# daisy9542/yolo-puncture

Hardware: AMD Instinct MI355X
Metric: images/sec (higher is better)
Workload: dtype bf16

## Files before the change

### include/yolop.h

```cpp
#ifndef YOLOP_H
#define YOLOP_H

#include <stddef.h>
#include <stdint.h>

#ifdef __cplusplus
extern "C" {
#endif

#define YP_OK 0
#define YP_ERR_ARG -1
#define YP_ERR_STATE -2
#define YP_ERR_HIP -3
#define YP_ERR_WEIGHT -4

#define YP_BF16 0
#define YP_F32 1

#define YP_TASK_DETECT 0
#define YP_TASK_SEGMENT 1

#define YP_NM 32
#define YP_MAX_MASKS 480

typedef struct yp_engine yp_engine;

typedef struct yp_model_desc {
    int variant;
    int nc;
    int task;
    int dtype;
    int max_det;
    int family;
} yp_model_desc;

#define YP_FAMILY_V10 0
#define YP_FAMILY_V8 8
#define YP_FAMILY_11 11

const char* yp_last_error(void);

int yp_create(const yp_model_desc* desc, int device, yp_engine** out);
int yp_destroy(yp_engine* e);

int yp_weight_count(const yp_engine* e);
int yp_weight_info(const yp_engine* e, int i, char* name, int name_cap, int64_t shape[4], int* ndim);

int yp_set_weight(yp_engine* e, const char* name, const float* host, const int64_t* shape, int ndim);

int yp_finalize(yp_engine* e);

int yp_forward(yp_engine* e, const uint8_t* in_dev, int B, int H, int W, float* det_out, int32_t* idx_out,
               float* coeff_out, void* stream);

int yp_proto(const yp_engine* e, const void** proto_dev, int* Hp, int* Wp);

int yp_masks(yp_engine* e, int b, const float* coeff_dev, const float* boxes_dev, int n, int oh, int ow,
             int retina, uint8_t* masks_out, int64_t* id_out, int32_t* kept_out, int suppress_small,
             int min_area, void* stream);

int yp_id_mask_resized(yp_engine* e, int b, const float* coeff_dev, const float* boxes_dev, int n, int oh, int ow, int rh,
                       int rw, int64_t* id_out, int32_t* kept_out, int suppress_small, int min_area, void* stream);

int yp_masks_frames(yp_engine* e, const int32_t* frame_idx_host, int k, const float* coeff_dev, long coeff_row_stride,
                    const float* boxes_dev, int oh, int ow, uint8_t* masks_out, void* stream);
int yp_masks_frames_input(yp_engine* e, const int32_t* frame_idx_host, int k, const float* coeff_dev, long coeff_row_stride,
                          const float* boxes_dev, int oh, int ow, uint8_t* masks_out, void* stream);

#define YP_CONTOURS_LARGEST 0
#define YP_CONTOURS_ALL 1
int yp_mask_contours(const uint8_t* masks_dev, int n, int H, int W, int strategy, int max_pts, int32_t* pts_out, int32_t* count_out,
                     int32_t* parts_out, int parts_cap, double* rect_out, void* stream);
int yp_mask_contours_scaled(const uint8_t* masks_dev, int n, int H, int W, int strategy, int max_pts, int32_t* pts_out, int32_t* count_out,
                            int32_t* parts_out, int parts_cap, double* rect_out, int H0, int W0, void* stream);

#define YP_CONTOURS_ONLY_DECLINED 1
#define YP_CONTOURS_LARGE_MAX_DIM 4096
#define YP_CONTOURS_LARGE_MAX_STARTS 65536
size_t yp_mask_contours_large_workspace(int n, int H, int W);
int yp_mask_contours_large(const uint8_t* masks_dev, int n, int H, int W, int strategy, int max_pts, int32_t* pts_out, int32_t* count_out,
                           int32_t* parts_out, int parts_cap, double* rect_out, int H0, int W0, int flags, void* workspace_dev,
                           size_t workspace_bytes, void* stream);

int yp_letterbox(const uint8_t* src_dev, int h0, int w0, uint8_t* dst_dev, int out_h, int out_w, int new_h, int new_w,
                 int top, int left, int pad_value, void* stream);
int yp_letterbox_batch(const uint8_t* src_dev, int n, int h0, int w0, uint8_t* dst_dev, int out_h, int out_w, int new_h,
                       int new_w, int top, int left, int pad_value, void* stream);

typedef struct yp_u2net yp_u2net;
int yp_u2net_create(int variant, int dtype, int device, yp_u2net** out);
int yp_u2net_destroy(yp_u2net* e);
int yp_u2net_weight_count(const yp_u2net* e);
int yp_u2net_weight_info(const yp_u2net* e, int i, char* name, int name_cap, int64_t shape[4], int* ndim);
int yp_u2net_set_weight(yp_u2net* e, const char* name, const float* host, const int64_t* shape, int ndim);
int yp_u2net_finalize(yp_u2net* e);
int yp_u2net_forward(yp_u2net* e, const uint8_t* bgr_dev, int B, int H, int W, float* prob_out, float* norm_out,
                     uint8_t* mask_out, void* stream);
int yp_u2net_forward_crops(yp_u2net* e, const uint8_t* frames_dev, int N, int H, int W, const int32_t* windows, const int32_t* frame_idx,
                           int B, int ch, int cw, float* prob_out, uint8_t* crop_mask_out, uint8_t* frame_mask_out, void* stream);
int yp_u2net_set_graph(yp_u2net* e, int enable);
int yp_u2net_tensor_count(const yp_u2net* e);
int yp_u2net_tensor_info(const yp_u2net* e, int i, char* name, int name_cap, int dims[4] );
int yp_u2net_tensor_read(yp_u2net* e, int i, float* host_out);
#define YP_U2_OP_INFO 17
int yp_u2net_op_count(const yp_u2net* e);
int yp_u2net_op_info(const yp_u2net* e, int i, char* name, int name_cap, int32_t* info, int info_cap);

typedef struct yp_cls yp_cls;
int yp_cls_create(int variant, int dtype, int device, yp_cls** out);
int yp_cls_destroy(yp_cls* e);
int yp_cls_weight_count(const yp_cls* e);
int yp_cls_weight_info(const yp_cls* e, int i, char* name, int name_cap, int64_t shape[4], int* ndim);
int yp_cls_set_weight(yp_cls* e, const char* name, const float* host, const int64_t* shape, int ndim);
int yp_cls_finalize(yp_cls* e);
int yp_cls_forward(yp_cls* e, const uint8_t* frames_dev, int B, int H, int W, int bgr, const int32_t* boxes_dev, float* logits_out,
                   float* prob_out, int32_t* cls_out, void* stream);
int yp_cls_set_graph(yp_cls* e, int enable);
int yp_cls_tensor_count(const yp_cls* e);
int yp_cls_tensor_info(const yp_cls* e, int i, char* name, int name_cap, int dims[4] );
int yp_cls_tensor_read(yp_cls* e, int i, float* host_out);

typedef struct yp_comm yp_comm;
int yp_comm_unique_id(void* id128);
int yp_comm_create(const void* id128, int rank, int world, int device, yp_comm** out);
int yp_allgather(yp_comm* c, const void* send_dev, void* recv_dev, size_t bytes_per_rank, void* stream);
int yp_comm_destroy(yp_comm* c);

#define YP_MAX_ANCHORS 294912
int yp_max_batch(const yp_engine* e, int H, int W);
int yp_plan(yp_engine* e, int B, int H, int W);
int yp_op_info(const yp_engine* e, int i, char* name, int name_cap, int* kind, double* flops,
               double* bytes);
int yp_op_kernel(const yp_engine* e, int i, char* name, int name_cap);
int yp_op_output(const yp_engine* e, int i, int* tensor, int* coff, int* C);
int yp_op_input(const yp_engine* e, int i, int* tensor, int* coff, int* C, int* c_read);
int yp_op_fusion(const yp_engine* e, int i, int* pre, int* pre_stored);
int yp_debug_op_form(const yp_engine* e, int i, int* form, int* absorbed, int cap);
int yp_run_op(yp_engine* e, int i, const uint8_t* in_dev, float* det_out, int32_t* idx_out, float* coeff_out, void* stream);
int yp_tensor_write(yp_engine* e, int tensor, int coff, int C, const float* host);
int yp_tensor_count(const yp_engine* e);
int yp_tensor_info(const yp_engine* e, int i, char* name, int name_cap, int dims[4] , int* is_f32);
int yp_tensor_read(yp_engine* e, int i, float* host_out);

int yp_profile(yp_engine* e, const uint8_t* in_dev, int B, int H, int W, float* det_out, int32_t* idx_out,
               float* coeff_out, float* ms_out, int iters, void* stream);

int yp_set_nms(yp_engine* e, float conf, float iou);

int yp_set_autotune(yp_engine* e, int enable);

int yp_tuning_export(const yp_engine* e, int32_t* cfg_out, int cap);
int yp_tuning_import(yp_engine* e, int B, int H, int W, const int32_t* cfg, int n);

int yp_debug_force_conv_cfg(int cfg);
int yp_debug_op_cfg(const yp_engine* e, int i, int* cfg);
int yp_debug_last_store_form(void);
int yp_debug_conv_families(int* base, int* num_cfgs, int cap);
int yp_debug_ablation(int v);
int yp_debug_head_clocks(uint64_t* out8);
int yp_debug_topk_anchors(const uint32_t* const mk_dev[3], int B, const int hw[3][2], int k, int32_t* sel_out_dev, uint32_t* thr_out_dev, void* stream);
int yp_debug_head_branch_clocks(uint64_t* out8);
int yp_debug_head_winners(yp_engine* e, int32_t* sel_host, float* box_host, float* coeff_host);
int yp_debug_contour_clocks(uint64_t* out12);
int yp_debug_pwsp_clocks(uint64_t* out32);

int yp_tuning_source(const yp_engine* e);

int yp_debug_host_selftest(yp_engine* e);
int yp_debug_graph_info(const yp_engine* e, int64_t* out6);
int yp_debug_head_positions(yp_engine* e, int64_t* out6);
int yp_debug_marker(void* stream);

int yp_set_graph(yp_engine* e, int enable);

#ifdef __cplusplus
}
#endif
#endif
```

### yolo-puncture_amd/csrc/c2f_fused.hip

```cpp
#include "common.h"
#include <cstdio>
#include <cstdlib>
#include <vector>

namespace yp {

constexpr int CF_NW = 8;
constexpr int CF_TH = 8;
constexpr int CF_PW = 20, CF_PP = 12 * 20;
constexpr int CF_TW = 18, CF_TP = 10 * 18;
constexpr int CF_AB = CF_PP * 128;
constexpr int CF_TS = 192 * 64, CF_CS = 128 * 64;
constexpr int CF_W33 = 9 * 32 * 64, CF_W3 = 3 * 64 * 64;
constexpr int CF_LDS = 2 * CF_AB + CF_TS + CF_CS + 2 * CF_W33 + CF_W3 + 512;

__global__ __launch_bounds__(CF_NW * 64) void c2f_fused_kernel(const C2fParams p, const int tiles_h, const int tiles_w, const int G) {
    constexpr unsigned OOB = 0x80000000u;
    extern __shared__ __attribute__((aligned(1024))) unsigned char smem[];
    unsigned char* const ABs = smem;
    unsigned char* const Ts = ABs + 2 * CF_AB;
    unsigned char* const Cs = Ts + CF_TS;
    unsigned char* const W1s = Cs + CF_CS;
    unsigned char* const W2s = W1s + CF_W33;
    unsigned char* const W3s = W2s + CF_W33;
    float* const Bs = (float*)(W3s + CF_W3);

    const int tid = threadIdx.x, lane = tid & 63;
    const int wave = __builtin_amdgcn_readfirstlane(tid >> 6);
    const int fr = lane & 15, fc = lane >> 4;
    const int num_tiles = p.B * tiles_h * tiles_w;

    const int bid = xcd_remap(blockIdx.x, gridDim.x);

    const __amdgpu_buffer_rsrc_t xrs = __builtin_amdgcn_make_buffer_rsrc((void*)p.x, 0, (int)p.x_bytes, 0x00020000);
    const __amdgpu_buffer_rsrc_t w1rs = __builtin_amdgcn_make_buffer_rsrc((void*)p.w1, 0, (int)p.w1_bytes, 0x00020000);
    const __amdgpu_buffer_rsrc_t w2rs = __builtin_amdgcn_make_buffer_rsrc((void*)p.w2, 0, (int)p.w2_bytes, 0x00020000);
    const __amdgpu_buffer_rsrc_t w3rs = __builtin_amdgcn_make_buffer_rsrc((void*)p.w3, 0, (int)p.w3_bytes, 0x00020000);
    const __amdgpu_buffer_rsrc_t yrs = __builtin_amdgcn_make_buffer_rsrc((void*)p.y, 0, (int)p.y_bytes, 0x00020000);

    auto issue_ab = [&](int tile, unsigned char* dst) {
        int t = tile;
        const int tw = t % tiles_w; t /= tiles_w;
        const int th = t % tiles_h;
        const int b = t / tiles_h;
        const bool tv = tile < num_tiles;
#pragma unroll
        for (int k = 0; k < 4; ++k) {
            const int ii = wave + k * CF_NW;
            if (ii < CF_AB / 1024) {
                const int s = ii * 64 + lane;
                const int row = s >> 3, pc = s & 7;
                const int c8 = pc ^ cswz128(row);
                const int py = row / CF_PW, px = row - py * CF_PW;
                const int iy = th * CF_TH - 2 + py, ix = tw * 16 - 2 + px;
                const bool ok = tv && (unsigned)iy < (unsigned)p.H && (unsigned)ix < (unsigned)p.W;
                const unsigned voff = ok ? (unsigned)((((b * p.H + iy) * p.W + ix) * p.x_stride + p.x_coff + c8 * 8) * 2) : OOB;
                __builtin_amdgcn_raw_ptr_buffer_load_lds(xrs, (lds_void*)(dst + ii * 1024), 16, voff, 0, 0, 0);
            }
        }
    };

    for (int ii = wave; ii < CF_W33 / 1024; ii += CF_NW) {
        const int s = ii * 64 + lane;
        const int rg = s >> 2, pc = s & 3;
        const int c8 = pc ^ cswz64(rg);
        const int n = rg & 31, tap = rg >> 5;
        __builtin_amdgcn_raw_ptr_buffer_load_lds(w1rs, (lds_void*)(W1s + ii * 1024), 16, (unsigned)((n * p.Kpad1 + tap * 32 + c8 * 8) * 2), 0, 0, 0);
        __builtin_amdgcn_raw_ptr_buffer_load_lds(w2rs, (lds_void*)(W2s + ii * 1024), 16, (unsigned)((n * p.Kpad2 + tap * 32 + c8 * 8) * 2), 0, 0, 0);
    }
    for (int ii = wave; ii < CF_W3 / 1024; ii += CF_NW) {
        const int s = ii * 64 + lane;
        const int rg = s >> 2, pc = s & 3;
        const int c8 = pc ^ cswz64(rg);
        const int n = rg & 63, ch = rg >> 6;
        __builtin_amdgcn_raw_ptr_buffer_load_lds(w3rs, (lds_void*)(W3s + ii * 1024), 16, (unsigned)((n * p.Kpad3 + ch * 32 + c8 * 8) * 2), 0, 0, 0);
    }

    const int cf = wave & 1, wq = wave >> 1;
    if (tid < 128) Bs[tid] = tid < 32 ? p.bias1[tid] : tid < 64 ? p.bias2[tid - 32] : p.bias3[tid - 64];
    const float* const bias1 = Bs + cf * 16 + fc * 4;
    const float* const bias2 = Bs + 32 + cf * 16 + fc * 4;
    const float* const bias3 = Bs + 64 + cf * 32 + fc * 4;

    int tile = bid;
    issue_ab(tile, ABs);
    __builtin_amdgcn_s_waitcnt(0 | (7 << 4) | (0xF << 8));

    asm volatile("s_waitcnt lgkmcnt(0)" ::: "memory");
    __builtin_amdgcn_s_barrier();
    bf16x8 wf1[9], wf2[9];
#pragma unroll
    for (int tap = 0; tap < 9; ++tap) {
        const int rw = tap * 32 + cf * 16 + fr;
        wf1[tap] = *(const bf16x8*)(W1s + swz64((unsigned)(rw * 64 + fc * 16)));
        wf2[tap] = *(const bf16x8*)(W2s + swz64((unsigned)(rw * 64 + fc * 16)));
    }

    unsigned long long clk[7] = {0, 0, 0, 0, 0, 0, 0};
#define CF_STAMP(i) if (p.clk) { const unsigned long long now = __builtin_amdgcn_s_memtime(); clk[i] += now - last; last = now; }
    unsigned long long last = p.clk ? __builtin_amdgcn_s_memtime() : 0ull;
    for (int it = 0; tile < num_tiles; tile += G, ++it) {
        int t = tile;
        const int tw = t % tiles_w; t /= tiles_w;
        const int th = t % tiles_h;
        const int b = t / tiles_h;
        unsigned char* const AB = ABs + (it & 1) * CF_AB;
        if (it) asm volatile("s_waitcnt vmcnt(4)" ::: "memory");
        CF_STAMP(0)
        __builtin_amdgcn_s_barrier();
        CF_STAMP(1)
        issue_ab(tile + G, ABs + ((it & 1) ^ 1) * CF_AB);

        {
            constexpr int D = 3;
            bf16x8 xf[D + 1][3];
            int ty[3], tx[3];
#pragma unroll
            for (int j = 0; j < 3; ++j) {
                const int q = (wq + 4 * j) * 16 + fr;
                const int qc = q < CF_TP ? q : CF_TP - 1;
                ty[j] = qc / CF_TW; tx[j] = qc - ty[j] * CF_TW;
            }
            auto rd = [&](int tap) {
#pragma unroll
                for (int j = 0; j < 3; ++j) {
                    const int pp = (ty[j] + tap / 3) * CF_PW + tx[j] + tap % 3;
                    xf[tap % (D + 1)][j] = *(const bf16x8*)(AB + pp * 128 + (((4 + fc) ^ cswz128(pp)) * 16));
                }
            };
            f32x4 acc[3];
#pragma unroll
            for (int j = 0; j < 3; ++j) acc[j] = *(const f32x4*)bias1;
#pragma unroll
            for (int tap = 0; tap < D; ++tap) rd(tap);
            __builtin_amdgcn_sched_barrier(0);
#pragma unroll
            for (int tap = 0; tap < 9; ++tap) {
                if (tap + D < 9) rd(tap + D);
#pragma unroll
                for (int j = 0; j < 3; ++j) acc[j] = __builtin_amdgcn_mfma_f32_16x16x32_bf16(wf1[tap], xf[tap % (D + 1)][j], acc[j], 0, 0, 0);
                __builtin_amdgcn_sched_barrier(0);
            }
#pragma unroll
            for (int j = 0; j < 3; ++j) {
                const int q = (wq + 4 * j) * 16 + fr;
                const int iy = th * CF_TH - 1 + ty[j], ix = tw * 16 - 1 + tx[j];
                const bool in = (unsigned)iy < (unsigned)p.H && (unsigned)ix < (unsigned)p.W;
                float v[4] = {acc[j][0], acc[j][1], acc[j][2], acc[j][3]};
                if (p.act1 == ACT_SILU) silu4_packed(v);
                __attribute__((aligned(8))) __bf16 o[4];
#pragma unroll
                for (int i = 0; i < 4; ++i) o[i] = (__bf16)(in ? v[i] : 0.f);
                if (q < CF_TP) lds_write8(Ts + q * 64 + (((cf * 2 + (fc >> 1)) ^ cswz64(q)) * 16) + (fc & 1) * 8, *(const unsigned long long*)o);
            }
        }
        asm volatile("s_waitcnt lgkmcnt(0)" ::: "memory");
        CF_STAMP(2)
        __builtin_amdgcn_s_barrier();
        CF_STAMP(3)
        {
            constexpr int D = 4;
            bf16x8 xf[D + 1][2];
            unsigned long long rr[2] = {0ull, 0ull};
            auto rd = [&](int tap) {
#pragma unroll
                for (int j = 0; j < 2; ++j) {
                    const int tp = (wq + 4 * j + tap / 3) * CF_TW + fr + tap % 3;
                    xf[tap % (D + 1)][j] = *(const bf16x8*)(Ts + swz64((unsigned)(tp * 64 + fc * 16)));
                }
            };
            f32x4 acc[2];
#pragma unroll
            for (int j = 0; j < 2; ++j) acc[j] = *(const f32x4*)bias2;
#pragma unroll
            for (int tap = 0; tap < D; ++tap) rd(tap);
#pragma unroll
            for (int j = 0; j < 2; ++j) {
                const int pp = (wq + 4 * j + 2) * CF_PW + fr + 2;
                if (p.shortcut) rr[j] = lds_read8_async(AB + pp * 128 + (((4 + cf * 2 + (fc >> 1)) ^ cswz128(pp)) * 16) + (fc & 1) * 8);
            }
            __builtin_amdgcn_sched_barrier(0);
#pragma unroll
            for (int tap = 0; tap < 9; ++tap) {
                if (tap + D < 9) rd(tap + D);
#pragma unroll
                for (int j = 0; j < 2; ++j) acc[j] = __builtin_amdgcn_mfma_f32_16x16x32_bf16(wf2[tap], xf[tap % (D + 1)][j], acc[j], 0, 0, 0);
                __builtin_amdgcn_sched_barrier(0);
            }
            asm volatile("s_waitcnt lgkmcnt(0)" : "+v"(rr[0]), "+v"(rr[1])::"memory");
#pragma unroll
            for (int j = 0; j < 2; ++j) {
                float v[4] = {acc[j][0], acc[j][1], acc[j][2], acc[j][3]};
                if (p.act2 == ACT_SILU) silu4_packed(v);
                if (p.shortcut) {
                    const unsigned lo = (unsigned)rr[j], hi = (unsigned)(rr[j] >> 32);
                    v[0] += __uint_as_float(lo << 16); v[1] += __uint_as_float(lo & 0xffff0000u);
                    v[2] += __uint_as_float(hi << 16); v[3] += __uint_as_float(hi & 0xffff0000u);
                }
                const int q = (wq + 4 * j) * 16 + fr;
                __attribute__((aligned(8))) __bf16 o[4] = {(__bf16)v[0], (__bf16)v[1], (__bf16)v[2], (__bf16)v[3]};
                lds_write8(Cs + q * 64 + (((cf * 2 + (fc >> 1)) ^ cswz64(q)) * 16) + (fc & 1) * 8, *(const unsigned long long*)o);
            }
        }
        asm volatile("s_waitcnt lgkmcnt(0)" ::: "memory");
        CF_STAMP(4)
        __builtin_amdgcn_s_barrier();
        CF_STAMP(5)
        {
            bf16x8 xf[2][3], wf3[3][2];
#pragma unroll
            for (int ch = 0; ch < 3; ++ch)
#pragma unroll
                for (int a = 0; a < 2; ++a) { const int rw = ch * 64 + (cf * 2 + a) * 16 + fr; wf3[ch][a] = *(const bf16x8*)(W3s + swz64((unsigned)(rw * 64 + fc * 16))); }
#pragma unroll
            for (int j = 0; j < 2; ++j) {
                const int r = wq + 4 * j;
                const int pp = (r + 2) * CF_PW + fr + 2, q = r * 16 + fr;
                xf[j][0] = *(const bf16x8*)(AB + pp * 128 + ((fc ^ cswz128(pp)) * 16));
                xf[j][1] = *(const bf16x8*)(AB + pp * 128 + (((4 + fc) ^ cswz128(pp)) * 16));
                xf[j][2] = *(const bf16x8*)(Cs + swz64((unsigned)(q * 64 + fc * 16)));
            }
            f32x4 acc[2][2];
#pragma unroll
            for (int j = 0; j < 2; ++j)
#pragma unroll
                for (int a = 0; a < 2; ++a) acc[j][a] = *(const f32x4*)(bias3 + a * 16);
#pragma unroll
            for (int ch = 0; ch < 3; ++ch)
#pragma unroll
                for (int j = 0; j < 2; ++j)
#pragma unroll
                    for (int a = 0; a < 2; ++a) acc[j][a] = __builtin_amdgcn_mfma_f32_16x16x32_bf16(wf3[ch][a], xf[j][ch], acc[j][a], 0, 0, 0);
            const int wo = tw * 16 + fr;
#pragma unroll
            for (int j = 0; j < 2; ++j) {
                const int ho = th * CF_TH + wq + 4 * j;
                const bool pix_ok = (ho < p.H) && (wo < p.W);
                const unsigned m = (unsigned)((b * p.H + ho) * p.W + wo);
#pragma unroll
                for (int a = 0; a < 2; ++a) {
                    float v[4] = {acc[j][a][0], acc[j][a][1], acc[j][a][2], acc[j][a][3]};
                    if (p.act3 == ACT_SILU) silu4_packed(v);
                    const int co = (cf * 2 + a) * 16 + fc * 4;
                    const unsigned off = pix_ok ? (m * (unsigned)p.y_stride + (unsigned)(p.y_coff + co)) * 2u : OOB;
                    __attribute__((aligned(8))) __bf16 o[4] = {(__bf16)v[0], (__bf16)v[1], (__bf16)v[2], (__bf16)v[3]};
                    __builtin_amdgcn_raw_buffer_store_b64(*(const __attribute__((ext_vector_type(2))) unsigned*)o, yrs, off, 0, 0);
                }
            }
        }
        CF_STAMP(6)
    }
    __builtin_amdgcn_s_waitcnt(0 | (7 << 4) | (0xF << 8));
    if (p.clk && lane == 0)
        for (int i = 0; i < 7; ++i) p.clk[((size_t)blockIdx.x * CF_NW + wave) * 7 + i] = clk[i];
}

bool c2f_fused_valid(const C2fParams& p) {
    if (p.C != 32 || p.Cout != 64 || p.Kpad1 != 9 * 32 || p.Kpad2 != 9 * 32 || p.Kpad3 != 96) return false;
    if ((p.x_stride & 7) || (p.x_coff & 7) || (p.y_stride & 3) || (p.y_coff & 3)) return false;
    if (p.x_bytes >= (1ull << 31) || p.y_bytes >= (1ull << 31)) return false;
    if (p.w1_bytes < (size_t)32 * p.Kpad1 * 2 || p.w2_bytes < (size_t)32 * p.Kpad2 * 2 || p.w3_bytes < (size_t)64 * p.Kpad3 * 2) return false;
    const long covered = (long)((p.H + CF_TH - 1) / CF_TH * CF_TH) * ((p.W + 15) / 16 * 16);
    if (covered * 2 > (long)p.H * p.W * 3) return false;
    return true;
}

hipError_t launch_c2f_fused(const C2fParams& p, hipStream_t st) {
    const int tiles_h = (p.H + CF_TH - 1) / CF_TH, tiles_w = (p.W + 15) / 16;
    const int num_tiles = p.B * tiles_h * tiles_w;
    int G = 256;
    if (G > num_tiles) G = num_tiles;
    static size_t granted = 0;
    if (hipError_t e = allow_dynamic_lds((const void*)c2f_fused_kernel, (size_t)CF_LDS, granted)) return e;
    static const bool clocks = env_on("YOLOP_C2F_CLOCKS");
    if (clocks) {
        C2fParams q = p;
        const size_t n = (size_t)G * CF_NW * 7;
        if (hipMalloc((void**)&q.clk, n * 8) != hipSuccess) return hipErrorOutOfMemory;
        hipLaunchKernelGGL(c2f_fused_kernel, dim3(G), dim3(CF_NW * 64), (size_t)CF_LDS, st, q, tiles_h, tiles_w, G);
        (void)hipStreamSynchronize(st);
        std::vector<unsigned long long> h(n);
        (void)hipMemcpy(h.data(), q.clk, n * 8, hipMemcpyDeviceToHost);
        (void)hipFree(q.clk);
        static const char* nm[7] = {"wait-dma", "barrier1", "S2", "barrier2", "S3", "barrier3", "S4"};
        const double tiles_per = (double)num_tiles / G;
        for (int w = 0; w < CF_NW; w += 7) {
            fprintf(stderr, "[c2f clocks] wave %d, s_memtime ticks per tile:", w);
            for (int i = 0; i < 7; ++i) {
                double s = 0;
                for (int g = 0; g < G; ++g) s += (double)h[((size_t)g * CF_NW + w) * 7 + i];
                fprintf(stderr, " %s %.0f", nm[i], s / G / tiles_per);
            }
            fprintf(stderr, "\n");
        }
        return hipGetLastError();
    }
    hipLaunchKernelGGL(c2f_fused_kernel, dim3(G), dim3(CF_NW * 64), (size_t)CF_LDS, st, p, tiles_h, tiles_w, G);
    return hipGetLastError();
}

}
```

### yolo-puncture_amd/csrc/common.h

```cpp
#pragma once
#include <hip/hip_runtime.h>
#include <stdint.h>
#include <atomic>
#include <cstdlib>
#include <string>
#include <vector>

namespace yp {

enum DType { DT_BF16 = 0, DT_F32 = 1 };
enum Act { ACT_NONE = 0, ACT_SILU = 1, ACT_RELU = 2 };

enum OpKind {
    OP_STEM = 0,
    OP_CONV = 1,
    OP_DWCONV = 2,
    OP_POOL5 = 3,
    OP_UPSAMPLE = 4,
    OP_ATTN = 5,
    OP_HEAD = 6,
    OP_CONVT = 7,
    OP_AMAX = 9,
    OP_POOL3 = 8,
};

struct View {
    int t = -1;
    int coff = 0;
    int C = 0;
};

struct TensorDesc {
    std::string name;
    int C = 0;
    int sdiv = 1;
    bool f32 = false;
    int H = 0, W = 0;
    size_t bytes = 0;
    void* ptr = nullptr;
};

struct WeightDesc {
    std::string name;
    int cout = 0, cin_g = 0, k = 1, groups = 1;
    int cin_pad = 0;
    bool transposed = false;
    bool is_stem = false;
    bool have_w = false, have_b = false;
    std::vector<float> w, b;
    void* d_w = nullptr;
    void* d_w2 = nullptr;
    float* d_b = nullptr;
    int Kpad = 0;
    size_t mat_bytes = 0;
};

enum Form {
    FORM_PLAIN = 0,
    FORM_DWPW,
    FORM_DWPW_TAIL,
    FORM_S2PW,
    FORM_FRONTEND,
    FORM_C2F,
    FORM_SCDOWN,
    FORM_PWSP,
    FORM_CLS_OUT,
};

struct Op {
    int kind = OP_CONV;
    std::string name;
    View in, out, res;
    int widx = -1;
    int k = 1, s = 1, act = ACT_NONE;
    int gs = 0, gstride = 0;
    int nh = 0, kd = 0, hd = 0;
    View box[3], cls[3], cf[3];
    View amax[3];
    int nlev = 0;
    double flops = 0, bytes = 0;
    std::string kernel;
    int cfg = -1;
    int fuse_dw = -1;
    Form form = FORM_PLAIN;
    bool skip = false;
    int fuse_pre = -1;
    int stem_op = -1;
    int fold_up = -1;
    bool folded = false;
    int c2f_m1 = -1, c2f_m2 = -1;
    int scd_pre = -1;
    int fuse_tail = -1, tail_amax = -1;
    int amax_post = -1;
    int pw_pre = -1;
    bool pw_store = false;
    int lane = 0;
    bool nms = false;
    int hb_box[3][3] = {{-1, -1, -1}, {-1, -1, -1}, {-1, -1, -1}}, hb_cf[3][3] = {{-1, -1, -1}, {-1, -1, -1}, {-1, -1, -1}};
    bool sparse_box = false, sparse_cf = false;
};

struct ConvParams {
    const void* x; int x_stride, x_coff;
    int H, W, Cin;
    const void* w; int Kpad;
    const float* bias;
    void* y; int y_stride, y_coff; int Ho, Wo, Cout;
    const void* res; int res_stride, res_coff;
    int M;
    int ks, stride, pad;
    int act, out_f32;
    int up, oy, ox;
    size_t x_bytes, w_bytes, y_bytes;
    int cfg;
    int dbg;
    const void* x2; size_t x2_bytes; int x2_stride, x2_coff, x2_C, x2_H, x2_W;
    const void* w2; const float* bias2; int C2, act2, Kpad2; size_t w2_bytes;
    unsigned long long* clk;
    int dil;
    int pool_in, src_H, src_W;
    int up_bilinear;
    int wide;
};

struct DwParams {
    const void* x; int x_stride, x_coff; int H, W, C;
    const void* w;
    const float* bias;
    void* y; int y_stride, y_coff; int Ho, Wo;
    const void* res; int res_stride, res_coff;
    int B, ks, stride, pad, act;
    int gs, gstride;
    size_t x_bytes;
};

struct StemParams {
    const uint8_t* x; int H, W;
    const float* w;
    const void* wpk;
    const float* bias;
    void* y; int y_stride, y_coff; int Ho, Wo, C0; int B;
    int act;
};

struct FrontParams {
    const uint8_t* img; int imgH, imgW, B;
    const void* w0; const float* bias0; int act0, C0; int H1, W1;
    const void* w1; const float* bias1; int act1, C1, Kpad1; size_t w1_bytes;
    const void* w2; const float* bias2; int act2, C2, Kpad2; size_t w2_bytes;
    void* y; int y_stride, y_coff; size_t y_bytes; int Ho, Wo;
    unsigned long long* clk;
};
bool frontend_valid(const FrontParams& p);
hipError_t launch_frontend(const FrontParams& p, hipStream_t st);

struct C2fParams {
    const void* x; int x_stride, x_coff; size_t x_bytes;
    int B, H, W, C;
    const void* w1; const float* bias1; int act1, Kpad1; size_t w1_bytes;
    const void* w2; const float* bias2; int act2, Kpad2; size_t w2_bytes;
    int shortcut;
    const void* w3; const float* bias3; int act3, Kpad3, Cout; size_t w3_bytes;
    void* y; int y_stride, y_coff; size_t y_bytes;
    unsigned long long* clk;
};
bool c2f_fused_valid(const C2fParams& p);

struct ScdParams {
    const void* x; int x_stride, x_coff; size_t x_bytes; int B, H, W, K;
    const void* w1; const float* bias1; int act1, Kpad1, C; size_t w1_bytes;
    const void* wd; const float* biasd; int actd;
    void* y; int y_stride, y_coff; size_t y_bytes; int Ho, Wo;
    unsigned long long* clk;
};
bool scdown_fused_valid(const ScdParams& p);
const char* scdown_fused_kernel_name(const ScdParams& p);
bool scdown_stream_valid(const ScdParams& p);
const char* scdown_stream_kernel_name(const ScdParams& p);
hipError_t launch_scdown_stream(const ScdParams& p, hipStream_t st);
hipError_t launch_scdown_fused(const ScdParams& p, hipStream_t st);
hipError_t launch_c2f_fused(const C2fParams& p, hipStream_t st);

struct PoolParams {
    const void* x; int x_stride, x_coff;
    void* y; int y_stride, y_coff;
    int B, H, W, C;
};

struct UpParams {
    const void* x; int x_stride, x_coff;
    void* y; int y_stride, y_coff;
    int B, H, W, C;
};

struct AttnParams {
    const void* qkv; int q_stride, q_coff;
    void* o; int o_stride, o_coff;
    int B, N, nh, kd, hd;
    float scale;
};

struct HeadParams {
    const float* box[3]; const float* cls[3]; const float* cf[3];
    int hw[3][2]; int nlev;
    int B, nc, max_det, A;
    float* det; int32_t* idx; float* coeff;
    void* scratch;
    const unsigned* mk[3];
    const float* nms_params;
    float* nms_ws;
    int* sp_sel; int* sp_wlist; int* sp_wcount; unsigned* sp_thr; float* sp_box; float* sp_cf;
    int* sp_plist; int* sp_pcount; int sp_plist_off[3], sp_plist_cap[3];
};
hipError_t launch_head_stage1(const HeadParams& p, hipStream_t st);
hipError_t launch_head_stage2(const HeadParams& p, hipStream_t st);
constexpr int HEAD_MAXK = 512;
struct HeadBranchParams {
    const void* x[3]; int x_stride[3], x_coff[3], H[3], W[3], Cin[3]; size_t x_bytes[3];
    const void* w0[3]; int Kpad0[3]; const float* b0[3];
    const void* w1[3]; int Kpad1[3]; const float* b1[3];
    const void* w2[3]; int Kpad2[3]; const float* b2[3];
    int act0, act1;
    int B, max_det, maxk, cmid, cout;
    int A0, A1;
    const int* sel;
    const int* wlist;
    const int* wcount;
    float* out;
    const int* plist; const int* pcount;
    int plist_off[3], plist_cap[3];
    void* t0; size_t t0_off[3], t0_bytes;
    int pos_grid;
};
bool head_branch_valid(const HeadBranchParams& p);
hipError_t launch_head_branch(const HeadBranchParams& p, hipStream_t st);
hipError_t launch_head_nms(const HeadParams& p, hipStream_t st);
size_t head_nms_scratch_bytes(int B, int A);
hipError_t launch_head_nms_large(const HeadParams& p, hipStream_t st);

inline bool env_on(const char* name) { const char* v = std::getenv(name); return v && *v == '1'; }
inline int env_int(const char* name, int dflt) { const char* v = std::getenv(name); return v ? atoi(v) : dflt; }

inline hipError_t allow_dynamic_lds(const void* kern, size_t bytes, size_t& granted) {
    if (bytes <= 64 * 1024 || bytes <= granted) return hipSuccess;
    hipFuncAttributes fa;
    if (hipError_t e = hipFuncGetAttributes(&fa, kern)) return e;
    const size_t most = 160 * 1024 - fa.sharedSizeBytes;
    if (hipError_t e = hipFuncSetAttribute(kern, hipFuncAttributeMaxDynamicSharedMemorySize, (int)most)) return e;
    granted = most;
    return hipSuccess;
}

inline std::atomic<bool>& store_form_watched() { static std::atomic<bool> v{false}; return v; }
inline std::atomic<int>& last_store_form() { static std::atomic<int> v{-1}; return v; }
inline bool wide_store_ok(int want, int frags, int Cout, int y_stride, int y_coff, bool out_f32, const void* res = nullptr, int res_stride = 0, int res_coff = 0) {
    const bool ok = want && !out_f32 && frags > 0 && (frags & 1) == 0 && (Cout % 32) == 0 && (y_stride & 7) == 0 && (y_coff & 7) == 0 &&
                    (!res || ((res_stride & 7) == 0 && (res_coff & 7) == 0));
    if (store_form_watched().load(std::memory_order_relaxed)) last_store_form().store(ok ? 1 : 0, std::memory_order_relaxed);
    return ok;
}
inline ConvParams with_store_form(const ConvParams& p, int frags) {
    ConvParams q = p;
    q.wide = wide_store_ok(p.wide, frags, p.Cout, p.y_stride, p.y_coff, p.out_f32 != 0, p.res, p.res_stride, p.res_coff) ? 1 : 0;
    return q;
}

hipError_t launch_conv(const ConvParams& p, int dtype, hipStream_t st);
hipError_t launch_conv_igemm(const ConvParams& p, int dtype, hipStream_t st);
std::string conv_kernel_name(const ConvParams& p, int dtype);
bool conv_cfg_usable(const ConvParams& p, int dtype, int cfg);
bool conv_dma_supported(const ConvParams& p);
int conv_dma_requested_cfg(const ConvParams& p);
int conv_launch_cfg(const ConvParams& p, int dtype);
void conv_dma_force_cfg(int cfg);
int conv_dma_forced_cfg();
void conv_set_debug_ablation(int v);
int conv_debug_ablation();
bool tile_balance_enabled(int family);

struct ConvFamily {
    int base, num_cfgs;
    bool (*valid)(const ConvParams& p, int c);
    std::string (*symbol)(const ConvParams& p, int c);
    hipError_t (*launch)(const ConvParams& p, int c, hipStream_t st);
    bool two_source;
    const char* tune_env;
    bool opt_in;
};
inline const char* res_f32_args(const ConvParams& p) { return p.out_f32 ? ",false,true" : p.res ? ",true,false" : ",false,false"; }
extern const ConvFamily conv_dma_family, conv_halo_family, conv_halo_p_family, conv_dma_p_family, conv_dma_lc_family, conv_halo_s2_family,
    conv_tile1_family, conv_wreg_family, conv_pxd_family, conv_ks_family, conv_wres_family, conv_wrs_family;
constexpr int kNumConvFamilies = 12;
extern const ConvFamily* const kConvFamilies[kNumConvFamilies];
int conv_halo_s2_pw_cfg(const ConvParams& p);
hipError_t launch_dwconv(const DwParams& p, int dtype, hipStream_t st);
std::string dwconv_kernel_name(const DwParams& p, int dtype);
hipError_t launch_stem(const StemParams& p, int dtype, hipStream_t st);
std::string stem_kernel_name(const StemParams& p, int dtype);
hipError_t launch_pool5(const PoolParams& p, int dtype, hipStream_t st);
hipError_t launch_sppf_pool3(const PoolParams& p, int dtype, hipStream_t st);
bool sppf_pool3_fits(const PoolParams& p, int dtype);
bool dwconv_mfma_valid(const DwParams& p, int dtype);
hipError_t launch_dwconv_mfma(const DwParams& p, hipStream_t st);
const char* dwconv_mfma_kernel_name(const DwParams& p);
hipError_t launch_upsample(const UpParams& p, int dtype, hipStream_t st);
hipError_t launch_attention(const AttnParams& p, int dtype, hipStream_t st);
bool attention_fits(const AttnParams& p, int dtype, int* max_tokens);
bool conv_small_valid(const ConvParams& p, int dtype);
hipError_t launch_conv_small(const ConvParams& p, int dtype, hipStream_t st);
bool conv_halo_f32_valid(const ConvParams& p, int dtype);
hipError_t launch_conv_halo_f32(const ConvParams& p, int dtype, hipStream_t st);
hipError_t launch_head(const HeadParams& p, hipStream_t st);
hipError_t launch_letterbox(const uint8_t* src, int h0, int w0, uint8_t* dst, int out_h, int out_w, int new_h, int new_w, int top,
                            int left, int pad, hipStream_t st);
hipError_t launch_letterbox_batch(const uint8_t* src, int n, int h0, int w0, uint8_t* dst, int out_h, int out_w, int new_h, int new_w,
                                  int top, int left, int pad, hipStream_t st);
size_t head_scratch_bytes(int B, int A);
constexpr int HEAD_LDS_ANCHORS = 12288;
constexpr int HEAD_MAX_ANCHORS = HEAD_LDS_ANCHORS * (HEAD_LDS_ANCHORS / HEAD_MAXK);
inline int head_large_chunks(int A) { return (A + HEAD_LDS_ANCHORS - 1) / HEAD_LDS_ANCHORS; }
inline size_t head_large_ckeys_offset(int B, int A) { return ((size_t)B * A * sizeof(unsigned) + 255) & ~(size_t)255; }
hipError_t launch_head_large(const HeadParams& p, int mode, hipStream_t st);
const char* head_large_kernel_name(int mode);
hipError_t head_read_clocks(unsigned long long* out8);
hipError_t head_branch_read_clocks(unsigned long long* out8);
hipError_t launch_copy_out(const float* det, float* det_out, const int32_t* idx, int32_t* idx_out, const float* coeff, float* coeff_out,
                           size_t rows, hipStream_t st);
hipError_t launch_anchor_max_level(const float* cls, int B, int HW, int nc, unsigned* out, hipStream_t st);

struct DwPwParams {
    const void* x; int x_stride, x_coff; int B, H, W, C; size_t x_bytes;
    const void* w_dw; const float* b_dw; int act_dw;
    const void* w_pw; int Kpad; size_t wpw_bytes; const float* b_pw; int act_pw;
    void* y; int y_stride, y_coff; size_t y_bytes; int Cout; int out_f32;
    unsigned long long* clk;
    const void* w3; int Kpad3; size_t w3_bytes; const float* b3; int C3;
    float* y3; int y3_stride, y3_coff; size_t y3_bytes;
    unsigned* keys;
};
bool dwpw_stream_valid(const DwPwParams& p);
hipError_t launch_dwpw_stream(const DwPwParams& p, hipStream_t st);
struct PwSpParams {
    const void* x; int x_stride, x_coff; size_t x_bytes; int B, H, W, K;
    const void* w1; const float* bias1; int act1, Kpad1, C1; size_t w1_bytes;
    void* y1; int y1_stride, y1_coff;
    const void* res1; int res1_stride, res1_coff;
    int sp;
    int sp_c0, Csp;
    const void* wd; const float* biasd; int actd;
    const void* res; int res_stride, res_coff;
    void* y2; int y2_stride, y2_coff;
    int dbg;
};
bool pwsp_valid(const PwSpParams& p);
const char* pwsp_kernel_name(const PwSpParams& p);
constexpr int PWSP_CFG = 1000;
hipError_t launch_pwsp(const PwSpParams& p, hipStream_t st);
hipError_t pwsp_read_clocks(unsigned long long* out32);

struct ClsOutParams {
    const void* x; int x_stride, x_coff; size_t x_bytes;
    int M, K, nc;
    const void* w; int Kpad; size_t w_bytes; const float* bias;
    float* y; int y_stride, y_coff;
    unsigned* keys;
};
bool cls_out_valid(const ClsOutParams& p);
const char* cls_out_kernel_name(const ClsOutParams& p);
hipError_t launch_cls_out(const ClsOutParams& p, hipStream_t st);

bool conv_dwpw_valid(const DwPwParams& p);
const char* conv_dwpw_kernel_name(const DwPwParams& p);
hipError_t launch_conv_dwpw(const DwPwParams& p, hipStream_t st);

struct MaskParams {
    const void* proto; int Hp, Wp;
    const float* coeff; const float* boxes; int n;
    int oh, ow;
    int t, l, ch, cw;
    float bsx, bsy;
    int crop_before;
    uint8_t* masks; int64_t* ids; int32_t* kept; int32_t* area;
    int suppress_small, min_area;
    int rh, rw;
};
hipError_t launch_masks(const MaskParams& p, int dtype, hipStream_t st);
size_t masks_workspace_bytes(const MaskParams& p);
struct MaskFramesParams {
    MaskParams p;
    const int32_t* fidx; int k;
    size_t proto_stride; long coeff_stride;
};
hipError_t launch_masks_frames(const MaskFramesParams& f, float* M, int dtype, hipStream_t st);
hipError_t contour_read_clocks(unsigned long long* out12);
hipError_t launch_contours(const uint8_t* masks, int n, int H, int W, int strategy, int max_pts, int32_t* pts, int32_t* count, int32_t* parts, int parts_cap,
                           double* rect, hipStream_t st);
hipError_t launch_contours_scaled(const uint8_t* masks, int n, int H, int W, int H0, int W0, int strategy, int max_pts, int32_t* pts, int32_t* count,
                                  int32_t* parts, int parts_cap, double* rect, hipStream_t st);

constexpr int CL_MAXDIM = 4096;
constexpr int CL_MAXCAND = 65536;
size_t contours_large_workspace_bytes(int n, int H, int W);
hipError_t launch_contours_large(const uint8_t* masks, int n, int H, int W, int strategy, int max_pts, int32_t* pts, int32_t* count, int32_t* parts,
                                 int parts_cap, double* rect, int H0, int W0, int flags, void* workspace, hipStream_t st);

static inline uint16_t f2bf(float f) {
    uint32_t u;
    __builtin_memcpy(&u, &f, 4);
    if ((u & 0x7fffffffu) > 0x7f800000u) return (uint16_t)((u >> 16) | 0x40);
    u += 0x7fffu + ((u >> 16) & 1u);
    return (uint16_t)(u >> 16);
}
static inline float bf2f(uint16_t h) {
    uint32_t u = ((uint32_t)h) << 16;
    float f;
    __builtin_memcpy(&f, &u, 4);
    return f;
}

}

#include "kernel_util.h"
```

### yolo-puncture_amd/csrc/conv_dwpw_stream.hip

```cpp
#include "common.h"
#include <cstdlib>

namespace yp {

constexpr int DS_TH = 8, DS_TW = 16;
constexpr int DS_C = 128;
constexpr int DS_HP = (DS_TH + 2) * (DS_TW + 2);
constexpr int DS_PIECES = 48;
constexpr int DS_HB = DS_PIECES * 1024;
constexpr int DS_AB = DS_TH * DS_TW * 256;

template <int NW>
__global__ __launch_bounds__(NW * 64, 2) void conv_dwpw_stream_kernel(const DwPwParams p, const int tiles_h, const int tiles_w, const int num_tiles, const int G) {
    constexpr int RPW = DS_TH / NW;
    constexpr int NFW = 8 / NW;
    constexpr int NSLOT = NW == 8 ? 2 : 1;
    constexpr int NST = DS_TH * NFW;
    constexpr unsigned OOB = 0x80000000u;
    extern __shared__ __attribute__((aligned(1024))) unsigned char smem[];
    unsigned char* const Hs = smem;
    unsigned char* const As = smem + NSLOT * DS_HB;
    const int tid = threadIdx.x, lane = tid & 63;
    const int wave = __builtin_amdgcn_readfirstlane(tid >> 6);
    const int fr = lane & 15, fc = lane >> 4;

    const __amdgpu_buffer_rsrc_t xrs = __builtin_amdgcn_make_buffer_rsrc((void*)p.x, 0, (int)p.x_bytes, 0x00020000);
    const __amdgpu_buffer_rsrc_t wrs = __builtin_amdgcn_make_buffer_rsrc((void*)p.w_pw, 0, (int)p.wpw_bytes, 0x00020000);
    const __amdgpu_buffer_rsrc_t yrs = __builtin_amdgcn_make_buffer_rsrc((void*)p.y, 0, (int)p.y_bytes, 0x00020000);

    auto issue_tile = [&](int tile, int slot) {
        int t = tile;
        const int tw = t % tiles_w; t /= tiles_w;
        const int th = t % tiles_h;
        const int b = t / tiles_h;
        const int h0 = th * DS_TH - 1, w0 = tw * DS_TW - 1;
        unsigned char* const dst = Hs + slot * DS_HB;
#pragma unroll
        for (int j = 0; j < DS_PIECES / NW; ++j) {
            const int ii = wave + j * NW;
            const int s = ii * 64 + lane;
            const int hp = s >> 4, c = s & 15;
            const int hy = hp / (DS_TW + 2), hx = hp - hy * (DS_TW + 2);
            const int hi = h0 + hy, wi = w0 + hx;
            const bool ok = tile < num_tiles && hp < DS_HP && (unsigned)hi < (unsigned)p.H && (unsigned)wi < (unsigned)p.W;
            const unsigned voff = ok ? (unsigned)((((b * p.H + hi) * p.W + wi) * p.x_stride + p.x_coff + c * 8) * 2) : OOB;
            __builtin_amdgcn_raw_ptr_buffer_load_lds(xrs, (lds_void*)(dst + ii * 1024), 16, voff, 0, 0, 0);
        }
    };
    int tile = blockIdx.x;
    issue_tile(tile, 0);

    f32x2 wd[9], bd;
    {
        const unsigned* w32 = (const unsigned*)p.w_dw;
#pragma unroll
        for (int t = 0; t < 9; ++t) {
            const unsigned u = w32[t * (DS_C / 2) + lane];
            wd[t] = f32x2{__uint_as_float(u << 16), __uint_as_float(u & 0xffff0000u)};
        }
        bd = f32x2{p.b_dw[2 * lane], p.b_dw[2 * lane + 1]};
    }
    bf16x8 wreg[4][NFW];
    float bpw[NFW][4];
#pragma unroll
    for (int i = 0; i < NFW; ++i) {
#pragma unroll
        for (int ks = 0; ks < 4; ++ks) {
            const unsigned voff = (unsigned)((((wave * NFW + i) * 16 + fr) * p.Kpad + (ks >> 1) * 64 + fc * 16 + (ks & 1) * 8) * 2);
            const __attribute__((ext_vector_type(4))) unsigned v = __builtin_amdgcn_raw_buffer_load_b128(wrs, voff, 0, 0);
            wreg[ks][i] = __builtin_bit_cast(bf16x8, v);
        }
#pragma unroll
        for (int r = 0; r < 4; ++r) { const int co = (wave * NFW + i) * 16 + fc * 4 + r; bpw[i][r] = (co < p.Cout) ? p.b_pw[co] : 0.f; }
    }
    wait_vmcnt<0>();
#pragma unroll
    for (int t = 0; t < 9; ++t) asm volatile("" : "+v"(wd[t]));
    asm volatile("" : "+v"(bd));
#pragma unroll
    for (int i = 0; i < NFW; ++i) {
#pragma unroll
        for (int ks = 0; ks < 4; ++ks) asm volatile("" : "+v"(wreg[ks][i]));
#pragma unroll
        for (int r = 0; r < 4; ++r) asm volatile("" : "+v"(bpw[i][r]));
    }

    const unsigned as_l = lds_addr(As);
    for (int it = 0; tile < num_tiles; tile += G, ++it) {
        if (it == 0) wait_vmcnt<0>();
        else wait_vmcnt<NST>();
        __builtin_amdgcn_s_barrier();
        const int slot = NSLOT == 2 ? (it & 1) : 0;
        if (NSLOT == 2) issue_tile(tile + G, slot ^ 1);
        int t = tile;
        const int tw = t % tiles_w; t /= tiles_w;
        const int th = t % tiles_h;
        const int b = t / tiles_h;
#pragma unroll
        for (int rr = 0; rr < RPW; ++rr) {
            const int row = wave * RPW + rr;
            f32x2 win[3][3];
            auto rd = [&](int ky, int col) -> f32x2 {
                const unsigned u = *(const unsigned*)(Hs + slot * DS_HB + ((row + ky) * (DS_TW + 2) + col) * 256 + lane * 4);
                return f32x2{__uint_as_float(u << 16), __uint_as_float(u & 0xffff0000u)};
            };
#pragma unroll
            for (int ky = 0; ky < 3; ++ky) { win[ky][0] = rd(ky, 0); win[ky][1] = rd(ky, 1); }
#pragma unroll
            for (int x = 0; x < DS_TW; ++x) {
#pragma unroll
                for (int ky = 0; ky < 3; ++ky) win[ky][2] = rd(ky, x + 2);
                f32x2 a = bd;
#pragma unroll
                for (int ky = 0; ky < 3; ++ky)
#pragma unroll
                    for (int kx = 0; kx < 3; ++kx) a = __builtin_elementwise_fma(win[ky][kx], wd[ky * 3 + kx], a);
                if (p.act_dw == ACT_SILU) {
                    f32x2 e = a * -1.4426950408889634f;
                    e[0] = __builtin_amdgcn_exp2f(e[0]); e[1] = __builtin_amdgcn_exp2f(e[1]);
                    e = e + 1.0f;
                    e[0] = __builtin_amdgcn_rcpf(e[0]); e[1] = __builtin_amdgcn_rcpf(e[1]);
                    a = a * e;
                }
                __attribute__((aligned(4))) __bf16 o[2] = {(__bf16)a[0], (__bf16)a[1]};
                const int px = row * DS_TW + x;
                const unsigned dst = as_l + (unsigned)(px * 256 + (((lane >> 2) ^ (px & 15)) << 4) + (lane & 3) * 4);
                asm volatile("ds_write_b32 %0, %1" : : "v"(dst), "v"(*(const unsigned*)o) : "memory");
#pragma unroll
                for (int ky = 0; ky < 3; ++ky) { win[ky][0] = win[ky][1]; win[ky][1] = win[ky][2]; }
            }
        }
        asm volatile("s_waitcnt lgkmcnt(0)" ::: "memory");
        __builtin_amdgcn_s_barrier();
        if (NSLOT == 1) issue_tile(tile + G, 0);
        f32x4 acc[NFW][DS_TH];
#pragma unroll
        for (int i = 0; i < NFW; ++i)
#pragma unroll
            for (int f = 0; f < DS_TH; ++f) acc[i][f] = f32x4{bpw[i][0], bpw[i][1], bpw[i][2], bpw[i][3]};
#pragma unroll
        for (int ks = 0; ks < 4; ++ks) {
            const int ch = (ks >> 1) * 8 + fc * 2 + (ks & 1);
            bf16x8 xf[DS_TH];
#pragma unroll
            for (int f = 0; f < DS_TH; ++f) xf[f] = *(const bf16x8*)(As + (f * 16 + fr) * 256 + ((ch ^ fr) << 4));
#pragma unroll
            for (int i = 0; i < NFW; ++i)
#pragma unroll
                for (int f = 0; f < DS_TH; ++f) acc[i][f] = __builtin_amdgcn_mfma_f32_16x16x32_bf16(wreg[ks][i], xf[f], acc[i][f], 0, 0, 0);
        }
        const int wo = tw * DS_TW + fr;
#pragma unroll
        for (int i = 0; i < NFW; ++i) {
            const int co = (wave * NFW + i) * 16 + fc * 4;
#pragma unroll
            for (int f = 0; f < DS_TH; ++f) {
                const int ho = th * DS_TH + f;
                const bool ok = ho < p.H && wo < p.W && co < p.Cout;
                float v[4] = {acc[i][f][0], acc[i][f][1], acc[i][f][2], acc[i][f][3]};
                if (p.act_pw == ACT_SILU) silu4_packed(v);
                __attribute__((aligned(8))) __bf16 o[4] = {(__bf16)v[0], (__bf16)v[1], (__bf16)v[2], (__bf16)v[3]};
                const unsigned off = ok ? (unsigned)((((b * p.H + ho) * p.W + wo) * p.y_stride + p.y_coff + co) * 2) : OOB;
                __builtin_amdgcn_raw_buffer_store_b64(*(const __attribute__((ext_vector_type(2))) unsigned*)o, yrs, off, 0, 0);
            }
        }
    }
    wait_vmcnt<0>();
}

bool dwpw_stream_valid(const DwPwParams& p) {
    static const bool off = env_on("YOLOP_NO_DWPW_STREAM");
    if (off || p.w3 || p.out_f32 || p.clk) return false;
    if (p.C != DS_C || p.Kpad != DS_C || p.Cout != 128) return false;
    if ((p.x_stride & 7) || (p.x_coff & 7) || (p.y_stride & 3) || (p.y_coff & 3)) return false;
    if (p.x_bytes >= (1ull << 31) || p.y_bytes >= (1ull << 31) || p.wpw_bytes >= (1ull << 31)) return false;
    if (p.act_dw != ACT_SILU && p.act_dw != ACT_NONE) return false;
    if (p.act_pw != ACT_SILU && p.act_pw != ACT_NONE) return false;
    return (long)((p.H + DS_TH - 1) / DS_TH * DS_TH) * ((p.W + DS_TW - 1) / DS_TW * DS_TW) * 2 <= (long)p.H * p.W * 3;
}

template <int NW>
static hipError_t launch_dwpw_stream_t(const DwPwParams& p, hipStream_t st) {
    const size_t sh = (size_t)(NW == 8 ? 2 : 1) * DS_HB + DS_AB;
    auto kern = conv_dwpw_stream_kernel<NW>;
    static size_t granted = 0;
    if (hipError_t e = allow_dynamic_lds((const void*)kern, sh, granted)) return e;
    const int tiles_h = (p.H + DS_TH - 1) / DS_TH, tiles_w = (p.W + DS_TW - 1) / DS_TW;
    const int num_tiles = p.B * tiles_h * tiles_w;
    const int gmax = NW == 8 ? 256 : 512;
    const int G = num_tiles < gmax ? num_tiles : gmax;
    hipLaunchKernelGGL(kern, dim3((unsigned)G), dim3(NW * 64), sh, st, p, tiles_h, tiles_w, num_tiles, G);
    return hipGetLastError();
}

hipError_t launch_dwpw_stream(const DwPwParams& p, hipStream_t st) {
    if (!dwpw_stream_valid(p)) return hipErrorInvalidValue;
    static const bool one = env_on("YOLOP_DWPW_STREAM_ONE");
    return one ? launch_dwpw_stream_t<8>(p, st) : launch_dwpw_stream_t<4>(p, st);
}

}
```

### yolo-puncture_amd/csrc/conv_wres.hip

```cpp
#include "common.h"

namespace yp {

constexpr int WR_NW = 8;
constexpr int WR_MAXNF = 8;

template <int N, int FM, int NFW> __device__ __forceinline__ void wr_wait_lgkm(bf16x8 (&xs)[FM], bf16x8 (&ws)[NFW]) {
    static_assert(N >= 0 && N < 16, "lgkmcnt range");
    asm volatile("s_waitcnt lgkmcnt(%0)" : : "n"(N) : "memory");
#pragma unroll
    for (int f = 0; f < FM; ++f) asm volatile("" : "+v"(xs[f]));
#pragma unroll
    for (int i = 0; i < NFW; ++i) asm volatile("" : "+v"(ws[i]));
}

template <int TP, int WGN, bool HAS_RES>
__global__ __launch_bounds__(WR_NW * 64) void conv_wres_kernel(const ConvParams p, const int NB, const int nblk, const int G, const int TPe) {
    constexpr int WGM = WR_NW / WGN;
    constexpr int FM = TP / (16 * WGM);
    constexpr int NFW = WR_MAXNF / WGN;
    static_assert(FM >= 1 && FM * 16 * WGM == TP, "pixel tile");
    constexpr unsigned OOB = 0x80000000u;
    extern __shared__ __attribute__((aligned(1024))) unsigned char smem[];
    const int K = p.Cin, KA = p.x2_C, KB = K - KA;
    const int RBW = K * 2, RBA = KA * 2, RBB = KB * 2;
    const int mA = (KA % 128) == 0 ? 15 : 7, mB = (KB % 128) == 0 ? 15 : 7, mW = ((K % 128) == 0 && (KA % 128) == 0) ? 15 : 7;
    const int nfb = (NB + 15) >> 4;
    const int nfw = nfb / WGN;
    unsigned char* const Ws = smem;
    const size_t xtile = (size_t)TP * RBW;
    unsigned char* const Xs = smem + (size_t)nfb * 16 * RBW;
    const int tid = threadIdx.x, lane = tid & 63;
    const int wave = __builtin_amdgcn_readfirstlane(tid >> 6);
    const int wm = wave % WGM, wn = wave / WGM;
    const int fr = lane & 15, fc = lane >> 4;
    const int ntiles = (p.M + TPe - 1) / TPe;
    const int HoWo = p.Ho * p.Wo;

    const int xcd = blockIdx.x & 7, slot = blockIdx.x >> 3;
    const int nb = slot % nblk, g = (slot / nblk) * 8 + xcd;
    const int Gt = G / nblk;
    const int n0 = nb * NB;

    const __amdgpu_buffer_rsrc_t xrs = __builtin_amdgcn_make_buffer_rsrc((void*)p.x, 0, (int)p.x_bytes, 0x00020000);
    const __amdgpu_buffer_rsrc_t x2rs = __builtin_amdgcn_make_buffer_rsrc((void*)(KA > 0 ? p.x2 : p.x), 0, (int)(KA > 0 ? p.x2_bytes : p.x_bytes), 0x00020000);
    const __amdgpu_buffer_rsrc_t wrs = __builtin_amdgcn_make_buffer_rsrc((void*)p.w, 0, (int)p.w_bytes, 0x00020000);
    const __amdgpu_buffer_rsrc_t yrs = __builtin_amdgcn_make_buffer_rsrc((void*)p.y, 0, (int)p.y_bytes, 0x00020000);

    auto issue_tile = [&](int tile, unsigned char* dst) {
        const long row0 = (long)tile * TPe;
        if (KA > 0) {
            const int cpr = RBA >> 4, pieces = (TP * cpr) >> 6;
            for (int ii = wave; ii < pieces; ii += WR_NW) {
                const int s = ii * 64 + lane;
                const int r = s / cpr, pc = s - r * cpr;
                const int c = pc ^ (r & mA);
                const long m = row0 + r;
                unsigned voff = OOB;
                if (m < p.M && r < TPe) {
                    const int mi = (int)m;
                    const int b = mi / HoWo, q = mi - b * HoWo;
                    const int ho = q / p.Wo, wo = q - ho * p.Wo;
                    voff = (unsigned)((((b * p.x2_H + (ho >> 1)) * p.x2_W + (wo >> 1)) * p.x2_stride + p.x2_coff + c * 8) * 2);
                }
                __builtin_amdgcn_raw_ptr_buffer_load_lds(x2rs, (lds_void*)(dst + ii * 1024), 16, voff, 0, 0, 0);
            }
        }
        {
            unsigned char* const d2 = dst + (size_t)TP * RBA;
            const int cpr = RBB >> 4, pieces = (TP * cpr) >> 6;
            for (int ii = wave; ii < pieces; ii += WR_NW) {
                const int s = ii * 64 + lane;
                const int r = s / cpr, pc = s - r * cpr;
                const int c = pc ^ (r & mB);
                const long m = row0 + r;
                const unsigned voff = (m < p.M && r < TPe) ? (unsigned)((m * p.x_stride + p.x_coff + KA + c * 8) * 2) : OOB;
                __builtin_amdgcn_raw_ptr_buffer_load_lds(xrs, (lds_void*)(d2 + ii * 1024), 16, voff, 0, 0, 0);
            }
        }
    };
    {
        const int cpr = RBW >> 4, pieces = (nfb * 16 * cpr) >> 6;
        for (int ii = wave; ii < pieces; ii += WR_NW) {
            const int s = ii * 64 + lane;
            const int r = s / cpr, pc = s - r * cpr;
            const int c = pc ^ (r & mW);
            const unsigned voff = (unsigned)(((n0 + r) * p.Kpad + c * 8) * 2);
            __builtin_amdgcn_raw_ptr_buffer_load_lds(wrs, (lds_void*)(Ws + ii * 1024), 16, voff, 0, 0, 0);
        }
    }
    int tile = g;
    if (tile < ntiles) issue_tile(tile, Xs);

    float bias[NFW][4];
#pragma unroll
    for (int i = 0; i < NFW; ++i)
#pragma unroll
        for (int r = 0; r < 4; ++r) {
            const int co = n0 + (wn * nfw + i) * 16 + fc * 4 + r;
            bias[i][r] = (i < nfw && co < p.Cout) ? p.bias[co] : 0.f;
        }
    wait_vmcnt<0>();
#pragma unroll
    for (int i = 0; i < NFW; ++i)
#pragma unroll
        for (int r = 0; r < 4; ++r) asm volatile("" : "+v"(bias[i][r]));

    for (int it = 0; tile < ntiles; tile += Gt, ++it) {
        if (it == 0) wait_vmcnt<0>();
        else wait_vmcnt<FM * NFW>();
        __builtin_amdgcn_s_barrier();
        if (tile + Gt < ntiles) issue_tile(tile + Gt, Xs + ((it & 1) ^ 1) * xtile);
        const unsigned char* const XA = Xs + (it & 1) * xtile;
        const unsigned char* const XB = XA + (size_t)TP * RBA;
        f32x4 acc[NFW][FM];
#pragma unroll
        for (int i = 0; i < NFW; ++i)
#pragma unroll
            for (int f = 0; f < FM; ++f) acc[i][f] = f32x4{bias[i][0], bias[i][1], bias[i][2], bias[i][3]};
        auto run_segment = [&](const unsigned char* X, int rb, int kchunk0, int nks, int mX) {
            unsigned xrow[FM], wrow[NFW];
            const unsigned xl = (unsigned)(size_t)(const __attribute__((address_space(3))) unsigned char*)X;
            const unsigned wl = (unsigned)(size_t)(const __attribute__((address_space(3))) unsigned char*)Ws;
#pragma unroll
            for (int f = 0; f < FM; ++f) xrow[f] = xl + (unsigned)(((wm * FM + f) * 16 + fr) * rb);
#pragma unroll
            for (int i = 0; i < NFW; ++i) wrow[i] = wl + (unsigned)(((wn * nfw + min(i, nfw - 1)) * 16 + fr) * RBW + kchunk0 * 16);
            const unsigned swx = (unsigned)(fr & mX), sww = (unsigned)(fr & mW);
            auto rd = [&](bf16x8 (&xd)[FM], bf16x8 (&wd)[NFW], int ks) {
                const unsigned ch = (unsigned)(ks * 4 + fc);
                const unsigned offx = (ch ^ swx) << 4, offw = (ch ^ sww) << 4;
#pragma unroll
                for (int f = 0; f < FM; ++f) asm volatile("ds_read_b128 %0, %1" : "=v"(xd[f]) : "v"(xrow[f] + offx));
#pragma unroll
                for (int i = 0; i < NFW; ++i) asm volatile("ds_read_b128 %0, %1" : "=v"(wd[i]) : "v"(wrow[i] + offw));
            };
            auto mma = [&](bf16x8 (&xd)[FM], bf16x8 (&wd)[NFW]) {
#pragma unroll
                for (int i = 0; i < NFW; ++i)
#pragma unroll
                    for (int f = 0; f < FM; ++f) acc[i][f] = __builtin_amdgcn_mfma_f32_16x16x32_bf16(wd[i], xd[f], acc[i][f], 0, 0, 0);
            };
            bf16x8 xa[FM], wa[NFW], xb[FM], wb[NFW];
            rd(xa, wa, 0);
            for (int ks = 0; ks < nks; ks += 2) {
                rd(xb, wb, ks + 1);
                wr_wait_lgkm<FM + NFW>(xa, wa);
                mma(xa, wa);
                if (ks + 2 < nks) {
                    rd(xa, wa, ks + 2);
                    wr_wait_lgkm<FM + NFW>(xb, wb);
                } else {
                    wr_wait_lgkm<0>(xb, wb);
                }
                mma(xb, wb);
            }
        };
        if (KA > 0) run_segment(XA, RBA, 0, KA >> 5, mA);
        run_segment(XB, RBB, KA >> 3, KB >> 5, mB);
#pragma unroll
        for (int f = 0; f < FM; ++f) {
            const int ri = (wm * FM + f) * 16 + fr;
            const long m = (long)tile * TPe + ri;
#pragma unroll
            for (int i = 0; i < NFW; ++i) {
                const int co = n0 + (wn * nfw + i) * 16 + fc * 4;
                const bool ok = i < nfw && ri < TPe && m < p.M && co < p.Cout;
                float v[4] = {acc[i][f][0], acc[i][f][1], acc[i][f][2], acc[i][f][3]};
                if (p.act == ACT_SILU && i < nfw) silu4_packed(v);
                if (HAS_RES && ok) {
                    const uint2 rr = *(const uint2*)((const __bf16*)p.res + m * p.res_stride + p.res_coff + co);
                    v[0] += __uint_as_float(rr.x << 16); v[1] += __uint_as_float(rr.x & 0xffff0000u);
                    v[2] += __uint_as_float(rr.y << 16); v[3] += __uint_as_float(rr.y & 0xffff0000u);
                }
                __attribute__((aligned(8))) __bf16 o[4] = {(__bf16)v[0], (__bf16)v[1], (__bf16)v[2], (__bf16)v[3]};
                const unsigned off = ok ? (unsigned)((m * p.y_stride + p.y_coff + co) * 2) : OOB;
                __builtin_amdgcn_raw_buffer_store_b64(*(const __attribute__((ext_vector_type(2))) unsigned*)o, yrs, off, 0, 0);
            }
        }
    }
    wait_vmcnt<0>();
}

struct WresCfg { int TP, WGN; const char* name; };
static const WresCfg kWres[] = {
    {64, 2, "conv_wres_kernel<64,2"},
    {128, 2, "conv_wres_kernel<128,2"},
    {32, 4, "conv_wres_kernel<32,4"},
};
constexpr int kNumWres = (int)(sizeof(kWres) / sizeof(kWres[0]));

static std::string conv_wres_symbol(const ConvParams& p, int c) { return std::string(kWres[c].name) + (p.res ? ",true>" : ",false>"); }

static void wres_blocks(const ConvParams& p, const WresCfg& k, int& NB, int& nblk) {
    nblk = (p.Cout + 127) / 128;
    const int q = 16 * k.WGN;
    NB = ((p.Cout + nblk - 1) / nblk + q - 1) / q * q;
}
static size_t wres_lds(const ConvParams& p, const WresCfg& k) {
    int NB, nblk;
    wres_blocks(p, k, NB, nblk);
    return (size_t)NB * p.Cin * 2 + (size_t)2 * k.TP * p.Cin * 2;
}

static bool conv_wres_cfg_valid(const ConvParams& p, int c) {
    if (c < 0 || c >= kNumWres) return false;
    const WresCfg& k = kWres[c];
    if (p.ks != 1 || p.stride != 1 || p.up != 1 || p.w2 || p.out_f32 || p.pool_in || p.up_bilinear) return false;
    if (p.act != ACT_SILU && p.act != ACT_NONE) return false;
    if (p.Cin < 64 || (p.Cin % 64) != 0 || p.Kpad != p.Cin || p.Cin > 1024) return false;
    if (p.x2_C > 0 && ((p.x2_C % 64) != 0 || p.x2_C >= p.Cin || (p.x2_stride & 7) || (p.x2_coff & 7) || p.x2_bytes >= (1ull << 31))) return false;
    if ((p.x_stride & 7) || (p.x_coff & 7)) return false;
    if ((p.Cout & 3) || (p.y_stride & 3) || (p.y_coff & 3) || (p.res && ((p.res_stride & 3) || (p.res_coff & 3)))) return false;
    if (p.x_bytes >= (1ull << 31) || p.w_bytes >= (1ull << 31) || p.y_bytes >= (1ull << 31) || p.M <= 0 || p.Ho <= 0 || p.Wo <= 0) return false;
    if ((((size_t)k.TP * (p.Cin - p.x2_C) * 2) & 1023) || (((size_t)k.TP * p.x2_C * 2) & 1023)) return false;
    return wres_lds(p, k) <= 156 * 1024;
}

template <int TP, int WGN, bool HAS_RES>
static hipError_t launch_wres_t(const ConvParams& p, const WresCfg& k, hipStream_t st) {
    int NB, nblk;
    wres_blocks(p, k, NB, nblk);
    const size_t sh = wres_lds(p, k);
    auto kern = conv_wres_kernel<TP, WGN, HAS_RES>;
    static size_t granted = 0;
    if (hipError_t e = allow_dynamic_lds((const void*)kern, sh, granted)) return e;
    const int ntiles = (p.M + TP - 1) / TP;
    const int gmax = sh <= 78 * 1024 ? 512 : 256;
    int lanes8 = gmax / (8 * nblk);
    if (lanes8 < 1) lanes8 = 1;
    while (lanes8 > 1 && (lanes8 - 1) * 8 >= ntiles) --lanes8;
    const int G = lanes8 * 8 * nblk;
    const long lanes = (long)lanes8 * 8;
    const int rounds = (int)((p.M + lanes * TP - 1) / (lanes * TP));
    const int TPe = tile_balance_enabled(2) ? (int)((p.M + lanes * rounds - 1) / (lanes * rounds)) : TP;
    hipLaunchKernelGGL(kern, dim3((unsigned)G), dim3(WR_NW * 64), sh, st, p, NB, nblk, G, TPe);
    return hipGetLastError();
}

static hipError_t launch_conv_wres(const ConvParams& p, int c, hipStream_t st) {
    if (!conv_wres_cfg_valid(p, c)) return hipErrorInvalidValue;
    const WresCfg& k = kWres[c];
    const bool r = p.res != nullptr;
    switch (c) {
        case 0: return r ? launch_wres_t<64, 2, true>(p, k, st) : launch_wres_t<64, 2, false>(p, k, st);
        case 1: return r ? launch_wres_t<128, 2, true>(p, k, st) : launch_wres_t<128, 2, false>(p, k, st);
        default: return r ? launch_wres_t<32, 4, true>(p, k, st) : launch_wres_t<32, 4, false>(p, k, st);
    }
}

#if !defined(__HIP_DEVICE_COMPILE__)
const ConvFamily conv_wres_family = {1100, kNumWres, conv_wres_cfg_valid, conv_wres_symbol, launch_conv_wres, true, "YOLOP_NO_WRES", false};
#endif

}
```

### yolo-puncture_amd/csrc/engine.hip

```cpp
#include "../../include/yolop.h"
#include "common.h"
#include <algorithm>
#include <array>
#include <chrono>

#include <cmath>
#include <cstdarg>
#include <cstdio>
#include <cstring>
#include <cstdlib>
#include <dlfcn.h>
#include <fcntl.h>
#include <fstream>
#include <map>
#include <sstream>
#include <memory>

using namespace yp;

static thread_local char g_err[512] = "";
static int fail(int code, const char* fmt, ...) {
    va_list ap;
    va_start(ap, fmt);
    vsnprintf(g_err, sizeof(g_err), fmt, ap);
// ... 524 lines not shown
    }
    B.lane = 0;
    head.lane = 0;
    e.ops.push_back(head);
    return finish_graph_passes(e);
}

static bool views_overlap(const View& a, const View& b) {
    return a.t >= 0 && a.t == b.t && a.coff < b.coff + b.C && b.coff < a.coff + a.C;
}
static std::vector<int> readers_of(const yp_engine& e, const View& v, int except = -1) {
    std::vector<int> r;
    for (size_t j = 0; j < e.ops.size(); ++j)
        if ((int)j != except && (views_overlap(e.ops[j].in, v) || views_overlap(e.ops[j].res, v))) r.push_back((int)j);
    return r;
}

static int finish_graph_passes(yp_engine& e) {
    for (size_t i = 0; i + 1 < e.ops.size(); ++i) {
        const Op& d = e.ops[i];
        Op& c = e.ops[i + 1];
        if (d.kind != OP_DWCONV || d.k != 3 || d.s != 1 || d.res.t >= 0 || d.gs != 0) continue;
        if (c.kind != OP_CONV || c.k != 1 || c.s != 1 || c.res.t >= 0) continue;
        if (c.in.t != d.out.t || c.in.coff != d.out.coff || c.in.C != d.out.C) continue;
        if (readers_of(e, d.out, (int)i + 1).empty()) c.fuse_dw = (int)i;
    }
    for (size_t i = 0; i < e.ops.size(); ++i) {
        const Op& u = e.ops[i];
        if (u.kind != OP_UPSAMPLE || (u.out.C % 64) != 0) continue;
        const std::vector<int> readers = readers_of(e, u.out);
        if (readers.size() != 1) continue;
        Op& c = e.ops[readers[0]];
        if (c.kind != OP_CONV || c.k != 1 || c.s != 1 || views_overlap(c.res, u.out) || c.in.t != u.out.t || c.in.coff != u.out.coff || c.in.C <= u.out.C) continue;
        c.fold_up = (int)i;
    }
    for (size_t i = 0; i + 1 < e.ops.size(); ++i) {
        const Op& a = e.ops[i];
        Op& c = e.ops[i + 1];
        if (a.kind != OP_CONV || a.k != 3 || a.s != 2 || a.res.t >= 0) continue;
        if (c.kind != OP_CONV || c.k != 1 || c.s != 1 || c.res.t >= 0 || c.fold_up >= 0 || c.fuse_dw >= 0) continue;
        if (c.in.t != a.out.t || c.in.coff != a.out.coff || c.in.C != a.out.C) continue;
        if (!readers_of(e, a.out, (int)i + 1).empty()) continue;
        c.fuse_pre = (int)i;
        for (size_t j = 0; j < e.ops.size(); ++j)
            if (e.ops[j].kind == OP_STEM && e.ops[j].out.t == a.in.t && readers_of(e, View{a.in.t, 0, e.tensors[a.in.t].C}, (int)i).empty()) c.stem_op = (int)j;
    }
    for (size_t i = 1; i < e.ops.size(); ++i) {
        Op& c2 = e.ops[i];
        const Op& c1 = e.ops[i - 1];
        if (c2.kind != OP_CONV || c2.k != 1 || c2.s != 1 || c2.res.t >= 0 || c2.act != ACT_NONE || c2.fold_up >= 0 || c2.fuse_dw >= 0 || c2.fuse_pre >= 0) continue;
        if (!e.tensors[c2.out.t].f32 || c2.out.coff != 0 || c2.out.C != e.tensors[c2.out.t].C) continue;
        if (c1.kind != OP_CONV || c1.fuse_dw < 0 || c1.res.t >= 0) continue;
        if (c2.in.t != c1.out.t || c2.in.coff != c1.out.coff || c2.in.C != c1.out.C) continue;
        if (!readers_of(e, c1.out, (int)i).empty()) continue;
        c2.fuse_tail = (int)i - 1;
        if (i + 1 < e.ops.size() && e.ops[i + 1].kind == OP_AMAX && e.ops[i + 1].in.t == c2.out.t) c2.tail_amax = (int)i + 1;
    }
    for (size_t i = 0; i < e.ops.size(); ++i) {
        const Op& m = e.ops[i];
        if (m.kind != OP_AMAX) continue;
        for (size_t j = 0; j < i; ++j) {
            Op& c = e.ops[j];
            if (c.kind == OP_CONV && c.k == 1 && c.s == 1 && c.act == ACT_NONE && c.res.t < 0 && c.fold_up < 0 && c.out.t == m.in.t && c.out.coff == 0 &&
                c.out.C == e.tensors[c.out.t].C && e.tensors[c.out.t].f32 && m.in.coff == 0 && m.in.C == c.out.C)
                c.amax_post = (int)i;
        }
    }
    for (size_t i = 0; i < e.ops.size(); ++i) {
        Op& d = e.ops[i];
        const bool dw = d.kind == OP_DWCONV && (d.k == 3 || d.k == 7) && d.s == 1 && d.gs == 0;
        if (!dw && d.kind != OP_POOL3) continue;
        int c = -1;
        for (size_t j = i; j-- > 0;) {
            if (views_overlap(e.ops[j].out, d.in)) { c = (int)j; break; }
        }
        if (c < 0) continue;
        const Op& pw = e.ops[c];
        if (pw.kind != OP_CONV || pw.k != 1 || pw.s != 1 || pw.res.t >= 0 || pw.fold_up >= 0) continue;
        if (d.in.coff < pw.out.coff || d.in.coff + d.in.C > pw.out.coff + pw.out.C) continue;
        if (e.tensors[pw.out.t].f32 || e.tensors[d.out.t].f32) continue;
        d.pw_pre = c;
    }
    return YP_OK;
}

static bool plain_conv(const Op& o) { return (o.kind == OP_CONV || o.kind == OP_CONVT) && !o.skip && o.form == FORM_PLAIN; }
static size_t tensor_elem_bytes(const yp_engine& e, const TensorDesc& t) { return (t.f32 || e.dtype == DT_F32) ? 4 : 2; }
static double view_bytes(const yp_engine& e, const View& v) {
    if (v.t < 0) return 0.0;
    const TensorDesc& t = e.tensors[v.t];
    return (double)e.pB * t.H * t.W * v.C * (double)tensor_elem_bytes(e, t);
}

struct RunArgs { const uint8_t* in; float* det; int32_t* idx; float* coeff; };

static ConvParams conv_params(const yp_engine& e, const Op& o) {
    if (o.form == FORM_S2PW || o.form == FORM_FRONTEND) {
        const Op& a = e.ops[o.fuse_pre];
        Op a1 = a;
        a1.cfg = o.cfg;
        ConvParams p = conv_params(e, a1);
        const WeightDesc& w2 = e.weights[o.widx];
        const TensorDesc& to = e.tensors[o.out.t];
        p.y = to.ptr; p.y_stride = to.C; p.y_coff = o.out.coff; p.y_bytes = to.bytes;
        p.w2 = w2.d_w; p.bias2 = w2.d_b; p.C2 = o.out.C; p.act2 = o.act; p.Kpad2 = w2.Kpad; p.w2_bytes = w2.mat_bytes;
        return p;
    }
    const WeightDesc& w = e.weights[o.widx];
    const TensorDesc &ti = e.tensors[o.in.t], &to = e.tensors[o.out.t];
    ConvParams p{};
    p.x = ti.ptr; p.x_stride = ti.C; p.x_coff = o.in.coff; p.H = ti.H; p.W = ti.W; p.Cin = o.in.C;
    if (w.cin_pad > o.in.C) p.Cin = w.cin_pad;
    p.w = w.d_w; p.Kpad = w.Kpad; p.bias = w.d_b;
    p.y = to.ptr; p.y_stride = to.C; p.y_coff = o.out.coff; p.Ho = to.H; p.Wo = to.W; p.Cout = o.out.C;
    if (o.res.t >= 0) { const TensorDesc& tr = e.tensors[o.res.t]; p.res = tr.ptr ? tr.ptr : (const void*)1; p.res_stride = tr.C; p.res_coff = o.res.coff; }
    p.M = e.pB * to.H * to.W; p.ks = o.k; p.stride = o.s; p.pad = o.k / 2; p.act = o.act;
    p.out_f32 = (to.f32 && e.dtype == DT_BF16) ? 1 : 0;
    p.wide = (e.dtype == DT_BF16 && !p.out_f32 && !e.narrow_store) ? 1 : 0;
    p.up = 1; p.oy = 0; p.ox = 0;
    p.x_bytes = ti.bytes; p.w_bytes = w.mat_bytes; p.y_bytes = to.bytes; p.cfg = o.cfg; p.dbg = conv_debug_ablation();
    if (o.folded) {
        const Op& u = e.ops[o.fold_up];
        const TensorDesc& t2 = e.tensors[u.in.t];
        p.x2 = t2.ptr; p.x2_bytes = t2.bytes; p.x2_stride = t2.C; p.x2_coff = u.in.coff; p.x2_C = u.out.C; p.x2_H = t2.H; p.x2_W = t2.W;
    }
    return p;
}

static FrontParams front_params(const yp_engine& e, const Op& o, const uint8_t* img) {
    const Op& c1 = e.ops[o.fuse_pre];
    const Op& st = e.ops[o.stem_op];
    const WeightDesc &w0 = e.weights[st.widx], &w1 = e.weights[c1.widx], &w2 = e.weights[o.widx];
    const TensorDesc &t0 = e.tensors[st.out.t], &to = e.tensors[o.out.t];
    FrontParams p{};
    p.img = img; p.imgH = e.pH; p.imgW = e.pW; p.B = e.pB;
    p.w0 = w0.d_w2; p.bias0 = w0.d_b; p.act0 = st.act; p.C0 = st.out.C; p.H1 = t0.H; p.W1 = t0.W;
    p.w1 = w1.d_w; p.bias1 = w1.d_b; p.act1 = c1.act; p.C1 = c1.out.C; p.Kpad1 = w1.Kpad; p.w1_bytes = w1.mat_bytes;
    p.w2 = w2.d_w; p.bias2 = w2.d_b; p.act2 = o.act; p.C2 = o.out.C; p.Kpad2 = w2.Kpad; p.w2_bytes = w2.mat_bytes;
    p.y = to.ptr; p.y_stride = to.C; p.y_coff = o.out.coff; p.y_bytes = to.bytes; p.Ho = to.H; p.Wo = to.W;
    return p;
}

static C2fParams c2f_params(const yp_engine& e, const Op& o) {
    const Op &m1 = e.ops[o.c2f_m1], &m2 = e.ops[o.c2f_m2];
    const WeightDesc &w1 = e.weights[m1.widx], &w2 = e.weights[m2.widx], &w3 = e.weights[o.widx];
    const TensorDesc &ti = e.tensors[o.in.t], &to = e.tensors[o.out.t];
    C2fParams p{};
    p.x = ti.ptr; p.x_stride = ti.C; p.x_coff = o.in.coff; p.x_bytes = ti.bytes; p.B = e.pB; p.H = ti.H; p.W = ti.W; p.C = m1.in.C;
    p.w1 = w1.d_w; p.bias1 = w1.d_b; p.act1 = m1.act; p.Kpad1 = w1.Kpad; p.w1_bytes = w1.mat_bytes;
    p.w2 = w2.d_w; p.bias2 = w2.d_b; p.act2 = m2.act; p.Kpad2 = w2.Kpad; p.w2_bytes = w2.mat_bytes;
    p.shortcut = m2.res.t >= 0 ? 1 : 0;
    p.w3 = w3.d_w; p.bias3 = w3.d_b; p.act3 = o.act; p.Kpad3 = w3.Kpad; p.Cout = o.out.C; p.w3_bytes = w3.mat_bytes;
    p.y = to.ptr; p.y_stride = to.C; p.y_coff = o.out.coff; p.y_bytes = to.bytes;
    if (m1.in.t != o.in.t || m1.in.coff != o.in.coff + p.C || m2.out.t != o.in.t || m2.out.coff != o.in.coff + 2 * p.C || o.in.C != 3 * p.C ||
        m1.k != 3 || m2.k != 3 || m1.s != 1 || m2.s != 1 || m1.out.C != p.C || m2.out.C != p.C || m1.res.t >= 0 ||
        (m2.res.t >= 0 && (m2.res.t != m1.in.t || m2.res.coff != m1.in.coff)) || (to.f32 && e.dtype == DT_BF16)) p.C = 0;
    return p;
}

static ScdParams scd_params(const yp_engine& e, const Op& o) {
    const Op& c1 = e.ops[o.scd_pre];
    const WeightDesc &w1 = e.weights[c1.widx], &wd = e.weights[o.widx];
    const TensorDesc &ti = e.tensors[c1.in.t], &to = e.tensors[o.out.t];
    ScdParams p{};
    p.x = ti.ptr; p.x_stride = ti.C; p.x_coff = c1.in.coff; p.x_bytes = ti.bytes; p.B = e.pB; p.H = ti.H; p.W = ti.W; p.K = c1.in.C;
    p.w1 = w1.d_w; p.bias1 = w1.d_b; p.act1 = c1.act; p.Kpad1 = w1.Kpad; p.C = c1.out.C; p.w1_bytes = w1.mat_bytes;
    p.wd = wd.d_w; p.biasd = wd.d_b; p.actd = o.act;
    p.y = to.ptr; p.y_stride = to.C; p.y_coff = o.out.coff; p.y_bytes = to.bytes; p.Ho = to.H; p.Wo = to.W;
    if (c1.k != 1 || c1.s != 1 || c1.res.t >= 0 || o.k != 3 || o.s != 2 || o.res.t >= 0 || o.gs != 0 || o.in.t != c1.out.t ||
        o.in.coff != c1.out.coff || o.in.C != c1.out.C || o.out.C != c1.out.C || c1.fold_up >= 0 || to.f32) p.K = 0;
    return p;
}

static ClsOutParams cls_out_params(const yp_engine& e, const Op& o) {
    ClsOutParams p{};
    const WeightDesc& w = e.weights[o.widx];
    const TensorDesc &ti = e.tensors[o.in.t], &to = e.tensors[o.out.t], &tk = e.tensors[e.ops[o.amax_post].out.t];
    p.x = ti.ptr; p.x_stride = ti.C; p.x_coff = o.in.coff; p.x_bytes = ti.bytes;
    p.M = e.pB * to.H * to.W; p.K = o.in.C; p.nc = o.out.C;
    p.w = w.d_w; p.Kpad = w.Kpad; p.w_bytes = w.mat_bytes; p.bias = w.d_b;
    p.y = (float*)to.ptr; p.y_stride = to.C; p.y_coff = o.out.coff;
    p.keys = (unsigned*)tk.ptr;
    if (w.cin_pad != o.in.C) p.K = 0;
    return p;
}

static PwSpParams pwsp_params(const yp_engine& e, const Op& o) {
    PwSpParams p{};
    const bool pair = o.kind != OP_CONV;
    const Op& c1 = pair ? e.ops[o.pw_pre] : o;
    const WeightDesc& w1 = e.weights[c1.widx];
    const TensorDesc &ti = e.tensors[c1.in.t], &t1 = e.tensors[c1.out.t];
    p.x = ti.ptr; p.x_stride = ti.C; p.x_coff = c1.in.coff; p.x_bytes = ti.bytes; p.B = e.pB; p.H = ti.H; p.W = ti.W; p.K = c1.in.C;
    p.w1 = w1.d_w; p.bias1 = w1.d_b; p.act1 = c1.act; p.Kpad1 = w1.Kpad; p.C1 = c1.out.C; p.w1_bytes = w1.mat_bytes;
    p.dbg = conv_debug_ablation();
    if (!pair || o.pw_store) { p.y1 = t1.ptr ? t1.ptr : (void*)1; p.y1_stride = t1.C; p.y1_coff = c1.out.coff; }
    if (!pair) {
        if (c1.res.t >= 0) { const TensorDesc& tr = e.tensors[c1.res.t]; p.res1 = tr.ptr ? tr.ptr : (const void*)1; p.res1_stride = tr.C; p.res1_coff = c1.res.coff; }
        if (w1.cin_pad != c1.in.C || t1.f32 || c1.k != 1 || c1.s != 1 || c1.fold_up >= 0) p.sp = -1;
        return p;
    }
    const TensorDesc& t2 = e.tensors[o.out.t];
    p.sp = o.kind == OP_POOL3 ? 3 : (o.k == 3 ? 1 : 2);
    p.sp_c0 = o.in.coff - c1.out.coff; p.Csp = o.in.C;
    if (o.kind == OP_DWCONV) {
        const WeightDesc& wd = e.weights[o.widx];
        p.wd = wd.d_w; p.biasd = wd.d_b; p.actd = o.act;
        if (o.res.t >= 0) { const TensorDesc& tr = e.tensors[o.res.t]; p.res = tr.ptr ? tr.ptr : (const void*)1; p.res_stride = tr.C; p.res_coff = o.res.coff; }
        if (o.out.C != o.in.C) p.sp = -1;
    } else if (o.out.C != 3 * o.in.C) p.sp = -1;
    p.y2 = t2.ptr ? t2.ptr : (void*)1; p.y2_stride = t2.C; p.y2_coff = o.out.coff;
    if (w1.cin_pad != c1.in.C || c1.in.t < 0) p.sp = -1;
    return p;
}

static ConvParams convt_params(const yp_engine& e, const Op& o, int dy, int dx) {
    const WeightDesc& w = e.weights[o.widx];
    const TensorDesc &ti = e.tensors[o.in.t], &to = e.tensors[o.out.t];
    ConvParams p{};
    p.x = ti.ptr; p.x_stride = ti.C; p.x_coff = o.in.coff; p.H = ti.H; p.W = ti.W; p.Cin = o.in.C;
    const size_t sub = (size_t)((w.cout + 127) / 128 * 128) * w.Kpad * e.es();
    p.w = (const char*)w.d_w + sub * (dy * 2 + dx); p.Kpad = w.Kpad; p.bias = w.d_b;
    p.y = to.ptr; p.y_stride = to.C; p.y_coff = o.out.coff; p.Ho = ti.H; p.Wo = ti.W; p.Cout = o.out.C;
    p.M = e.pB * ti.H * ti.W; p.ks = 1; p.stride = 1; p.pad = 0; p.act = o.act; p.out_f32 = 0;
    p.up = 2; p.oy = dy; p.ox = dx;
    p.x_bytes = ti.bytes; p.w_bytes = w.mat_bytes; p.y_bytes = to.bytes; p.cfg = o.cfg;
    return p;
}

static DwPwParams dwpw_params(const yp_engine& e, const Op& c) {
    if (c.form == FORM_DWPW_TAIL) {
        DwPwParams p = dwpw_params(e, e.ops[c.fuse_tail]);
        const WeightDesc& w3 = e.weights[c.widx];
        const TensorDesc& to = e.tensors[c.out.t];
        p.w3 = w3.d_w ? w3.d_w : (const void*)1; p.Kpad3 = w3.Kpad; p.w3_bytes = w3.mat_bytes; p.b3 = w3.d_b ? w3.d_b : (const float*)1; p.C3 = c.out.C;
        p.y3 = to.ptr ? (float*)to.ptr : (float*)1; p.y3_stride = to.C; p.y3_coff = c.out.coff; p.y3_bytes = to.bytes;
        p.keys = c.tail_amax >= 0 ? (unsigned*)e.tensors[e.ops[c.tail_amax].out.t].ptr : nullptr;
        p.out_f32 = 0;
        return p;
    }
    const Op& d = e.ops[c.fuse_dw];
    const WeightDesc &wd = e.weights[d.widx], &wp = e.weights[c.widx];
    const TensorDesc &ti = e.tensors[d.in.t], &to = e.tensors[c.out.t];
    DwPwParams p{};
    p.x = ti.ptr; p.x_stride = ti.C; p.x_coff = d.in.coff; p.B = e.pB; p.H = ti.H; p.W = ti.W; p.C = d.in.C; p.x_bytes = ti.bytes;
    p.w_dw = wd.d_w; p.b_dw = wd.d_b; p.act_dw = d.act;
    p.w_pw = wp.d_w; p.Kpad = wp.Kpad; p.wpw_bytes = wp.mat_bytes; p.b_pw = wp.d_b; p.act_pw = c.act;
    p.y = to.ptr; p.y_stride = to.C; p.y_coff = c.out.coff; p.y_bytes = to.bytes; p.Cout = c.out.C;
    p.out_f32 = (to.f32 && e.dtype == DT_BF16) ? 1 : 0;
    return p;
}

static DwParams dw_params(const yp_engine& e, const Op& o) {
    const WeightDesc& w = e.weights[o.widx];
    const TensorDesc &ti = e.tensors[o.in.t], &to = e.tensors[o.out.t];
    DwParams p{};
    p.x = ti.ptr; p.x_stride = ti.C; p.x_coff = o.in.coff; p.H = ti.H; p.W = ti.W; p.C = o.out.C;
    p.w = w.d_w; p.bias = w.d_b;
    p.y = to.ptr; p.y_stride = to.C; p.y_coff = o.out.coff; p.Ho = to.H; p.Wo = to.W;
    if (o.res.t >= 0) { const TensorDesc& tr = e.tensors[o.res.t]; p.res = tr.ptr ? tr.ptr : (const void*)1; p.res_stride = tr.C; p.res_coff = o.res.coff; }
    p.B = e.pB; p.ks = o.k; p.stride = o.s; p.pad = o.k / 2; p.act = o.act; p.gs = o.gs; p.gstride = o.gstride;
    p.x_bytes = ti.bytes;
    return p;
}

static StemParams stem_params(const yp_engine& e, const Op& o, const uint8_t* img) {
    const WeightDesc& w = e.weights[o.widx];
    const TensorDesc& to = e.tensors[o.out.t];
    StemParams p{};
    p.x = img; p.H = e.pH; p.W = e.pW; p.w = (const float*)w.d_w; p.wpk = w.d_w2; p.bias = w.d_b;
    p.y = to.ptr; p.y_stride = to.C; p.y_coff = o.out.coff; p.Ho = to.H; p.Wo = to.W; p.C0 = o.out.C; p.B = e.pB; p.act = o.act;
    return p;
}

struct FormRec {
    const char* off_env;
    bool own_cfg;
    bool reads_frames;
    int (*absorbed)(const yp_engine& e, const Op& o, int m[3]);
    std::string (*admit)(const yp_engine& e, const Op& o, int& cfg);
    void (*views)(const yp_engine& e, const Op& o, View& in, View& extra);
    hipError_t (*launch)(const yp_engine& e, const Op& o, const RunArgs& a, hipStream_t st);
};
static int link1(int i, int m[3]) { m[0] = i; return i >= 0 ? 1 : 0; }

static int dwpw_absorbed(const yp_engine&, const Op& o, int m[3]) { return link1(o.fuse_dw, m); }
static std::string dwpw_admit(const yp_engine& e, const Op& o, int&) {
    const DwPwParams q = dwpw_params(e, o);
    return conv_dwpw_valid(q) ? conv_dwpw_kernel_name(q) : "";
}
static void dwpw_views(const yp_engine& e, const Op& o, View& in, View&) { in = e.ops[o.fuse_dw].in; }
static hipError_t dwpw_launch(const yp_engine& e, const Op& o, const RunArgs&, hipStream_t st) { return launch_conv_dwpw(dwpw_params(e, o), st); }

static int tail_absorbed(const yp_engine& e, const Op& o, int m[3]) {
    if (o.fuse_tail < 0) return 0;
    m[0] = e.ops[o.fuse_tail].fuse_dw; m[1] = o.fuse_tail; m[2] = o.tail_amax;
    return o.tail_amax >= 0 ? 3 : 2;
}
static std::string tail_admit(const yp_engine& e, const Op& o, int& cfg) {
    return e.tail && e.ops[o.fuse_tail].form == FORM_DWPW ? dwpw_admit(e, o, cfg) : "";
}
static void tail_views(const yp_engine& e, const Op& o, View& in, View& extra) {
    in = e.ops[e.ops[o.fuse_tail].fuse_dw].in;
    if (o.tail_amax >= 0) extra = e.ops[o.tail_amax].out;
}

static int s2pw_absorbed(const yp_engine&, const Op& o, int m[3]) { return link1(o.fuse_pre, m); }
static std::string s2pw_admit(const yp_engine& e, const Op& o, int& cfg) {
    const ConvParams q = conv_params(e, o);
    const int c = conv_halo_s2_pw_cfg(q);
    if (c < 0) return "";
    cfg = conv_halo_s2_family.base + c;
    return conv_halo_s2_family.symbol(q, c);
}
static void s2pw_views(const yp_engine& e, const Op& o, View& in, View&) { in = e.ops[o.fuse_pre].in; }
static hipError_t s2pw_launch(const yp_engine& e, const Op& o, const RunArgs&, hipStream_t st) {
    return conv_halo_s2_family.launch(conv_params(e, o), o.cfg - conv_halo_s2_family.base, st);
}

static int front_absorbed(const yp_engine&, const Op& o, int m[3]) {
    m[0] = o.stem_op; m[1] = o.fuse_pre;
    return o.stem_op >= 0 && o.fuse_pre >= 0 ? 2 : 0;
}
static std::string front_admit(const yp_engine& e, const Op& o, int&) {
    return e.weights[e.ops[o.stem_op].widx].d_w2 && frontend_valid(front_params(e, o, nullptr)) ? "frontend_kernel" : "";
}
static void front_views(const yp_engine&, const Op&, View& in, View&) { in = View{}; }
static hipError_t front_launch(const yp_engine& e, const Op& o, const RunArgs& a, hipStream_t st) { return launch_frontend(front_params(e, o, a.in), st); }

static int c2f_absorbed(const yp_engine&, const Op& o, int m[3]) {
    m[0] = o.c2f_m1; m[1] = o.c2f_m2;
    return o.c2f_m1 >= 0 ? 2 : 0;
}
static std::string c2f_admit(const yp_engine& e, const Op& o, int&) { return c2f_fused_valid(c2f_params(e, o)) ? "c2f_fused_kernel" : ""; }
static void c2f_views(const yp_engine& e, const Op& o, View& in, View&) { in = View{o.in.t, o.in.coff, 2 * e.ops[o.c2f_m1].in.C}; }
static hipError_t c2f_launch(const yp_engine& e, const Op& o, const RunArgs&, hipStream_t st) { return launch_c2f_fused(c2f_params(e, o), st); }

static int scd_absorbed(const yp_engine&, const Op& o, int m[3]) { return link1(o.scd_pre, m); }
static std::string scd_admit(const yp_engine& e, const Op& o, int&) {
    const ScdParams q = scd_params(e, o);
    return scdown_fused_valid(q) ? scdown_fused_kernel_name(q) : "";
}
static void scd_views(const yp_engine& e, const Op& o, View& in, View&) { in = e.ops[o.scd_pre].in; }
static hipError_t scd_launch(const yp_engine& e, const Op& o, const RunArgs&, hipStream_t st) { return launch_scdown_fused(scd_params(e, o), st); }

static int pwsp_absorbed(const yp_engine&, const Op& o, int m[3]) { return link1(o.pw_pre, m); }
static std::string pwsp_admit(const yp_engine& e, const Op& o, int&) {
    const PwSpParams q = pwsp_params(e, o);
    return pwsp_valid(q) ? pwsp_kernel_name(q) : "";
}
static void pwsp_views(const yp_engine& e, const Op& o, View& in, View& extra) {
    in = e.ops[o.pw_pre].in;
    if (o.pw_store) extra = e.ops[o.pw_pre].out;
}
static hipError_t pwsp_launch(const yp_engine& e, const Op& o, const RunArgs&, hipStream_t st) { return launch_pwsp(pwsp_params(e, o), st); }

static int clsout_absorbed(const yp_engine&, const Op& o, int m[3]) { return link1(o.amax_post, m); }
static std::string clsout_admit(const yp_engine& e, const Op& o, int&) {
    const ClsOutParams q = cls_out_params(e, o);
    return cls_out_valid(q) ? cls_out_kernel_name(q) : "";
}
static void clsout_views(const yp_engine& e, const Op& o, View&, View& extra) { extra = e.ops[o.amax_post].out; }
static hipError_t clsout_launch(const yp_engine& e, const Op& o, const RunArgs&, hipStream_t st) { return launch_cls_out(cls_out_params(e, o), st); }

static const FormRec kForms[] = {
         {nullptr, false, false, nullptr, nullptr, nullptr, nullptr},
          {nullptr, false, false, dwpw_absorbed, dwpw_admit, dwpw_views, dwpw_launch},
     {nullptr, false, false, tail_absorbed, tail_admit, tail_views, dwpw_launch},
          {nullptr, true, false, s2pw_absorbed, s2pw_admit, s2pw_views, s2pw_launch},
      {"YOLOP_NO_FRONT", false, true, front_absorbed, front_admit, front_views, front_launch},
           {"YOLOP_NO_C2F", false, false, c2f_absorbed, c2f_admit, c2f_views, c2f_launch},
        {"YOLOP_NO_SCD", false, false, scd_absorbed, scd_admit, scd_views, scd_launch},
          {"YOLOP_NO_PWSP", false, false, pwsp_absorbed, pwsp_admit, pwsp_views, pwsp_launch},
       {"YOLOP_NO_CLSOUT", false, false, clsout_absorbed, clsout_admit, clsout_views, clsout_launch},
};
constexpr int kNumForms = (int)(sizeof(kForms) / sizeof(kForms[0]));
static_assert(kNumForms == FORM_CLS_OUT + 1, "one record per Form, in the enum's order");
static const FormRec* fused(const Op& o) { return (o.skip || o.form == FORM_PLAIN) ? nullptr : &kForms[o.form]; }
static void build_form_params(const yp_engine& e, const Op& o) { int cfg; (void)kForms[o.form].admit(e, o, cfg); }

static void op_views(const yp_engine& e, const Op& o, std::vector<View>& rd, std::vector<View>& wr) {
    rd.clear(); wr.clear();
    if (o.skip) return;
    View in = o.in, extra;
    if (const FormRec* r = fused(o)) r->views(e, o, in, extra);
    if (in.t >= 0) rd.push_back(in);
    if (o.folded) rd.push_back(e.ops[o.fold_up].in);
    if (o.res.t >= 0) rd.push_back(o.res);
    if (o.out.t >= 0) wr.push_back(o.out);
    if (extra.t >= 0) wr.push_back(extra);
    if (o.kind == OP_HEAD)
        for (int l = 0; l < 3; ++l) {
            if (o.sparse_box) rd.push_back(e.ops[o.hb_box[l][0]].in);
            else if (o.box[l].t >= 0) rd.push_back(o.box[l]);
            if (o.cls[l].t >= 0) rd.push_back(o.cls[l]);
            if (o.sparse_cf) rd.push_back(e.ops[o.hb_cf[l][0]].in);
            else if (o.cf[l].t >= 0) rd.push_back(o.cf[l]);
            if (o.amax[l].t >= 0) rd.push_back(o.amax[l]);
        }
}

static void drop_graph(yp_engine& e) {
// ... 1294 lines not shown

int yp_letterbox(const uint8_t* src_dev, int h0, int w0, uint8_t* dst_dev, int out_h, int out_w, int new_h, int new_w, int top, int left,
                 int pad_value, void* stream) {
    if (!src_dev || !dst_dev) return fail(YP_ERR_ARG, "yp_letterbox: null buffer");
    if (h0 <= 0 || w0 <= 0 || new_h <= 0 || new_w <= 0 || out_h <= 0 || out_w <= 0 || top < 0 || left < 0 || top + new_h > out_h ||
        left + new_w > out_w || pad_value < 0 || pad_value > 255)
        return fail(YP_ERR_ARG, "yp_letterbox: bad geometry %dx%d -> %dx%d at (%d,%d) in %dx%d", h0, w0, new_h, new_w, top, left, out_h, out_w);
    if ((long)h0 * w0 * 3 >= (1l << 31) || (long)out_h * out_w * 3 >= (1l << 31)) return fail(YP_ERR_ARG, "yp_letterbox: image too large");
    HIPCHK(launch_letterbox(src_dev, h0, w0, dst_dev, out_h, out_w, new_h, new_w, top, left, pad_value, (hipStream_t)stream));
    return YP_OK;
}

int yp_letterbox_batch(const uint8_t* src_dev, int n, int h0, int w0, uint8_t* dst_dev, int out_h, int out_w, int new_h, int new_w, int top,
                       int left, int pad_value, void* stream) {
    if (n < 0 || n > 65535) return fail(YP_ERR_ARG, "yp_letterbox_batch: n = %d outside [0,65535]", n);
    if (n > 0 && (!src_dev || !dst_dev)) return fail(YP_ERR_ARG, "yp_letterbox_batch: null buffer");
    if (h0 <= 0 || w0 <= 0 || new_h <= 0 || new_w <= 0 || out_h <= 0 || out_w <= 0 || top < 0 || left < 0 || top + new_h > out_h ||
        left + new_w > out_w || pad_value < 0 || pad_value > 255)
        return fail(YP_ERR_ARG, "yp_letterbox_batch: bad geometry %dx%d -> %dx%d at (%d,%d) in %dx%d", h0, w0, new_h, new_w, top, left, out_h, out_w);
    if ((long long)n * h0 * w0 * 3 >= (1ll << 31) || (long long)n * out_h * out_w * 3 >= (1ll << 31))
        return fail(YP_ERR_ARG, "yp_letterbox_batch: batch too large");
    if (n == 0) return YP_OK;
    HIPCHK(launch_letterbox_batch(src_dev, n, h0, w0, dst_dev, out_h, out_w, new_h, new_w, top, left, pad_value, (hipStream_t)stream));
    return YP_OK;
}

int yp_debug_head_clocks(uint64_t* out8) {
    if (!out8) return fail(YP_ERR_ARG, "yp_debug_head_clocks: null output");
    HIPCHK(hipDeviceSynchronize());
    HIPCHK(head_read_clocks((unsigned long long*)out8));
    return YP_OK;
}

int yp_debug_head_branch_clocks(uint64_t* out8) {
    if (!out8) return fail(YP_ERR_ARG, "yp_debug_head_branch_clocks: null output");
    HIPCHK(hipDeviceSynchronize());
    HIPCHK(head_branch_read_clocks((unsigned long long*)out8));
    return YP_OK;
}

int yp_debug_head_winners(yp_engine* e, int32_t* sel_host, float* box_host, float* coeff_host) {
    if (!e) return fail(YP_ERR_ARG, "null engine");
    if (!e->allocated) return fail(YP_ERR_STATE, "no forward has run yet");
    const Op* h = nullptr;
    for (const Op& o : e->ops) if (o.kind == OP_HEAD) h = &o;
    if (!h || !(h->sparse_box || h->sparse_cf) || !e->sp_ws) return 0;
    HIPCHK(hipSetDevice(e->device));
    HIPCHK(hipDeviceSynchronize());
    const SparseWs ws = sparse_ws_layout(*e);
    const char* base = (const char*)e->sp_ws;
    if (sel_host) HIPCHK(hipMemcpy(sel_host, base + ws.sel, (size_t)e->pB * HEAD_MAXK * 4, hipMemcpyDeviceToHost));
    if (box_host && h->sparse_box) HIPCHK(hipMemcpy(box_host, base + ws.box, (size_t)e->pB * e->desc.max_det * 64 * 4, hipMemcpyDeviceToHost));
    if (coeff_host && h->sparse_cf) HIPCHK(hipMemcpy(coeff_host, base + ws.cf, (size_t)e->pB * e->desc.max_det * 32 * 4, hipMemcpyDeviceToHost));
    return (h->sparse_box ? 1 : 0) | (h->sparse_cf ? 2 : 0);
}

int yp_debug_topk_anchors(const uint32_t* const mk_dev[3], int B, const int hw[3][2], int k, int32_t* sel_out_dev, uint32_t* thr_out_dev, void* stream) {
    if (!mk_dev || !hw || !sel_out_dev || !thr_out_dev) return fail(YP_ERR_ARG, "yp_debug_topk_anchors: null argument");
    if (B < 1 || B > 4096) return fail(YP_ERR_ARG, "yp_debug_topk_anchors: B = %d (1 .. 4096)", B);
    if (k < 1 || k > HEAD_MAXK) return fail(YP_ERR_ARG, "yp_debug_topk_anchors: k = %d (1 .. %d)", k, HEAD_MAXK);
    HeadParams p{};
    size_t A = 0;
    for (int l = 0; l < 3; ++l) {
        if (!mk_dev[l]) return fail(YP_ERR_ARG, "yp_debug_topk_anchors: level %d has no keys", l);
        if (hw[l][0] < 1 || hw[l][1] < 1 || hw[l][0] > 65536 || hw[l][1] > 65536) return fail(YP_ERR_ARG, "yp_debug_topk_anchors: level %d is %dx%d", l, hw[l][0], hw[l][1]);
        p.mk[l] = mk_dev[l]; p.hw[l][0] = hw[l][0]; p.hw[l][1] = hw[l][1];
        A += (size_t)hw[l][0] * hw[l][1];
    }
    if (A > (size_t)YP_MAX_ANCHORS) return fail(YP_ERR_ARG, "yp_debug_topk_anchors: %zu anchors; at most %d (YP_MAX_ANCHORS)", A, YP_MAX_ANCHORS);
    p.nlev = 3; p.A = (int)A; p.B = B; p.nc = 1; p.max_det = k;
    const size_t sel_b = (size_t)B * HEAD_MAXK * 4, wl_b = 3 * sel_b, wc_b = ((size_t)B * 3 * 4 + 255) & ~(size_t)255;
    char* ws = nullptr;
    HIPCHK(hipMalloc((void**)&ws, sel_b + wl_b + wc_b + head_scratch_bytes(B, (int)A)));
    p.sp_sel = (int*)ws; p.sp_wlist = (int*)(ws + sel_b); p.sp_wcount = (int*)(ws + sel_b + wl_b); p.sp_thr = thr_out_dev;
    p.scratch = ws + sel_b + wl_b + wc_b;
    hipStream_t st = (hipStream_t)stream;
    hipError_t err = launch_head_stage1(p, st);
    if (err == hipSuccess) err = hipMemcpyAsync(sel_out_dev, p.sp_sel, sel_b, hipMemcpyDeviceToDevice, st);
    if (err == hipSuccess) err = hipStreamSynchronize(st);
    (void)hipFree(ws);
    if (err != hipSuccess) return fail(YP_ERR_HIP, "yp_debug_topk_anchors: %s", hipGetErrorString(err));
    return YP_OK;
}

int yp_tuning_source(const yp_engine* e) {
    if (!e) return YP_ERR_ARG;
    return e->tune_source;
}

int yp_debug_graph_info(const yp_engine* e, int64_t* out6) {
    if (!e || !out6) return fail(YP_ERR_ARG, "yp_debug_graph_info: null argument");
    out6[0] = e->n_captures; out6[1] = e->g_nodes; out6[2] = e->g_edges; out6[3] = e->g_edges_expected;
    out6[4] = (int64_t)e->lanes_used.size() + 1; out6[5] = e->gexec ? 1 : 0;
    return YP_OK;
}

int yp_debug_head_positions(yp_engine* e, int64_t* out6) {
    if (!e || !out6) return fail(YP_ERR_ARG, "yp_debug_head_positions: null argument");
    for (int i = 0; i < 6; ++i) out6[i] = 0;
    if (!e->allocated) return fail(YP_ERR_STATE, "no forward has run yet");
    const Op* h = nullptr;
    for (const Op& o : e->ops) if (o.kind == OP_HEAD) h = &o;
    if (!h || !(h->sparse_box || h->sparse_cf) || !e->sp_ws) return 0;
    HIPCHK(hipSetDevice(e->device));
    HIPCHK(hipDeviceSynchronize());
    const SparseWs ws = sparse_ws_layout(*e);
    const char* base = (const char*)e->sp_ws;
    int pc[8];
    HIPCHK(hipMemcpy(pc, base + ws.pcount, sizeof(pc), hipMemcpyDeviceToHost));
    std::vector<int> wc((size_t)e->pB * 3);
    HIPCHK(hipMemcpy(wc.data(), base + ws.wcount, wc.size() * 4, hipMemcpyDeviceToHost));
    for (int l = 0; l < 3; ++l) {
        out6[l] = std::min(pc[4 + l], ws.plist_cap[l]);
        for (int b = 0; b < e->pB; ++b) out6[3 + l] += wc[(size_t)b * 3 + l];
    }
    return 1;
}

__global__ void op_marker_kernel(int* sink) { if (sink) *sink = 0; }
int yp_debug_marker(void* stream) {
    hipLaunchKernelGGL(op_marker_kernel, dim3(1), dim3(1), 0, (hipStream_t)stream, (int*)nullptr);
    HIPCHK(hipGetLastError());
    return YP_OK;
}

int yp_debug_pwsp_clocks(uint64_t* out32) {
    if (!out32) return fail(YP_ERR_ARG, "yp_debug_pwsp_clocks: null output");
    HIPCHK(hipDeviceSynchronize());
    HIPCHK(pwsp_read_clocks((unsigned long long*)out32));
    return YP_OK;
}

int yp_debug_contour_clocks(uint64_t* out12) {
    if (!out12) return fail(YP_ERR_ARG, "yp_debug_contour_clocks: null output");
    HIPCHK(hipDeviceSynchronize());
    HIPCHK(contour_read_clocks((unsigned long long*)out12));
    return YP_OK;
}

int yp_debug_ablation(int v) {
    conv_set_debug_ablation(v);
    return 0;
}

int yp_debug_force_conv_cfg(int cfg) {
    conv_dma_force_cfg(cfg);
    return conv_dma_family.num_cfgs;
}

int yp_debug_last_store_form(void) {
    store_form_watched().store(true);
    return last_store_form().exchange(-1);
}

int yp_debug_op_cfg(const yp_engine* e, int i, int* cfg) {
    if (!e || i < 0 || i >= (int)e->ops.size() || !cfg) return fail(YP_ERR_ARG, "bad argument");
    *cfg = op_launch_cfg(*e, e->ops[i]);
    return YP_OK;
}

int yp_debug_conv_families(int* base, int* num_cfgs, int cap) {
    for (int f = 0; f < kNumConvFamilies && f < cap; ++f) {
        if (base) base[f] = kConvFamilies[f]->base;
        if (num_cfgs) num_cfgs[f] = kConvFamilies[f]->num_cfgs;
    }
    return kNumConvFamilies;
}

int yp_debug_host_selftest(yp_engine* e) {
    if (!e) return fail(YP_ERR_ARG, "null engine");
    if (!e->planned) return fail(YP_ERR_STATE, "yp_plan has not been called");
    size_t acc = 0;
    if (!e->finalized)
        for (WeightDesc& w : e->weights) {
            if (!w.have_w || !w.have_b || w.w.empty()) continue;
            std::vector<unsigned char> main, aux;
            pack_weight(*e, w, main, aux);
            acc += main.size() + aux.size();
        }
    for (const Op& o : e->ops) {
        if (o.skip) continue;
        if (fused(o)) build_form_params(*e, o);
        else if (o.kind == OP_CONV) acc += (size_t)conv_params(*e, o).Cout;
    }
    save_tune_cache(*e);
    (void)load_tune_cache(*e);
    {
        const std::string tp = tune_cache_path(*e, true);
        if (!tp.empty() && std::ifstream(tp).good()) {
            std::vector<std::pair<int, std::string>> keep;
            for (const Op& o : e->ops) keep.emplace_back(o.cfg, o.kernel);
            const bool ok = load_tune_cache(*e, true);
            for (size_t i = 0; i < e->ops.size(); ++i) { e->ops[i].cfg = keep[i].first; e->ops[i].kernel = keep[i].second; }
            if (!ok) return fail(YP_ERR_STATE, "packaged tune table %s does not apply to this build's plan", tp.c_str());
        }
    }
    remember_tuning(*e);
    if (!recall_tuning(*e)) return fail(YP_ERR_STATE, "internal: tuning memo lost");
    int rc = build_lane_schedule(*e);
    if (rc != YP_OK) return rc;
    std::vector<char> rec(e->ops.size(), 0);
    std::vector<char> seen(e->n_lanes, 0);
    seen[0] = 1;
    for (const auto& stp : e->lane_steps) {
        const Op& o = e->ops[stp.op];
        for (int j : stp.waits)
            if (!rec[j]) return fail(YP_ERR_STATE, "internal: %s waits on %s, which never records", o.name.c_str(), e->ops[j].name.c_str());
        if (!seen[o.lane]) {
            bool via = stp.fork;
            for (int j : stp.waits) via |= seen[e->ops[j].lane] != 0;
            if (!via) return fail(YP_ERR_STATE, "internal: lane %d would start outside the capture at %s", o.lane, o.name.c_str());
            seen[o.lane] = 1;
        }
        if (stp.record) rec[stp.op] = 1;
    }
    int used = 0;
    for (int l = 1; l < e->n_lanes; ++l) used += seen[l];
    if (used != (int)e->lanes_used.size()) return fail(YP_ERR_STATE, "internal: %d side lanes launch but %zu are joined", used, e->lanes_used.size());
    {
        int next_id = 0, lane0_nodes = 0, bad = 0, nsteps = 0;
        auto launch = [&](const yp_engine::LaneStep& stp, std::vector<int>& deps, std::vector<int>& tail) -> int {
            for (int d : deps) if (d < 0 || d >= next_id) ++bad;
            if (deps.empty() && lane0_nodes > 0) ++bad;
            if (e->ops[stp.op].lane == 0) ++lane0_nodes;
            tail.assign(1, next_id++);
            ++nsteps;
            return YP_OK;
        };
        size_t joined = 0;
        auto finish = [&](std::vector<int>& all) -> int { joined = all.size(); return YP_OK; };
        int edges = 0;
        rc = walk_lane_dag<int>(*e, launch, finish, &edges);
        if (rc != YP_OK) return rc;
        if (bad) return fail(YP_ERR_STATE, "internal: the capture DAG has %d dangling or forward dependencies", bad);
        if (joined != e->lanes_used.size() + 1 || nsteps != (int)e->lane_steps.size()) return fail(YP_ERR_STATE, "internal: the capture ends behind %zu lane tails, %zu lanes launched", joined, e->lanes_used.size() + 1);
    }
    return (int)e->lane_steps.size() + (acc == 0 ? 0 : 0);
}

int yp_set_nms(yp_engine* e, float conf, float iou) {
    if (!e) return fail(YP_ERR_ARG, "null engine");
    if (!(conf >= 0.f && conf < 1.f) || !(iou > 0.f && iou <= 1.f)) return fail(YP_ERR_ARG, "yp_set_nms: conf in [0,1), iou in (0,1]");
    if (conf == e->nms_conf && iou == e->nms_iou) return YP_OK;
    e->nms_conf = conf; e->nms_iou = iou;
    e->nms_dirty = true;
    return YP_OK;
}

int yp_set_autotune(yp_engine* e, int enable) {
    if (!e) return fail(YP_ERR_ARG, "null engine");
    e->tune = enable != 0;
    e->tuned.clear();
    return YP_OK;
}

int yp_tuning_export(const yp_engine* e, int32_t* cfg_out, int cap) {
    if (!e) return fail(YP_ERR_ARG, "null engine");
    if (!e->allocated) return fail(YP_ERR_STATE, "yp_tuning_export: no forward has run on the current plan");
    const int n = (int)e->ops.size();
    if (cfg_out) {
        if (cap < n) return fail(YP_ERR_ARG, "yp_tuning_export: %d ops, buffer holds %d", n, cap);
        for (int i = 0; i < n; ++i) cfg_out[i] = e->ops[i].cfg;
    }
    return n;
}

int yp_tuning_import(yp_engine* e, int B, int H, int W, const int32_t* cfg, int n) {
    if (!e || !cfg) return fail(YP_ERR_ARG, "null argument");
    if (!e->finalized) return fail(YP_ERR_STATE, "yp_finalize has not been called");
    HIPCHK(hipSetDevice(e->device));
    HIPCHK(hipDeviceSynchronize());
    e->planned = false;
    int rc = make_plan(*e, B, H, W);
    if (rc != YP_OK) return rc;
    if (n != (int)e->ops.size()) return fail(YP_ERR_ARG, "yp_tuning_import: %d ids for a plan of %zu ops", n, e->ops.size());
    std::vector<int> v(cfg, cfg + n);
    if (!apply_tuning(*e, v.data(), n)) return fail(YP_ERR_ARG, "yp_tuning_import: a configuration id is not launchable for its layer in this build");
    remember_tuning(*e);
    return YP_OK;
}

int yp_set_graph(yp_engine* e, int enable) {
    if (!e) return fail(YP_ERR_ARG, "null engine");
    if (enable < 0 || enable > 3) return fail(YP_ERR_ARG, "yp_set_graph: 0 eager, 1 replay with lanes, 2 replay without lanes, 3 auto");
    const bool lanes = enable != 2;
    if (enable != 0 && e->use_lanes != lanes && e->gexec) {
        HIPCHK(hipSetDevice(e->device));
        if (e->have_last) HIPCHK(hipEventSynchronize(e->ev_done));
        drop_graph(*e);
        e->auto_replay.clear();
    }
    e->use_graph = enable != 0;
    e->graph_auto = enable == 3;
    if (enable != 0) e->use_lanes = lanes;
    return YP_OK;
}

int yp_profile(yp_engine* e, const uint8_t* in_dev, int B, int H, int W, float* det_out, int32_t* idx_out,
               float* coeff_out, float* ms_out, int iters, void* stream) {
    int rc = prepare(e, B, H, W, in_dev, det_out);
    if (rc != YP_OK) return rc;
    if (!ms_out || iters <= 0) return fail(YP_ERR_ARG, "bad profile arguments");
    HIPCHK(hipSetDevice(e->device));
    hipStream_t st = (hipStream_t)stream;
    RunArgs a{in_dev, det_out, idx_out, coeff_out};
    const size_t n = e->ops.size();
// ... 151 lines not shown
```

### yolo-puncture_amd/csrc/pwsp.hip

```cpp
#include "common.h"
#include <cstdlib>
#include <algorithm>

namespace yp {

typedef __attribute__((ext_vector_type(4))) unsigned u32x4;

__device__ unsigned long long g_ps_clk[32];
#define PS_STAMP(i) do { if (blockIdx.x == 0 && tid == 0) g_ps_clk[i] = __builtin_readcyclecounter(); } while (0)
hipError_t pwsp_read_clocks(unsigned long long* out32) { return hipMemcpyFromSymbol(out32, HIP_SYMBOL(g_ps_clk), 32 * sizeof(unsigned long long)); }

constexpr int PS_MF = 2;
constexpr int PS_NW = 16;
constexpr int PS_NT = PS_NW * 64;

template <int NS, int SP>
__global__ __launch_bounds__(PS_NT) void pwsp_kernel(const PwSpParams p) {
    constexpr int FN = NS / 16;
    constexpr int BK = 64, NSLOT = 3;
    constexpr int W_INSTR = NS / 8;
    constexpr int SLOT = W_INSTR * 1024;
    constexpr unsigned OOB = 0x80000000u;
    constexpr int KS = SP == 1 ? 3 : SP == 2 ? 7 : 1, PAD = KS / 2;
    constexpr int PIX = SP == 3 ? NS * 2 : NS * 2 + 8;
    constexpr int DW_NP = NS / 2, DW_G = PS_NT / DW_NP;
    constexpr int DW_PH = NS == 64 ? 5 : 3, DW_PW = 3;
    static_assert(SP != 3 || NS == 32, "the pool form keeps 64-byte pixel rows");

    extern __shared__ __attribute__((aligned(1024))) unsigned char smem[];
    unsigned char* const dump = smem + NSLOT * SLOT;
    unsigned char* const img = smem + NSLOT * SLOT + 1024;

    const int tid = threadIdx.x, lane = tid & 63;
    const int wave = __builtin_amdgcn_readfirstlane(tid >> 6);
    const int fr = lane & 15, fc = lane >> 4;
    const int HW = p.H * p.W;
    const int nsl = p.C1 / NS;

    int b, sl;
    {
        const int bid = blockIdx.x, nwg = gridDim.x;
        if ((p.B & 7) == 0) { const int xcd = bid & 7, j = bid >> 3; b = (j / nsl) * 8 + xcd; sl = j % nsl; }
        else { b = bid / nsl; sl = bid % nsl; }
        (void)nwg;
    }
    PS_STAMP(0);
    const int n0 = sl * NS;
    const bool spatial = SP != 0 && n0 >= p.sp_c0 && n0 + NS <= p.sp_c0 + p.Csp;
    const int nk = (p.Kpad1 + BK - 1) / BK;
    const __amdgpu_buffer_rsrc_t wrs = __builtin_amdgcn_make_buffer_rsrc((void*)p.w1, 0, (int)p.w1_bytes, 0x00020000);

    const int dgx = (p.W + DW_PW - 1) / DW_PW, dgy = (p.H + DW_PH - 1) / DW_PH;
    const int IW = (SP == 1 || SP == 2) ? dgx * DW_PW + 2 * PAD : p.W, IH = (SP == 1 || SP == 2) ? dgy * DW_PH + 2 * PAD : p.H;
    constexpr int PXS = 256 * 128;
    unsigned char* const wring = smem;
    unsigned char* const pxa = img;
    unsigned char* const pxb = img + 2 * PXS;
    const int nmf = (HW + 15) >> 4;
    const __amdgpu_buffer_rsrc_t xrs = __builtin_amdgcn_make_buffer_rsrc((void*)p.x, 0, (int)p.x_bytes, 0x00020000);
    unsigned pa_off[2], pb_off[2];
    int p_kc[2], w_kc;
#pragma unroll
    for (int j = 0; j < 2; ++j) {
        const int row = (wave * 2 + j) * 8 + (lane >> 3);
        const int c = (lane & 7) ^ ((row >> 1) & 7);
        p_kc[j] = c * 8;
        pa_off[j] = (row < HW && row < 256) ? (unsigned)((b * HW + row) * p.x_stride + p.x_coff + c * 8) * 2u : OOB;
        pb_off[j] = (row + 256 < HW) ? (unsigned)((b * HW + row + 256) * p.x_stride + p.x_coff + c * 8) * 2u : OOB;
    }
    unsigned wconst;
    {
        const int s_ = wave * 64 + lane;
        const int row = s_ >> 3, pc = s_ & 7;
        const int c = pc ^ ((row >> 1) & 7);
        w_kc = c * 8;
        wconst = (wave < W_INSTR) ? (unsigned)(((n0 + row) * p.Kpad1 + c * 8) * 2) : OOB;
    }
    auto kbyte = [&](int kt) { return (unsigned)(kt * BK) * 2u; };
    auto issue_A = [&](int kt) {
        const bool live = kt < nk;
        const unsigned kb = kbyte(kt);
        __builtin_amdgcn_raw_ptr_buffer_load_lds(wrs, (lds_void*)((wave < W_INSTR) ? wring + (kt % NSLOT) * SLOT + wave * 1024 : dump), 16,
                                                 (live && wconst != OOB && kt * BK + w_kc < p.K) ? wconst + kb : OOB, 0, 0, 0);
#pragma unroll
        for (int j = 0; j < 2; ++j)
            __builtin_amdgcn_raw_ptr_buffer_load_lds(xrs, (lds_void*)(pxa + (kt & 1) * PXS + (wave * 2 + j) * 1024), 16,
                                                     (live && pa_off[j] != OOB && kt * BK + p_kc[j] < p.K && !(p.dbg & 2)) ? pa_off[j] + kb : OOB, 0, 0, 0);
    };
    auto issue_B = [&](int kt) {
        const bool live = kt < nk;
        const unsigned kb = kbyte(kt);
#pragma unroll
        for (int j = 0; j < 2; ++j)
            __builtin_amdgcn_raw_ptr_buffer_load_lds(xrs, (lds_void*)(pxb + (kt & 1) * PXS + (wave * 2 + j) * 1024), 16,
                                                     (live && pb_off[j] != OOB && kt * BK + p_kc[j] < p.K && !(p.dbg & 2)) ? pb_off[j] + kb : OOB, 0, 0, 0);
    };

    f32x4 acc[FN][PS_MF];
#pragma unroll
    for (int a = 0; a < FN; ++a) {
        const float4 b4 = *(const float4*)(p.bias1 + n0 + a * 16 + fc * 4);
#pragma unroll
        for (int f = 0; f < PS_MF; ++f) acc[a][f] = f32x4{b4.x, b4.y, b4.z, b4.w};
    }
    const bool hasA = wave < nmf, hasB = wave + 16 < nmf;
    issue_A(0); issue_B(0); issue_A(1);
    PS_STAMP(1);
    const unsigned fro = (unsigned)(fr * 128), frs = (unsigned)((fr >> 1) & 7);
    for (int g = 0; g < nk; ++g) {
        if (g < 16) PS_STAMP(8 + g);
        __builtin_amdgcn_s_waitcnt(5 | (7 << 4) | (0xF << 8));
        __builtin_amdgcn_s_barrier();
        issue_B(g + 1);
        const unsigned char* ws = wring + (g % NSLOT) * SLOT;
        bf16x8 wf[2][FN];
#pragma unroll
        for (int s_ = 0; s_ < 2; ++s_)
#pragma unroll
            for (int a = 0; a < FN; ++a) wf[s_][a] = *(const bf16x8*)(ws + a * 2048 + fro + (((unsigned)(s_ * 4 + fc) ^ frs) << 4));
        if (hasA && !(p.dbg & 1)) {
            const unsigned char* ps = pxa + (g & 1) * PXS + wave * 2048;
#pragma unroll
            for (int s_ = 0; s_ < 2; ++s_) {
                const bf16x8 xf = *(const bf16x8*)(ps + fro + (((unsigned)(s_ * 4 + fc) ^ frs) << 4));
#pragma unroll
                for (int a = 0; a < FN; ++a) acc[a][0] = __builtin_amdgcn_mfma_f32_16x16x32_bf16(wf[s_][a], xf, acc[a][0], 0, 0, 0);
            }
        }
        __builtin_amdgcn_s_waitcnt(5 | (7 << 4) | (0xF << 8));
        __builtin_amdgcn_s_barrier();
        issue_A(g + 2);
        if (hasB && !(p.dbg & 1)) {
            const unsigned char* ps = pxb + (g & 1) * PXS + wave * 2048;
#pragma unroll
            for (int s_ = 0; s_ < 2; ++s_) {
                const bf16x8 xf = *(const bf16x8*)(ps + fro + (((unsigned)(s_ * 4 + fc) ^ frs) << 4));
#pragma unroll
                for (int a = 0; a < FN; ++a) acc[a][1] = __builtin_amdgcn_mfma_f32_16x16x32_bf16(wf[s_][a], xf, acc[a][1], 0, 0, 0);
            }
        }
    }
    __builtin_amdgcn_s_waitcnt(0 | (7 << 4) | (0xF << 8));
    __syncthreads();
    if (SP == 1 || SP == 2) {
        if (spatial) {
            const int n16 = (IH * IW * PIX + 15) >> 4;
            for (int i = tid; i < n16; i += PS_NT) *(uint4*)(img + (size_t)i * 16) = make_uint4(0, 0, 0, 0);
            __syncthreads();
        }
    }

    PS_STAMP(2);
#pragma unroll
    for (int f = 0; f < PS_MF; ++f) {
        const int m = (wave + PS_NW * f) * 16 + fr;
        const bool ok = m < HW;
        const int py = ok ? m / p.W : 0, px = ok ? m - py * p.W : 0;
#pragma unroll
        for (int a = 0; a < FN; ++a) {
            float v[4] = {acc[a][f][0], acc[a][f][1], acc[a][f][2], acc[a][f][3]};
            if (p.act1 == ACT_SILU) silu4_packed(v);
            const int co = a * 16 + fc * 4;
            if (SP == 0 && p.res1 && ok) {
                const uint2 rr = *(const uint2*)((const __bf16*)p.res1 + (size_t)(b * HW + m) * p.res1_stride + p.res1_coff + n0 + co);
                v[0] += __uint_as_float(rr.x << 16); v[1] += __uint_as_float(rr.x & 0xffff0000u);
                v[2] += __uint_as_float(rr.y << 16); v[3] += __uint_as_float(rr.y & 0xffff0000u);
            }
            __attribute__((aligned(8))) __bf16 o[4] = {(__bf16)v[0], (__bf16)v[1], (__bf16)v[2], (__bf16)v[3]};
            if (ok && p.y1) *(uint2*)((__bf16*)p.y1 + (size_t)(b * HW + m) * p.y1_stride + p.y1_coff + n0 + co) = *(const uint2*)o;
            if (SP != 0 && ok && spatial) *(uint2*)(img + (size_t)((py + PAD) * IW + px + PAD) * PIX + co * 2) = *(const uint2*)o;
        }
    }
    PS_STAMP(3);
    if (SP == 0) return;
    if (!spatial || (p.dbg & 4)) return;
    __syncthreads();
    PS_STAMP(4);

    const int cs0 = n0 - p.sp_c0;
    if constexpr (SP == 1 || SP == 2) {
        typedef __attribute__((address_space(3))) const unsigned* lds_u32p;
        typedef __attribute__((address_space(3))) const f32x2* lds_f2p;
        typedef __attribute__((address_space(3))) f32x2* lds_f2w;
        const int cp = tid % DW_NP, grp = tid / DW_NP;
        const int c = cs0 + cp * 2;
        const unsigned img_l = (unsigned)(size_t)(__attribute__((address_space(3))) unsigned char*)img;
        const unsigned wl_l = img_l + (unsigned)(((IH * IW * PIX) + 15) & ~15);
        f32x2 wk[KS == 3 ? 9 : 1];
        if constexpr (KS == 3) {
#pragma unroll
            for (int t = 0; t < 9; ++t) {
                const unsigned d = *(const unsigned*)((const __bf16*)p.wd + (size_t)t * p.Csp + c);
                wk[t] = f32x2{__uint_as_float(d << 16), __uint_as_float(d & 0xffff0000u)};
            }
        } else {
            for (int t = tid; t < KS * KS * DW_NP; t += PS_NT) {
                const unsigned d = *(const unsigned*)((const __bf16*)p.wd + (size_t)(t / DW_NP) * p.Csp + cs0 + (t % DW_NP) * 2);
                *(lds_f2w)(size_t)(wl_l + (unsigned)t * 8u) = f32x2{__uint_as_float(d << 16), __uint_as_float(d & 0xffff0000u)};
            }
            __syncthreads();
        }
        const f32x2 bias = f32x2{p.biasd[c], p.biasd[c + 1]};
        const int npatch = dgx * dgy;
        for (int q = grp; q < npatch; q += DW_G) {
            const int qy = q / dgx, qx = q - qy * dgx;
            const int oy0 = qy * DW_PH, ox0 = qx * DW_PW;
            f32x2 o[DW_PH][DW_PW];
#pragma unroll
            for (int i = 0; i < DW_PH; ++i)
#pragma unroll
                for (int j = 0; j < DW_PW; ++j) o[i][j] = bias;
            unsigned rowa = img_l + (unsigned)((oy0 * IW + ox0) * PIX + cp * 4);
#pragma unroll
            for (int r = 0; r < DW_PH + KS - 1; ++r) {
                unsigned wa = wl_l + (unsigned)cp * 8u;
                asm volatile("" : "+v"(wa));
                f32x2 xin[DW_PW + KS - 1];
#pragma unroll
                for (int cc = 0; cc < DW_PW + KS - 1; ++cc) {
                    const unsigned d = *(lds_u32p)(size_t)(rowa + (unsigned)(cc * PIX));
                    xin[cc] = f32x2{__uint_as_float(d << 16), __uint_as_float(d & 0xffff0000u)};
                }
#pragma unroll
                for (int i = 0; i < DW_PH; ++i) {
                    const int ky = r - i;
                    if (ky < 0 || ky >= KS) continue;
#pragma unroll
                    for (int kx = 0; kx < KS; ++kx) {
                        f32x2 w;
                        if constexpr (KS == 3) w = wk[ky * 3 + kx];
                        else w = *(lds_f2p)(size_t)(wa + (unsigned)((ky * KS + kx) * DW_NP * 8));
#pragma unroll
                        for (int j = 0; j < DW_PW; ++j) o[i][j] = __builtin_elementwise_fma(xin[j + kx], w, o[i][j]);
                    }
                }
                rowa += (unsigned)(IW * PIX);
#pragma unroll
                for (int i = 0; i < DW_PH; ++i) {
                    asm volatile("" : "+v"(o[i][0]), "+v"(o[i][1]), "+v"(o[i][2]));
                }
            }
            const unsigned pix0 = (unsigned)(b * HW + oy0 * p.W + ox0);
#pragma unroll
            for (int i = 0; i < DW_PH; ++i)
#pragma unroll
                for (int j = 0; j < DW_PW; ++j) {
                    if (oy0 + i >= p.H || ox0 + j >= p.W) continue;
                    float v0 = o[i][j][0], v1 = o[i][j][1];
                    if (p.actd == ACT_SILU) { v0 = silu_rcp(v0); v1 = silu_rcp(v1); }
                    const unsigned pix = pix0 + (unsigned)(i * p.W + j);
                    if (p.res) {
                        const unsigned rr = *(const unsigned*)((const __bf16*)p.res + (size_t)(pix * (unsigned)p.res_stride + (unsigned)(p.res_coff + c)));
                        v0 += __uint_as_float(rr << 16); v1 += __uint_as_float(rr & 0xffff0000u);
                    }
                    __attribute__((aligned(4))) __bf16 ob[2] = {(__bf16)v0, (__bf16)v1};
                    *(unsigned*)((__bf16*)p.y2 + (size_t)(pix * (unsigned)p.y2_stride + (unsigned)(p.y2_coff + c))) = *(const unsigned*)ob;
                }
        }
    } else if constexpr (SP == 3) {
        unsigned char* const bufA = img;
        unsigned char* const bufB = img + (size_t)HW * 64;
        unsigned char* const tmp = img + (size_t)HW * 128;
        const int items = HW * 4, W = p.W, H = p.H;
        for (int i = tid; i < items; i += PS_NT) *(uint4*)(bufA + i * 16) = bf16x8_key(*(const uint4*)(bufA + i * 16));
        __syncthreads();
        for (int stage = 0; stage < 3; ++stage) {
            const unsigned char* src = (stage & 1) ? bufB : bufA;
            unsigned char* dst = (stage & 1) ? bufA : bufB;
            for (int i = tid; i < items; i += PS_NT) {
                const int pxl = i >> 2, y = pxl / W, x = pxl - y * W;
                const int x0 = max(x - 2, 0), x1 = max(x - 1, 0), x3 = min(x + 1, W - 1), x4 = min(x + 2, W - 1);
                const unsigned char* row = src + (size_t)(y * W) * 64 + (i & 3) * 16;
                uint4 m = *(const uint4*)(row + x * 64);
                m = pkmax4(m, *(const uint4*)(row + x0 * 64));
                m = pkmax4(m, *(const uint4*)(row + x1 * 64));
                m = pkmax4(m, *(const uint4*)(row + x3 * 64));
                m = pkmax4(m, *(const uint4*)(row + x4 * 64));
                *(uint4*)(tmp + i * 16) = m;
            }
            __syncthreads();
            __bf16* yb = (__bf16*)p.y2 + (size_t)b * HW * p.y2_stride + p.y2_coff + stage * p.Csp + cs0;
            for (int i = tid; i < items; i += PS_NT) {
                const int pxl = i >> 2, y = pxl / W, x = pxl - y * W;
                const int y0 = max(y - 2, 0), y1 = max(y - 1, 0), y3 = min(y + 1, H - 1), y4 = min(y + 2, H - 1);
                const unsigned char* col = tmp + (size_t)x * 64 + (i & 3) * 16;
                uint4 m = *(const uint4*)(col + (size_t)(y * W) * 64);
                m = pkmax4(m, *(const uint4*)(col + (size_t)(y0 * W) * 64));
                m = pkmax4(m, *(const uint4*)(col + (size_t)(y1 * W) * 64));
                m = pkmax4(m, *(const uint4*)(col + (size_t)(y3 * W) * 64));
                m = pkmax4(m, *(const uint4*)(col + (size_t)(y4 * W) * 64));
                *(uint4*)(dst + i * 16) = m;
                *(uint4*)(yb + (size_t)pxl * p.y2_stride + (i & 3) * 8) = bf16x8_key(m);
            }
            __syncthreads();
        }
    }
    PS_STAMP(5);
}

static size_t pwsp_lds_bytes(const PwSpParams& p, int NS) {
    const size_t ring = (size_t)3 * (NS / 8) * 1024 + 1024;
    const size_t px = (size_t)4 * 256 * 128;
    size_t sp = 0;
    if (p.sp == 3) sp = (size_t)p.H * p.W * 64 * 3;
    else if (p.sp != 0) {
        const int pad = p.sp == 1 ? 1 : 3, PH = NS == 64 ? 5 : 3, PW = 3;
        const int IH = (p.H + PH - 1) / PH * PH + 2 * pad, IW = (p.W + PW - 1) / PW * PW + 2 * pad;
        sp = (((size_t)IH * IW * (NS * 2 + 8) + 15) & ~(size_t)15) + (p.sp == 2 ? (size_t)49 * (NS / 2) * 8 : 0);
    }
    return ring + std::max(px, sp);
}

int pwsp_slice(const PwSpParams& p) {
    if (p.sp == 3) return 32;
    static const int force = env_int("YOLOP_PWSP_NS", 0);
    if (force == 32) return 32;
    if (force == 64 && (p.C1 % 64) == 0 && (p.sp == 0 || ((p.sp_c0 % 64) == 0 && (p.Csp % 64) == 0))) return 64;
    if ((p.C1 % 64) == 0 && (p.sp == 0 || ((p.sp_c0 % 64) == 0 && (p.Csp % 64) == 0)) && (long)p.B * (p.C1 / 64) >= 96) return 64;
    return 32;
}

bool pwsp_valid(const PwSpParams& p) {
    if (p.sp < 0 || p.sp > 3) return false;
    const int NS = pwsp_slice(p);
    if ((p.C1 % NS) != 0 || (p.K % 32) != 0 || p.Kpad1 != p.K || p.K < 64) return false;
    if (p.H * p.W > 16 * PS_MF * PS_NW || p.H < 1 || p.W < 1) return false;
    if ((p.x_stride & 7) || (p.x_coff & 7) || p.x_bytes >= (1ull << 31) || p.w1_bytes >= (1ull << 31)) return false;
    if (p.y1 && ((p.y1_stride & 3) || (p.y1_coff & 3))) return false;
    if (p.res1 && (p.sp != 0 || (p.res1_stride & 3) || (p.res1_coff & 3))) return false;
    if ((p.C1 + 127) / 128 * 128 < p.C1) return false;
    if (p.sp != 0) {
        if (!p.y2 || (p.sp_c0 % NS) != 0 || (p.Csp % NS) != 0 || p.sp_c0 < 0 || p.sp_c0 + p.Csp > p.C1) return false;
        if ((p.y2_stride & 7) || (p.y2_coff & 7)) return false;
        if (p.res && ((p.res_stride & 1) || (p.res_coff & 1))) return false;
        if (p.sp == 3 && p.res) return false;
    } else if (!p.y1) return false;
    return pwsp_lds_bytes(p, NS) <= 160 * 1024;
}

const char* pwsp_kernel_name(const PwSpParams& p) {
    const int NS = pwsp_slice(p);
    static const char* n[2][4] = {{"pwsp_kernel<32,0>", "pwsp_kernel<32,1>", "pwsp_kernel<32,2>", "pwsp_kernel<32,3>"},
                                  {"pwsp_kernel<64,0>", "pwsp_kernel<64,1>", "pwsp_kernel<64,2>", "pwsp_kernel<64,3>"}};
    return n[NS == 64][p.sp];
}

template <int NS, int SP>
static hipError_t launch_pwsp_t(const PwSpParams& p, hipStream_t st) {
    const size_t sh = pwsp_lds_bytes(p, NS);
    auto kern = pwsp_kernel<NS, SP>;
    static size_t granted = 0;
    if (hipError_t e = allow_dynamic_lds((const void*)kern, sh, granted)) return e;
    hipLaunchKernelGGL(kern, dim3((unsigned)(p.B * (p.C1 / NS))), dim3(PS_NT), sh, st, p);
    return hipGetLastError();
}

hipError_t launch_pwsp(const PwSpParams& p, hipStream_t st) {
    if (!pwsp_valid(p)) return hipErrorInvalidValue;
    const int NS = pwsp_slice(p);
    if (NS == 64) {
        switch (p.sp) {
            case 0: return launch_pwsp_t<64, 0>(p, st);
            case 1: return launch_pwsp_t<64, 1>(p, st);
            case 2: return launch_pwsp_t<64, 2>(p, st);
            default: return hipErrorInvalidValue;
        }
    }
    switch (p.sp) {
        case 0: return launch_pwsp_t<32, 0>(p, st);
        case 1: return launch_pwsp_t<32, 1>(p, st);
        case 2: return launch_pwsp_t<32, 2>(p, st);
        default: return launch_pwsp_t<32, 3>(p, st);
    }
}

}
```

### yolo-puncture_amd/engine.py

```python
from __future__ import annotations

import ctypes as C
import os
from typing import Dict, List, Optional, Tuple

import numpy as np
import torch

from .weights import fold_state

_LIB: Optional[C.CDLL] = None
_HERE = os.path.dirname(os.path.abspath(__file__))
LIB_PATH = os.environ.get("YOLOP_LIB") or os.path.join(_HERE, "libyolop.so")

YP_BF16, YP_F32 = 0, 1
TASK_DETECT, TASK_SEGMENT = 0, 1
OP_KINDS = {0: "stem", 1: "conv", 2: "dwconv", 3: "pool5", 4: "upsample", 5: "attn", 6: "head", 7: "convT", 8: "pool3", 9: "amax"}
FORMS = ("plain", "dwpw", "dwpw_tail", "s2pw", "frontend", "c2f", "scdown", "pwsp", "cls_out")


class ModelDesc(C.Structure):
    _fields_ = [("variant", C.c_int), ("nc", C.c_int), ("task", C.c_int), ("dtype", C.c_int), ("max_det", C.c_int), ("family", C.c_int)]


class YolopError(RuntimeError):
    pass


def load_library(path: Optional[str] = None) -> C.CDLL:
    global _LIB
    if _LIB is not None and path is None:
        return _LIB
    p = path or LIB_PATH
    if not os.path.isfile(p):
        raise YolopError(f"{p} not found: build it with `python -c 'import __graft_entry__ as g; g.build()'` "
                         f"(hipcc --offload-arch=gfx950). There is no CPU fallback for the hot path.")
    lib = C.CDLL(p)
    vp, ip, fp = C.c_void_p, C.POINTER(C.c_int), C.POINTER(C.c_float)
    lib.yp_last_error.restype = C.c_char_p
    lib.yp_create.argtypes = [C.POINTER(ModelDesc), C.c_int, C.POINTER(vp)]
    lib.yp_destroy.argtypes = [vp]
    lib.yp_weight_count.argtypes = [vp]
    lib.yp_weight_info.argtypes = [vp, C.c_int, C.c_char_p, C.c_int, C.POINTER(C.c_int64), ip]
    lib.yp_set_weight.argtypes = [vp, C.c_char_p, vp, C.POINTER(C.c_int64), C.c_int]
    lib.yp_finalize.argtypes = [vp]
    lib.yp_forward.argtypes = [vp, vp, C.c_int, C.c_int, C.c_int, vp, vp, vp, vp]
    lib.yp_proto.argtypes = [vp, C.POINTER(vp), ip, ip]
    lib.yp_masks.argtypes = [vp, C.c_int, vp, vp, C.c_int, C.c_int, C.c_int, C.c_int, vp, vp, vp, C.c_int, C.c_int, vp]
    lib.yp_id_mask_resized.argtypes = [vp, C.c_int, vp, vp] + [C.c_int] * 5 + [vp, vp, C.c_int, C.c_int, vp]
    lib.yp_id_mask_resized.restype = C.c_int
    lib.yp_mask_contours.argtypes = [vp, C.c_int, C.c_int, C.c_int, C.c_int, vp, vp, vp, vp]
    lib.yp_mask_contours.restype = C.c_int
    lib.yp_mask_contours_scaled.argtypes = [vp, C.c_int, C.c_int, C.c_int, C.c_int, C.c_int, vp, vp, vp, C.c_int, vp, C.c_int, C.c_int, vp]
    lib.yp_mask_contours_scaled.restype = C.c_int
    lib.yp_mask_contours_large_workspace.argtypes = [C.c_int, C.c_int, C.c_int]
    lib.yp_mask_contours_large_workspace.restype = C.c_size_t
    lib.yp_mask_contours_large.argtypes = [vp, C.c_int, C.c_int, C.c_int, C.c_int, C.c_int, vp, vp, vp, C.c_int, vp, C.c_int, C.c_int, C.c_int, vp,
                                           C.c_size_t, vp]
    lib.yp_mask_contours_large.restype = C.c_int
    lib.yp_plan.argtypes = [vp, C.c_int, C.c_int, C.c_int]
    lib.yp_max_batch.argtypes = [vp, C.c_int, C.c_int]
    lib.yp_max_batch.restype = C.c_int
    lib.yp_debug_topk_anchors.argtypes = [C.POINTER(vp), C.c_int, C.POINTER(C.c_int), C.c_int, vp, vp, vp]
    lib.yp_debug_topk_anchors.restype = C.c_int
    lib.yp_op_info.argtypes = [vp, C.c_int, C.c_char_p, C.c_int, ip, C.POINTER(C.c_double), C.POINTER(C.c_double)]
    lib.yp_op_output.argtypes = [vp, C.c_int, ip, ip, ip]
    lib.yp_op_kernel.argtypes = [vp, C.c_int, C.c_char_p, C.c_int]
    lib.yp_op_fusion.argtypes = [vp, C.c_int, ip, ip]
    lib.yp_op_fusion.restype = C.c_int
    lib.yp_debug_op_form.argtypes = [vp, C.c_int, ip, ip, C.c_int]
    lib.yp_debug_op_form.restype = C.c_int
    lib.yp_run_op.argtypes = [vp, C.c_int, vp, vp, vp, vp, vp]
    lib.yp_tensor_write.argtypes = [vp, C.c_int, C.c_int, C.c_int, vp]
    lib.yp_tensor_count.argtypes = [vp]
    lib.yp_tensor_info.argtypes = [vp, C.c_int, C.c_char_p, C.c_int, ip, ip]
    lib.yp_tensor_read.argtypes = [vp, C.c_int, vp]
    lib.yp_profile.argtypes = [vp, vp, C.c_int, C.c_int, C.c_int, vp, vp, vp, vp, C.c_int, vp]
    lib.yp_set_graph.argtypes = [vp, C.c_int]
    lib.yp_set_autotune.argtypes = [vp, C.c_int]
    lib.yp_set_nms.argtypes = [vp, C.c_float, C.c_float]
    lib.yp_set_nms.restype = C.c_int
    lib.yp_debug_host_selftest.argtypes = [vp]
    lib.yp_debug_host_selftest.restype = C.c_int
    lib.yp_tuning_source.argtypes = [vp]
    lib.yp_tuning_source.restype = C.c_int
    lib.yp_debug_graph_info.argtypes = [vp, C.POINTER(C.c_int64)]
    lib.yp_debug_graph_info.restype = C.c_int
    lib.yp_debug_head_positions.argtypes = [vp, C.POINTER(C.c_int64)]
    lib.yp_debug_head_positions.restype = C.c_int
    lib.yp_debug_marker.argtypes = [vp]
    lib.yp_debug_marker.restype = C.c_int
    lib.yp_debug_force_conv_cfg.argtypes = [C.c_int]
    lib.yp_debug_op_cfg.argtypes = [vp, C.c_int, ip]
    lib.yp_debug_op_cfg.restype = C.c_int
    lib.yp_debug_last_store_form.argtypes = []
    lib.yp_debug_last_store_form.restype = C.c_int
    lib.yp_debug_conv_families.argtypes = [ip, ip, C.c_int]
    lib.yp_debug_conv_families.restype = C.c_int
    lib.yp_debug_ablation.argtypes = [C.c_int]
    lib.yp_debug_head_clocks.argtypes = [C.POINTER(C.c_uint64)]
    lib.yp_debug_head_branch_clocks.argtypes = [C.POINTER(C.c_uint64)]
    lib.yp_debug_contour_clocks.argtypes = [C.POINTER(C.c_uint64)]
    lib.yp_debug_pwsp_clocks.argtypes = [C.POINTER(C.c_uint64)]
    lib.yp_letterbox.argtypes = [vp, C.c_int, C.c_int, vp] + [C.c_int] * 7 + [vp]
    lib.yp_letterbox.restype = C.c_int
    lib.yp_letterbox_batch.argtypes = [vp, C.c_int, C.c_int, C.c_int, vp] + [C.c_int] * 7 + [vp]
    lib.yp_letterbox_batch.restype = C.c_int
    lib.yp_masks_frames.argtypes = [vp, vp, C.c_int, vp, C.c_long, vp, C.c_int, C.c_int, vp, vp]
    lib.yp_masks_frames.restype = C.c_int
    lib.yp_masks_frames_input.argtypes = [vp, vp, C.c_int, vp, C.c_long, vp, C.c_int, C.c_int, vp, vp]
    lib.yp_masks_frames_input.restype = C.c_int
    lib.yp_comm_unique_id.argtypes = [vp]
    lib.yp_comm_create.argtypes = [vp, C.c_int, C.c_int, C.c_int, C.POINTER(vp)]
    lib.yp_allgather.argtypes = [vp, vp, vp, C.c_size_t, vp]
    lib.yp_comm_destroy.argtypes = [vp]
    for fn in ("yp_comm_unique_id", "yp_comm_create", "yp_allgather", "yp_comm_destroy"):
        getattr(lib, fn).restype = C.c_int
    for fn in ("yp_create", "yp_destroy", "yp_weight_count", "yp_weight_info", "yp_set_weight", "yp_finalize",
               "yp_forward", "yp_proto", "yp_masks", "yp_plan", "yp_op_info", "yp_op_output", "yp_op_input", "yp_tensor_count",
               "yp_tensor_info", "yp_tensor_read", "yp_profile", "yp_set_graph", "yp_run_op", "yp_tensor_write",
               "yp_op_kernel", "yp_set_autotune", "yp_debug_force_conv_cfg", "yp_debug_ablation"):
        getattr(lib, fn).restype = C.c_int
    if path is None:
        _LIB = lib
    return lib


EXPORTS = ["yp_last_error", "yp_create", "yp_destroy", "yp_weight_count", "yp_weight_info", "yp_set_weight",
           "yp_finalize", "yp_forward", "yp_proto", "yp_masks", "yp_id_mask_resized", "yp_plan", "yp_op_info", "yp_op_output", "yp_op_input", "yp_op_fusion",
           "yp_tensor_count", "yp_tensor_info", "yp_tensor_read", "yp_profile", "yp_set_graph", "yp_run_op",
           "yp_tensor_write", "yp_op_kernel", "yp_set_autotune", "yp_tuning_export", "yp_tuning_import", "yp_set_nms", "yp_debug_force_conv_cfg", "yp_debug_op_cfg", "yp_debug_op_form", "yp_debug_last_store_form", "yp_debug_conv_families", "yp_debug_ablation", "yp_debug_head_clocks", "yp_debug_head_branch_clocks", "yp_debug_head_winners", "yp_debug_contour_clocks", "yp_debug_pwsp_clocks", "yp_debug_host_selftest", "yp_debug_graph_info", "yp_tuning_source", "yp_debug_head_positions", "yp_debug_marker", "yp_max_batch", "yp_debug_topk_anchors", "yp_letterbox", "yp_letterbox_batch", "yp_masks_frames", "yp_masks_frames_input", "yp_mask_contours",
           "yp_mask_contours_scaled", "yp_mask_contours_large_workspace", "yp_mask_contours_large", "yp_comm_unique_id", "yp_comm_create", "yp_allgather", "yp_comm_destroy",
           "yp_u2net_create", "yp_u2net_destroy", "yp_u2net_weight_count", "yp_u2net_weight_info", "yp_u2net_set_weight", "yp_u2net_finalize",
           "yp_u2net_forward", "yp_u2net_forward_crops", "yp_u2net_set_graph", "yp_u2net_tensor_count", "yp_u2net_tensor_info", "yp_u2net_tensor_read",
           "yp_u2net_op_count", "yp_u2net_op_info",
           "yp_cls_create", "yp_cls_destroy", "yp_cls_weight_count", "yp_cls_weight_info", "yp_cls_set_weight", "yp_cls_finalize",
           "yp_cls_forward", "yp_cls_set_graph", "yp_cls_tensor_count", "yp_cls_tensor_info", "yp_cls_tensor_read"]


MAX_ANCHORS = 294912


def topk_anchors(mk: List[torch.Tensor], hw, k: int) -> Tuple[torch.Tensor, torch.Tensor]:
    lib = load_library()
    if len(mk) != 3 or len(hw) != 3:
        raise ValueError("three levels")
    B = int(mk[0].shape[0])
    dev = mk[0].device
    for t, (h, w) in zip(mk, hw):
        if t.dtype != torch.int32 or not t.is_contiguous() or t.device != dev or tuple(t.shape) != (B, int(h) * int(w)):
            raise ValueError("mk[l] must be contiguous int32 [B, H_l * W_l] on one device")
    sel = torch.full((B, 512), -1, dtype=torch.int32, device=dev)
    thr = torch.zeros((B,), dtype=torch.int32, device=dev)
    ptrs = (C.c_void_p * 3)(*[t.data_ptr() for t in mk])
    hwa = (C.c_int * 6)(*[int(v) for pair in hw for v in pair])
    rc = lib.yp_debug_topk_anchors(ptrs, B, hwa, int(k), C.c_void_p(sel.data_ptr()), C.c_void_p(thr.data_ptr()), C.c_void_p(_stream_ptr(dev)))
    if rc < 0:
        raise YolopError(lib.yp_last_error().decode())
    return sel, thr


def conv_families() -> List[Tuple[int, int]]:
    lib = load_library()
    n = lib.yp_debug_conv_families(None, None, 0)
    base, num = (C.c_int * n)(), (C.c_int * n)()
    lib.yp_debug_conv_families(base, num, n)
    return list(zip(base, num))


def _stream_ptr(device: torch.device) -> int:
    return int(torch.cuda.current_stream(device).cuda_stream)


def letterbox_device(src: torch.Tensor, geo: dict, out: Optional[torch.Tensor] = None, pad_value: int = 114) -> torch.Tensor:
    if not (src.is_cuda and src.dtype == torch.uint8 and src.dim() == 3 and src.shape[2] == 3 and src.is_contiguous()):
        raise ValueError("letterbox_device needs a contiguous uint8 CUDA tensor [H,W,3]")
    oh, ow = int(geo["out_h"]), int(geo["out_w"])
    if out is None:
        out = torch.empty((oh, ow, 3), dtype=torch.uint8, device=src.device)
    if not (out.is_cuda and out.dtype == torch.uint8 and tuple(out.shape) == (oh, ow, 3) and out.is_contiguous()):
        raise ValueError(f"letterbox_device: output must be a contiguous uint8 CUDA tensor [{oh},{ow},3]")
    lib = load_library()
    with torch.cuda.device(src.device):
        rc = lib.yp_letterbox(C.c_void_p(src.data_ptr()), int(src.shape[0]), int(src.shape[1]), C.c_void_p(out.data_ptr()), oh, ow,
                              int(geo["new_h"]), int(geo["new_w"]), int(geo["top"]), int(geo["left"]), int(pad_value),
                              C.c_void_p(_stream_ptr(src.device)))
    if rc != 0:
        raise YolopError(lib.yp_last_error().decode())
    return out


def letterbox_batch_device(frames: torch.Tensor, geo: dict, out: torch.Tensor, pad_value: int = 114) -> torch.Tensor:
    if not (frames.is_cuda and frames.dtype == torch.uint8 and frames.dim() == 4 and frames.shape[3] == 3 and frames.is_contiguous()):
        raise ValueError("letterbox_batch_device needs a contiguous uint8 CUDA tensor [n,H,W,3]")
    n = int(frames.shape[0])
    oh, ow = int(geo["out_h"]), int(geo["out_w"])
    if not (out.is_cuda and out.dtype == torch.uint8 and tuple(out.shape) == (n, oh, ow, 3) and out.is_contiguous()):
        raise ValueError(f"letterbox_batch_device: output must be a contiguous uint8 CUDA tensor [{n},{oh},{ow},3]")
    if out.device != frames.device:
        raise ValueError(f"letterbox_batch_device: frames on {frames.device}, output on {out.device}")
    lib = load_library()
    with torch.cuda.device(frames.device):
        rc = lib.yp_letterbox_batch(C.c_void_p(frames.data_ptr()), n, int(frames.shape[1]), int(frames.shape[2]), C.c_void_p(out.data_ptr()),
                                    oh, ow, int(geo["new_h"]), int(geo["new_w"]), int(geo["top"]), int(geo["left"]), int(pad_value),
                                    C.c_void_p(_stream_ptr(frames.device)))
    if rc != 0:
        raise YolopError(lib.yp_last_error().decode())
    return out


CONTOUR_STRATEGIES = {"largest": 0, "all": 1}
_PARTS_CAP = 65


def mask_contours_device(masks: torch.Tensor, max_pts: Optional[int] = None, want_rect: bool = True, strategy: str = "all", want_parts: bool = False,
                         orig_hw: Optional[Tuple[int, int]] = None):
    if not (masks.is_cuda and masks.dtype == torch.uint8 and masks.dim() == 3):
        raise ValueError("mask_contours_device needs a uint8 CUDA tensor [n,H,W]")
    if strategy not in CONTOUR_STRATEGIES:
        raise ValueError(f"strategy must be 'all' or 'largest', got {strategy!r}")
    if orig_hw is not None and not (int(orig_hw[0]) > 0 and int(orig_hw[1]) > 0):
        raise ValueError(f"orig_hw must be a positive (H0, W0), got {orig_hw!r}")
    masks = masks.contiguous()
    n, H, W = (int(v) for v in masks.shape)
    if max_pts is None:
        max_pts = 131072 if n <= 2 else 16384
    dev = masks.device
    o_parts = (n + 1) // 2 * 2
    o_rect = o_parts + (n * _PARTS_CAP + 1) // 2 * 2
    o_pts = o_rect + 4 * n
    buf = torch.empty((o_pts + n * max_pts * 2,), dtype=torch.int32, device=dev)
    lib = load_library()
    with torch.cuda.device(dev):
        base = buf.data_ptr()
        args = (C.c_void_p(masks.data_ptr()), n, H, W, CONTOUR_STRATEGIES[strategy], int(max_pts), C.c_void_p(base + 4 * o_pts), C.c_void_p(base),
                C.c_void_p(base + 4 * o_parts), _PARTS_CAP, C.c_void_p(base + 4 * o_rect if want_rect else None))
        if orig_hw is None:
            rc = lib.yp_mask_contours(*args, C.c_void_p(_stream_ptr(dev)))
        else:
            rc = lib.yp_mask_contours_scaled(*args, int(orig_hw[0]), int(orig_hw[1]), C.c_void_p(_stream_ptr(dev)))
    if rc != 0:
        raise YolopError(lib.yp_last_error().decode())
    return _read_contours(buf, n, int(max_pts), _PARTS_CAP, o_parts, o_rect, o_pts, want_rect, want_parts)


class ContourList(list):
    max_pts: Optional[int] = None


def _read_contours(buf: torch.Tensor, n: int, max_pts: int, parts_cap: int, o_parts: int, o_rect: int, o_pts: int, want_rect: bool, want_parts: bool):
    if n == 0:
        polys = ContourList()
        polys.max_pts = max_pts
        return (polys, (np.zeros((0, 2)) if want_rect else None), []) if want_parts else (polys, (np.zeros((0, 2)) if want_rect else None))
    head_pts = min(max_pts, 1024)
    if n == 1:
        h = buf[:o_pts + 2 * head_pts].cpu().numpy()
        c = h[:1]
        if c[0] > head_pts:
            host = buf[o_pts:o_pts + 2 * int(c[0])].cpu().numpy().reshape(1, -1, 2)
        else:
            host = h[o_pts:].reshape(1, -1, 2)
    else:
        h = buf[:o_pts].cpu().numpy()
        c = h[:n]
        top = int(max(1, c.max()))
        host = buf[o_pts:].view(n, max_pts, 2)[:, :top].cpu().numpy()
    rect = h[o_rect:o_rect + 4 * n].view(np.float64).reshape(n, 2).copy() if want_rect else None
    polys = ContourList(host[i, :c[i]].copy() if c[i] >= 0 else None for i in range(n))
    polys.max_pts = max_pts
    if not want_parts:
        return polys, rect
    pr = h[o_parts:o_parts + n * parts_cap].reshape(n, parts_cap)
    parts = [[int(v) for v in pr[i, 1:1 + min(int(pr[i, 0]), parts_cap - 1)]] if c[i] >= 0 else None for i in range(n)]
    return polys, rect, parts


LARGE_MAX_DIM = 4096
_LARGE_MAX_BORDERS = 65536
YP_CONTOURS_ONLY_DECLINED = 1


def mask_contours_large_device(masks: torch.Tensor, max_pts: Optional[int] = None, want_rect: bool = True, strategy: str = "all",
                               want_parts: bool = False, orig_hw: Optional[Tuple[int, int]] = None):
# ... 296 lines not shown
```

Baseline: 23080.

## Extend paired 16-byte output stores to c2f, dwpw-stream, wres and pwsp kernels

After: 23310 (median of 6 runs). +1.0%, better.

```diff
diff --git a/include/yolop.h b/include/yolop.h
--- a/include/yolop.h
+++ b/include/yolop.h
@@ -155,6 +155,7 @@
 int yp_debug_force_conv_cfg(int cfg);
 int yp_debug_op_cfg(const yp_engine* e, int i, int* cfg);
 int yp_debug_last_store_form(void);
+int yp_debug_max_workgroups(int n);
 int yp_debug_conv_families(int* base, int* num_cfgs, int cap);
 int yp_debug_ablation(int v);
 int yp_debug_head_clocks(uint64_t* out8);
diff --git a/yolo-puncture_amd/csrc/c2f_fused.hip b/yolo-puncture_amd/csrc/c2f_fused.hip
--- a/yolo-puncture_amd/csrc/c2f_fused.hip
+++ b/yolo-puncture_amd/csrc/c2f_fused.hip
@@ -29,6 +29,7 @@
     const int wave = __builtin_amdgcn_readfirstlane(tid >> 6);
     const int fr = lane & 15, fc = lane >> 4;
     const int num_tiles = p.B * tiles_h * tiles_w;
+    const bool wide = p.wide != 0;
 
     const int bid = xcd_remap(blockIdx.x, gridDim.x);
 
@@ -73,14 +74,14 @@
         const int rg = s >> 2, pc = s & 3;
         const int c8 = pc ^ cswz64(rg);
         const int n = rg & 63, ch = rg >> 6;
-        __builtin_amdgcn_raw_ptr_buffer_load_lds(w3rs, (lds_void*)(W3s + ii * 1024), 16, (unsigned)((n * p.Kpad3 + ch * 32 + c8 * 8) * 2), 0, 0, 0);
+        __builtin_amdgcn_raw_ptr_buffer_load_lds(w3rs, (lds_void*)(W3s + ii * 1024), 16, (unsigned)((weight_row_channel(n, wide) * p.Kpad3 + ch * 32 + c8 * 8) * 2), 0, 0, 0);
     }
 
     const int cf = wave & 1, wq = wave >> 1;
     if (tid < 128) Bs[tid] = tid < 32 ? p.bias1[tid] : tid < 64 ? p.bias2[tid - 32] : p.bias3[tid - 64];
     const float* const bias1 = Bs + cf * 16 + fc * 4;
     const float* const bias2 = Bs + 32 + cf * 16 + fc * 4;
-    const float* const bias3 = Bs + 64 + cf * 32 + fc * 4;
+    const float* const bias3 = Bs + 64 + cf * 32;
 
     int tile = bid;
     issue_ab(tile, ABs);
@@ -105,7 +106,10 @@
         const int th = t % tiles_h;
         const int b = t / tiles_h;
         unsigned char* const AB = ABs + (it & 1) * CF_AB;
-        if (it) asm volatile("s_waitcnt vmcnt(4)" ::: "memory");
+        if (it) {
+            if (wide) asm volatile("s_waitcnt vmcnt(2)" ::: "memory");
+            else asm volatile("s_waitcnt vmcnt(4)" ::: "memory");
+        }
         CF_STAMP(0)
         __builtin_amdgcn_s_barrier();
         CF_STAMP(1)
@@ -224,7 +228,7 @@
 #pragma unroll
             for (int j = 0; j < 2; ++j)
 #pragma unroll
-                for (int a = 0; a < 2; ++a) acc[j][a] = *(const f32x4*)(bias3 + a * 16);
+                for (int a = 0; a < 2; ++a) acc[j][a] = *(const f32x4*)(bias3 + acc_channel(a, fc, wide));
 #pragma unroll
             for (int ch = 0; ch < 3; ++ch)
 #pragma unroll
@@ -237,6 +241,18 @@
                 const int ho = th * CF_TH + wq + 4 * j;
                 const bool pix_ok = (ho < p.H) && (wo < p.W);
                 const unsigned m = (unsigned)((b * p.H + ho) * p.W + wo);
+                if (wide) {
+                    float v[2][4];
+#pragma unroll
+                    for (int h = 0; h < 2; ++h) {
+#pragma unroll
+                        for (int q = 0; q < 4; ++q) v[h][q] = acc[j][h][q];
+                        if (p.act3 == ACT_SILU) silu4_packed(v[h]);
+                    }
+                    const int co = cf * 32 + acc_channel(0, fc, true);
+                    store_bf16x8(v[0], v[1], yrs, pix_ok ? (m * (unsigned)p.y_stride + (unsigned)(p.y_coff + co)) * 2u : OOB);
+                    continue;
+                }
 #pragma unroll
                 for (int a = 0; a < 2; ++a) {
                     float v[4] = {acc[j][a][0], acc[j][a][1], acc[j][a][2], acc[j][a][3]};
@@ -265,11 +281,14 @@
     return true;
 }
 
-hipError_t launch_c2f_fused(const C2fParams& p, hipStream_t st) {
+hipError_t launch_c2f_fused(const C2fParams& p_in, hipStream_t st) {
+    C2fParams p = p_in;
+    p.wide = wide_store_ok(p_in.wide, 2, p_in.Cout, p_in.y_stride, p_in.y_coff, false) ? 1 : 0;
     const int tiles_h = (p.H + CF_TH - 1) / CF_TH, tiles_w = (p.W + 15) / 16;
     const int num_tiles = p.B * tiles_h * tiles_w;
     int G = 256;
     if (G > num_tiles) G = num_tiles;
+    if (const int cap = debug_max_workgroups()) G = G < cap ? G : cap;
     static size_t granted = 0;
     if (hipError_t e = allow_dynamic_lds((const void*)c2f_fused_kernel, (size_t)CF_LDS, granted)) return e;
     static const bool clocks = env_on("YOLOP_C2F_CLOCKS");
diff --git a/yolo-puncture_amd/csrc/common.h b/yolo-puncture_amd/csrc/common.h
--- a/yolo-puncture_amd/csrc/common.h
+++ b/yolo-puncture_amd/csrc/common.h
@@ -163,6 +163,7 @@
     const void* w3; const float* bias3; int act3, Kpad3, Cout; size_t w3_bytes;
     void* y; int y_stride, y_coff; size_t y_bytes;
     unsigned long long* clk;
+    int wide;
 };
 bool c2f_fused_valid(const C2fParams& p);
 
@@ -264,6 +265,9 @@
     q.wide = wide_store_ok(p.wide, frags, p.Cout, p.y_stride, p.y_coff, p.out_f32 != 0, p.res, p.res_stride, p.res_coff) ? 1 : 0;
     return q;
 }
+
+inline std::atomic<int>& debug_max_workgroups_ref() { static std::atomic<int> v{0}; return v; }
+inline int debug_max_workgroups() { return debug_max_workgroups_ref().load(std::memory_order_relaxed); }
 
 hipError_t launch_conv(const ConvParams& p, int dtype, hipStream_t st);
 hipError_t launch_conv_igemm(const ConvParams& p, int dtype, hipStream_t st);
@@ -334,6 +338,7 @@
     const void* w_pw; int Kpad; size_t wpw_bytes; const float* b_pw; int act_pw;
     void* y; int y_stride, y_coff; size_t y_bytes; int Cout; int out_f32;
     unsigned long long* clk;
+    int wide;
     const void* w3; int Kpad3; size_t w3_bytes; const float* b3; int C3;
     float* y3; int y3_stride, y3_coff; size_t y3_bytes;
     unsigned* keys;
@@ -351,6 +356,7 @@
     const void* res; int res_stride, res_coff;
     void* y2; int y2_stride, y2_coff;
     int dbg;
+    int wide;
 };
 bool pwsp_valid(const PwSpParams& p);
 const char* pwsp_kernel_name(const PwSpParams& p);
diff --git a/yolo-puncture_amd/csrc/conv_dwpw_stream.hip b/yolo-puncture_amd/csrc/conv_dwpw_stream.hip
--- a/yolo-puncture_amd/csrc/conv_dwpw_stream.hip
+++ b/yolo-puncture_amd/csrc/conv_dwpw_stream.hip
@@ -23,11 +23,19 @@
     const int tid = threadIdx.x, lane = tid & 63;
     const int wave = __builtin_amdgcn_readfirstlane(tid >> 6);
     const int fr = lane & 15, fc = lane >> 4;
+    const bool wide = NFW % 2 == 0 && p.wide != 0;
 
     const __amdgpu_buffer_rsrc_t xrs = __builtin_amdgcn_make_buffer_rsrc((void*)p.x, 0, (int)p.x_bytes, 0x00020000);
     const __amdgpu_buffer_rsrc_t wrs = __builtin_amdgcn_make_buffer_rsrc((void*)p.w_pw, 0, (int)p.wpw_bytes, 0x00020000);
     const __amdgpu_buffer_rsrc_t yrs = __builtin_amdgcn_make_buffer_rsrc((void*)p.y, 0, (int)p.y_bytes, 0x00020000);
 
+    unsigned hyx[DS_PIECES / NW];
+#pragma unroll
+    for (int j = 0; j < DS_PIECES / NW; ++j) {
+        const int hp = ((wave + j * NW) * 64 + lane) >> 4;
+        const int hy = hp / (DS_TW + 2);
+        hyx[j] = (unsigned)((hy << 8) | (hp - hy * (DS_TW + 2)));
+    }
     auto issue_tile = [&](int tile, int slot) {
         int t = tile;
         const int tw = t % tiles_w; t /= tiles_w;
@@ -40,7 +48,9 @@
             const int ii = wave + j * NW;
             const int s = ii * 64 + lane;
             const int hp = s >> 4, c = s & 15;
-            const int hy = hp / (DS_TW + 2), hx = hp - hy * (DS_TW + 2);
+            unsigned q = hyx[j];
+            asm volatile("" : "+v"(q));
+            const int hy = (int)(q >> 8), hx = (int)(q & 255u);
             const int hi = h0 + hy, wi = w0 + hx;
             const bool ok = tile < num_tiles && hp < DS_HP && (unsigned)hi < (unsigned)p.H && (unsigned)wi < (unsigned)p.W;
             const unsigned voff = ok ? (unsigned)((((b * p.H + hi) * p.W + wi) * p.x_stride + p.x_coff + c * 8) * 2) : OOB;
@@ -66,12 +76,12 @@
     for (int i = 0; i < NFW; ++i) {
 #pragma unroll
         for (int ks = 0; ks < 4; ++ks) {
-            const unsigned voff = (unsigned)((((wave * NFW + i) * 16 + fr) * p.Kpad + (ks >> 1) * 64 + fc * 16 + (ks & 1) * 8) * 2);
+            const unsigned voff = (unsigned)((weight_row_channel((wave * NFW + i) * 16 + fr, wide) * p.Kpad + (ks >> 1) * 64 + fc * 16 + (ks & 1) * 8) * 2);
             const __attribute__((ext_vector_type(4))) unsigned v = __builtin_amdgcn_raw_buffer_load_b128(wrs, voff, 0, 0);
             wreg[ks][i] = __builtin_bit_cast(bf16x8, v);
         }
 #pragma unroll
-        for (int r = 0; r < 4; ++r) { const int co = (wave * NFW + i) * 16 + fc * 4 + r; bpw[i][r] = (co < p.Cout) ? p.b_pw[co] : 0.f; }
+        for (int r = 0; r < 4; ++r) { const int co = wave * NFW * 16 + acc_channel(i, fc, wide) + r; bpw[i][r] = (co < p.Cout) ? p.b_pw[co] : 0.f; }
     }
     wait_vmcnt<0>();
 #pragma unroll
@@ -88,6 +98,7 @@
     const unsigned as_l = lds_addr(As);
     for (int it = 0; tile < num_tiles; tile += G, ++it) {
         if (it == 0) wait_vmcnt<0>();
+        else if (wide) wait_vmcnt<NST / 2>();
         else wait_vmcnt<NST>();
         __builtin_amdgcn_s_barrier();
         const int slot = NSLOT == 2 ? (it & 1) : 0;
@@ -150,6 +161,26 @@
                 for (int f = 0; f < DS_TH; ++f) acc[i][f] = __builtin_amdgcn_mfma_f32_16x16x32_bf16(wreg[ks][i], xf[f], acc[i][f], 0, 0, 0);
         }
         const int wo = tw * DS_TW + fr;
+        if (wide) {
+#pragma unroll
+            for (int j = 0; j < NFW / 2; ++j) {
+                const int co = wave * NFW * 16 + acc_channel(2 * j, fc, true);
+#pragma unroll
+                for (int f = 0; f < DS_TH; ++f) {
+                    const int ho = th * DS_TH + f;
+                    const bool ok = ho < p.H && wo < p.W;
+                    float v[2][4];
+#pragma unroll
+                    for (int h = 0; h < 2; ++h) {
+#pragma unroll
+                        for (int q = 0; q < 4; ++q) v[h][q] = acc[2 * j + h][f][q];
+                        if (p.act_pw == ACT_SILU) silu4_packed(v[h]);
+                    }
+                    store_bf16x8(v[0], v[1], yrs, ok ? (unsigned)((((b * p.H + ho) * p.W + wo) * p.y_stride + p.y_coff + co) * 2) : OOB);
+                }
+            }
+            continue;
+        }
 #pragma unroll
         for (int i = 0; i < NFW; ++i) {
             const int co = (wave * NFW + i) * 16 + fc * 4;
@@ -180,7 +211,9 @@
 }
 
 template <int NW>
-static hipError_t launch_dwpw_stream_t(const DwPwParams& p, hipStream_t st) {
+static hipError_t launch_dwpw_stream_t(const DwPwParams& p_in, hipStream_t st) {
+    DwPwParams p = p_in;
+    p.wide = wide_store_ok(p_in.wide, 8 / NW, p_in.Cout, p_in.y_stride, p_in.y_coff, p_in.out_f32 != 0) ? 1 : 0;
     const size_t sh = (size_t)(NW == 8 ? 2 : 1) * DS_HB + DS_AB;
     auto kern = conv_dwpw_stream_kernel<NW>;
     static size_t granted = 0;
@@ -188,7 +221,8 @@
     const int tiles_h = (p.H + DS_TH - 1) / DS_TH, tiles_w = (p.W + DS_TW - 1) / DS_TW;
     const int num_tiles = p.B * tiles_h * tiles_w;
     const int gmax = NW == 8 ? 256 : 512;
-    const int G = num_tiles < gmax ? num_tiles : gmax;
+    int G = num_tiles < gmax ? num_tiles : gmax;
+    if (const int cap = debug_max_workgroups()) G = G < cap ? G : cap;
     hipLaunchKernelGGL(kern, dim3((unsigned)G), dim3(NW * 64), sh, st, p, tiles_h, tiles_w, num_tiles, G);
     return hipGetLastError();
 }
diff --git a/yolo-puncture_amd/csrc/conv_wres.hip b/yolo-puncture_amd/csrc/conv_wres.hip
--- a/yolo-puncture_amd/csrc/conv_wres.hip
+++ b/yolo-puncture_amd/csrc/conv_wres.hip
@@ -14,8 +14,10 @@
     for (int i = 0; i < NFW; ++i) asm volatile("" : "+v"(ws[i]));
 }
 
-template <int TP, int WGN, bool HAS_RES>
-__global__ __launch_bounds__(WR_NW * 64) void conv_wres_kernel(const ConvParams p, const int NB, const int nblk, const int G, const int TPe) {
+template <int TP, int WGN> constexpr bool wres_paired() { return (TP / (16 * (WR_NW / WGN))) * (WR_MAXNF / WGN) >= 8; }
+
+template <int TP, int WGN, bool HAS_RES, bool CLK>
+__device__ __forceinline__ void conv_wres_body(const ConvParams p, const int NB, const int nblk, const int G, const int TPe) {
     constexpr int WGM = WR_NW / WGN;
     constexpr int FM = TP / (16 * WGM);
     constexpr int NFW = WR_MAXNF / WGN;
@@ -34,8 +36,11 @@
     const int wave = __builtin_amdgcn_readfirstlane(tid >> 6);
     const int wm = wave % WGM, wn = wave / WGM;
     const int fr = lane & 15, fc = lane >> 4;
+    const bool wide = wres_paired<TP, WGN>() && p.wide != 0;
     const int ntiles = (p.M + TPe - 1) / TPe;
     const int HoWo = p.Ho * p.Wo;
+    unsigned long long clk[5] = {0, 0, 0, 0, 0}, last = CLK ? __builtin_amdgcn_s_memtime() : 0ull;
+#define WRES_STAMP(i) if constexpr (CLK) { const unsigned long long now = __builtin_amdgcn_s_memtime(); clk[i] += now - last; last = now; }
 
     const int xcd = blockIdx.x & 7, slot = blockIdx.x >> 3;
     const int nb = slot % nblk, g = (slot / nblk) * 8 + xcd;
@@ -85,7 +90,7 @@
             const int s = ii * 64 + lane;
             const int r = s / cpr, pc = s - r * cpr;
             const int c = pc ^ (r & mW);
-            const unsigned voff = (unsigned)(((n0 + r) * p.Kpad + c * 8) * 2);
+            const unsigned voff = (unsigned)(((n0 + weight_row_channel(r, wide)) * p.Kpad + c * 8) * 2);
             __builtin_amdgcn_raw_ptr_buffer_load_lds(wrs, (lds_void*)(Ws + ii * 1024), 16, voff, 0, 0, 0);
         }
     }
@@ -97,7 +102,7 @@
     for (int i = 0; i < NFW; ++i)
 #pragma unroll
         for (int r = 0; r < 4; ++r) {
-            const int co = n0 + (wn * nfw + i) * 16 + fc * 4 + r;
+            const int co = wres_paired<TP, WGN>() ? n0 + wn * nfw * 16 + acc_channel(i, fc, wide) + r : n0 + (wn * nfw + i) * 16 + fc * 4 + r;
             bias[i][r] = (i < nfw && co < p.Cout) ? p.bias[co] : 0.f;
         }
     wait_vmcnt<0>();
@@ -106,11 +111,15 @@
 #pragma unroll
         for (int r = 0; r < 4; ++r) asm volatile("" : "+v"(bias[i][r]));
 
+    WRES_STAMP(0)
     for (int it = 0; tile < ntiles; tile += Gt, ++it) {
         if (it == 0) wait_vmcnt<0>();
+        else if (wide) wait_vmcnt<FM * NFW / 2>();
         else wait_vmcnt<FM * NFW>();
         __builtin_amdgcn_s_barrier();
+        WRES_STAMP(1)
         if (tile + Gt < ntiles) issue_tile(tile + Gt, Xs + ((it & 1) ^ 1) * xtile);
+        WRES_STAMP(2)
         const unsigned char* const XA = Xs + (it & 1) * xtile;
         const unsigned char* const XB = XA + (size_t)TP * RBA;
         f32x4 acc[NFW][FM];
@@ -158,10 +167,33 @@
         };
         if (KA > 0) run_segment(XA, RBA, 0, KA >> 5, mA);
         run_segment(XB, RBB, KA >> 3, KB >> 5, mB);
+        WRES_STAMP(3)
 #pragma unroll
         for (int f = 0; f < FM; ++f) {
             const int ri = (wm * FM + f) * 16 + fr;
             const long m = (long)tile * TPe + ri;
+            if (wide) {
+#pragma unroll
+                for (int j = 0; j < NFW / 2; ++j) {
+                    const int co = n0 + wn * nfw * 16 + acc_channel(2 * j, fc, true);
+                    const bool ok = 2 * j < nfw && ri < TPe && m < p.M && co < p.Cout;
+                    float v[2][4];
+#pragma unroll
+                    for (int h = 0; h < 2; ++h) {
+#pragma unroll
+                        for (int q = 0; q < 4; ++q) v[h][q] = acc[2 * j + h][f][q];
+                        if (p.act == ACT_SILU && 2 * j < nfw) silu4_packed(v[h]);
+                    }
+                    if (HAS_RES) {
+                        uint2 rr[2];
+                        load_res_bf16x8((const __bf16*)p.res + m * p.res_stride + p.res_coff + co, ok, rr[0], rr[1]);
+                        add_res_bf16x4(v[0], rr[0]);
+                        add_res_bf16x4(v[1], rr[1]);
+                    }
+                    store_bf16x8(v[0], v[1], yrs, ok ? (unsigned)((m * p.y_stride + p.y_coff + co) * 2) : OOB);
+                }
+                continue;
+            }
 #pragma unroll
             for (int i = 0; i < NFW; ++i) {
                 const int co = n0 + (wn * nfw + i) * 16 + fc * 4;
@@ -178,8 +210,23 @@
                 __builtin_amdgcn_raw_buffer_store_b64(*(const __attribute__((ext_vector_type(2))) unsigned*)o, yrs, off, 0, 0);
             }
         }
+        WRES_STAMP(4)
     }
     wait_vmcnt<0>();
+    if constexpr (CLK) {
+        if (lane == 0)
+            for (int i = 0; i < 5; ++i) p.clk[((size_t)blockIdx.x * WR_NW + wave) * 5 + i] = clk[i];
+    }
+#undef WRES_STAMP
+}
+
+template <int TP, int WGN, bool HAS_RES>
+__global__ __launch_bounds__(WR_NW * 64) void conv_wres_kernel(const ConvParams p, const int NB, const int nblk, const int G, const int TPe) {
+    conv_wres_body<TP, WGN, HAS_RES, false>(p, NB, nblk, G, TPe);
+}
+template <int TP, int WGN>
+__global__ __launch_bounds__(WR_NW * 64) void conv_wres_clk_kernel(const ConvParams p, const int NB, const int nblk, const int G, const int TPe) {
+    conv_wres_body<TP, WGN, false, true>(p, NB, nblk, G, TPe);
 }
 
 struct WresCfg { int TP, WGN; const char* name; };
@@ -218,9 +265,10 @@
 }
 
 template <int TP, int WGN, bool HAS_RES>
-static hipError_t launch_wres_t(const ConvParams& p, const WresCfg& k, hipStream_t st) {
+static hipError_t launch_wres_t(const ConvParams& p_in, const WresCfg& k, hipStream_t st) {
     int NB, nblk;
-    wres_blocks(p, k, NB, nblk);
+    wres_blocks(p_in, k, NB, nblk);
+    const ConvParams p = with_store_form(p_in, wres_paired<TP, WGN>() ? NB / (16 * WGN) : 1);
     const size_t sh = wres_lds(p, k);
     auto kern = conv_wres_kernel<TP, WGN, HAS_RES>;
     static size_t granted = 0;
@@ -230,10 +278,33 @@
     int lanes8 = gmax / (8 * nblk);
     if (lanes8 < 1) lanes8 = 1;
     while (lanes8 > 1 && (lanes8 - 1) * 8 >= ntiles) --lanes8;
+    if (const int cap = debug_max_workgroups()) while (lanes8 > 1 && lanes8 * 8 * nblk > cap) --lanes8;
     const int G = lanes8 * 8 * nblk;
     const long lanes = (long)lanes8 * 8;
     const int rounds = (int)((p.M + lanes * TP - 1) / (lanes * TP));
     const int TPe = tile_balance_enabled(2) ? (int)((p.M + lanes * rounds - 1) / (lanes * rounds)) : TP;
+    if constexpr (TP == 128 && WGN == 2 && !HAS_RES) {
+        static const bool clocks = env_on("YOLOP_WRES_CLOCKS");
+        if (clocks) {
+            auto kc = conv_wres_clk_kernel<TP, WGN>;
+            static size_t granted_c = 0;
+            if (hipError_t e = allow_dynamic_lds((const void*)kc, sh, granted_c)) return e;
+            ConvParams q = p;
+            const size_t n = (size_t)G * WR_NW * 5;
+            if (hipMalloc((void**)&q.clk, n * 8) != hipSuccess) return hipErrorOutOfMemory;
+            hipLaunchKernelGGL(kc, dim3((unsigned)G), dim3(WR_NW * 64), sh, st, q, NB, nblk, G, TPe);
+            (void)hipStreamSynchronize(st);
+            std::vector<unsigned long long> h(n);
+            (void)hipMemcpy(h.data(), q.clk, n * 8, hipMemcpyDeviceToHost);
+            (void)hipFree(q.clk);
+            double s5[5] = {0, 0, 0, 0, 0};
+            for (size_t w = 0; w < n / 5; ++w)
+                for (int i = 0; i < 5; ++i) s5[i] += (double)h[w * 5 + i];
+            fprintf(stderr, "[wres clocks] %s G=%d tiles=%d  %s stores  per-wave mean cycles: prologue %.0f  wait+barrier %.0f  issue %.0f  k loop %.0f  epilogue %.0f\n",
+                    k.name, G, (p.M + TPe - 1) / TPe, p.wide ? "16-byte" : "8-byte", s5[0] / (n / 5), s5[1] / (n / 5), s5[2] / (n / 5), s5[3] / (n / 5), s5[4] / (n / 5));
+            return hipGetLastError();
+        }
+    }
     hipLaunchKernelGGL(kern, dim3((unsigned)G), dim3(WR_NW * 64), sh, st, p, NB, nblk, G, TPe);
     return hipGetLastError();
 }
diff --git a/yolo-puncture_amd/csrc/engine.hip b/yolo-puncture_amd/csrc/engine.hip
--- a/yolo-puncture_amd/csrc/engine.hip
+++ b/yolo-puncture_amd/csrc/engine.hip
@@ -700,6 +700,7 @@
     p.shortcut = m2.res.t >= 0 ? 1 : 0;
     p.w3 = w3.d_w; p.bias3 = w3.d_b; p.act3 = o.act; p.Kpad3 = w3.Kpad; p.Cout = o.out.C; p.w3_bytes = w3.mat_bytes;
     p.y = to.ptr; p.y_stride = to.C; p.y_coff = o.out.coff; p.y_bytes = to.bytes;
+    p.wide = (e.dtype == DT_BF16 && !to.f32 && !e.narrow_store) ? 1 : 0;
     if (m1.in.t != o.in.t || m1.in.coff != o.in.coff + p.C || m2.out.t != o.in.t || m2.out.coff != o.in.coff + 2 * p.C || o.in.C != 3 * p.C ||
         m1.k != 3 || m2.k != 3 || m1.s != 1 || m2.s != 1 || m1.out.C != p.C || m2.out.C != p.C || m1.res.t >= 0 ||
         (m2.res.t >= 0 && (m2.res.t != m1.in.t || m2.res.coff != m1.in.coff)) || (to.f32 && e.dtype == DT_BF16)) p.C = 0;
@@ -742,6 +743,7 @@
     p.x = ti.ptr; p.x_stride = ti.C; p.x_coff = c1.in.coff; p.x_bytes = ti.bytes; p.B = e.pB; p.H = ti.H; p.W = ti.W; p.K = c1.in.C;
     p.w1 = w1.d_w; p.bias1 = w1.d_b; p.act1 = c1.act; p.Kpad1 = w1.Kpad; p.C1 = c1.out.C; p.w1_bytes = w1.mat_bytes;
     p.dbg = conv_debug_ablation();
+    p.wide = (e.dtype == DT_BF16 && !t1.f32 && !e.narrow_store) ? 1 : 0;
     if (!pair || o.pw_store) { p.y1 = t1.ptr ? t1.ptr : (void*)1; p.y1_stride = t1.C; p.y1_coff = c1.out.coff; }
     if (!pair) {
         if (c1.res.t >= 0) { const TensorDesc& tr = e.tensors[c1.res.t]; p.res1 = tr.ptr ? tr.ptr : (const void*)1; p.res1_stride = tr.C; p.res1_coff = c1.res.coff; }
@@ -796,6 +798,7 @@
     p.w_pw = wp.d_w; p.Kpad = wp.Kpad; p.wpw_bytes = wp.mat_bytes; p.b_pw = wp.d_b; p.act_pw = c.act;
     p.y = to.ptr; p.y_stride = to.C; p.y_coff = c.out.coff; p.y_bytes = to.bytes; p.Cout = c.out.C;
     p.out_f32 = (to.f32 && e.dtype == DT_BF16) ? 1 : 0;
+    p.wide = (e.dtype == DT_BF16 && !p.out_f32 && !e.narrow_store) ? 1 : 0;
     return p;
 }
 
@@ -2396,6 +2399,8 @@
     store_form_watched().store(true);
     return last_store_form().exchange(-1);
 }
+
+int yp_debug_max_workgroups(int n) { return debug_max_workgroups_ref().exchange(n > 0 ? n : 0); }
 
 int yp_debug_op_cfg(const yp_engine* e, int i, int* cfg) {
     if (!e || i < 0 || i >= (int)e->ops.size() || !cfg) return fail(YP_ERR_ARG, "bad argument");
diff --git a/yolo-puncture_amd/csrc/pwsp.hip b/yolo-puncture_amd/csrc/pwsp.hip
--- a/yolo-puncture_amd/csrc/pwsp.hip
+++ b/yolo-puncture_amd/csrc/pwsp.hip
@@ -36,6 +36,7 @@
     const int fr = lane & 15, fc = lane >> 4;
     const int HW = p.H * p.W;
     const int nsl = p.C1 / NS;
+    const bool wide = SP == 0 && p.wide != 0;
 
     int b, sl;
     {
@@ -74,7 +75,7 @@
         const int row = s_ >> 3, pc = s_ & 7;
         const int c = pc ^ ((row >> 1) & 7);
         w_kc = c * 8;
-        wconst = (wave < W_INSTR) ? (unsigned)(((n0 + row) * p.Kpad1 + c * 8) * 2) : OOB;
+        wconst = (wave < W_INSTR) ? (unsigned)(((n0 + weight_row_channel(row, wide)) * p.Kpad1 + c * 8) * 2) : OOB;
     }
     auto kbyte = [&](int kt) { return (unsigned)(kt * BK) * 2u; };
     auto issue_A = [&](int kt) {
@@ -99,7 +100,7 @@
     f32x4 acc[FN][PS_MF];
 #pragma unroll
     for (int a = 0; a < FN; ++a) {
-        const float4 b4 = *(const float4*)(p.bias1 + n0 + a * 16 + fc * 4);
+        const float4 b4 = *(const float4*)(p.bias1 + n0 + acc_channel(a, fc, wide));
 #pragma unroll
         for (int f = 0; f < PS_MF; ++f) acc[a][f] = f32x4{b4.x, b4.y, b4.z, b4.w};
     }
@@ -156,6 +157,29 @@
         const int m = (wave + PS_NW * f) * 16 + fr;
         const bool ok = m < HW;
         const int py = ok ? m / p.W : 0, px = ok ? m - py * p.W : 0;
+        if (wide) {
+#pragma unroll
+            for (int a = 0; a + 1 < FN; a += 2) {
+                const int co = acc_channel(a, fc, true);
+                float v[2][4];
+#pragma unroll
+                for (int h = 0; h < 2; ++h) {
+#pragma unroll
+                    for (int q = 0; q < 4; ++q) v[h][q] = acc[a + h][f][q];
+                    if (p.act1 == ACT_SILU) silu4_packed(v[h]);
+                }
+                if (SP == 0 && p.res1) {
+                    uint2 rr[2];
+                    load_res_bf16x8((const __bf16*)p.res1 + (size_t)(b * HW + m) * p.res1_stride + p.res1_coff + n0 + co, ok, rr[0], rr[1]);
+                    add_res_bf16x4(v[0], rr[0]);
+                    add_res_bf16x4(v[1], rr[1]);
+                }
+                __attribute__((aligned(16))) __bf16 o[8] = {(__bf16)v[0][0], (__bf16)v[0][1], (__bf16)v[0][2], (__bf16)v[0][3],
+                                                            (__bf16)v[1][0], (__bf16)v[1][1], (__bf16)v[1][2], (__bf16)v[1][3]};
+                if (ok && p.y1) *(uint4*)((__bf16*)p.y1 + (size_t)(b * HW + m) * p.y1_stride + p.y1_coff + n0 + co) = *(const uint4*)o;
+            }
+            continue;
+        }
 #pragma unroll
         for (int a = 0; a < FN; ++a) {
             float v[4] = {acc[a][f][0], acc[a][f][1], acc[a][f][2], acc[a][f][3]};
@@ -346,7 +370,9 @@
 }
 
 template <int NS, int SP>
-static hipError_t launch_pwsp_t(const PwSpParams& p, hipStream_t st) {
+static hipError_t launch_pwsp_t(const PwSpParams& p_in, hipStream_t st) {
+    PwSpParams p = p_in;
+    p.wide = (SP == 0 && p_in.y1 && wide_store_ok(p_in.wide, NS / 16, p_in.C1, p_in.y1_stride, p_in.y1_coff, false, p_in.res1, p_in.res1_stride, p_in.res1_coff)) ? 1 : 0;
     const size_t sh = pwsp_lds_bytes(p, NS);
     auto kern = pwsp_kernel<NS, SP>;
     static size_t granted = 0;
diff --git a/yolo-puncture_amd/engine.py b/yolo-puncture_amd/engine.py
--- a/yolo-puncture_amd/engine.py
+++ b/yolo-puncture_amd/engine.py
@@ -95,6 +95,8 @@
     lib.yp_debug_op_cfg.restype = C.c_int
     lib.yp_debug_last_store_form.argtypes = []
     lib.yp_debug_last_store_form.restype = C.c_int
+    lib.yp_debug_max_workgroups.argtypes = [C.c_int]
+    lib.yp_debug_max_workgroups.restype = C.c_int
     lib.yp_debug_conv_families.argtypes = [ip, ip, C.c_int]
     lib.yp_debug_conv_families.restype = C.c_int
     lib.yp_debug_ablation.argtypes = [C.c_int]
@@ -129,7 +131,7 @@
 EXPORTS = ["yp_last_error", "yp_create", "yp_destroy", "yp_weight_count", "yp_weight_info", "yp_set_weight",
            "yp_finalize", "yp_forward", "yp_proto", "yp_masks", "yp_id_mask_resized", "yp_plan", "yp_op_info", "yp_op_output", "yp_op_input", "yp_op_fusion",
            "yp_tensor_count", "yp_tensor_info", "yp_tensor_read", "yp_profile", "yp_set_graph", "yp_run_op",
-           "yp_tensor_write", "yp_op_kernel", "yp_set_autotune", "yp_tuning_export", "yp_tuning_import", "yp_set_nms", "yp_debug_force_conv_cfg", "yp_debug_op_cfg", "yp_debug_op_form", "yp_debug_last_store_form", "yp_debug_conv_families", "yp_debug_ablation", "yp_debug_head_clocks", "yp_debug_head_branch_clocks", "yp_debug_head_winners", "yp_debug_contour_clocks", "yp_debug_pwsp_clocks", "yp_debug_host_selftest", "yp_debug_graph_info", "yp_tuning_source", "yp_debug_head_positions", "yp_debug_marker", "yp_max_batch", "yp_debug_topk_anchors", "yp_letterbox", "yp_letterbox_batch", "yp_masks_frames", "yp_masks_frames_input", "yp_mask_contours",
+           "yp_tensor_write", "yp_op_kernel", "yp_set_autotune", "yp_tuning_export", "yp_tuning_import", "yp_set_nms", "yp_debug_force_conv_cfg", "yp_debug_op_cfg", "yp_debug_op_form", "yp_debug_last_store_form", "yp_debug_max_workgroups", "yp_debug_conv_families", "yp_debug_ablation", "yp_debug_head_clocks", "yp_debug_head_branch_clocks", "yp_debug_head_winners", "yp_debug_contour_clocks", "yp_debug_pwsp_clocks", "yp_debug_host_selftest", "yp_debug_graph_info", "yp_tuning_source", "yp_debug_head_positions", "yp_debug_marker", "yp_max_batch", "yp_debug_topk_anchors", "yp_letterbox", "yp_letterbox_batch", "yp_masks_frames", "yp_masks_frames_input", "yp_mask_contours",
            "yp_mask_contours_scaled", "yp_mask_contours_large_workspace", "yp_mask_contours_large", "yp_comm_unique_id", "yp_comm_create", "yp_allgather", "yp_comm_destroy",
            "yp_u2net_create", "yp_u2net_destroy", "yp_u2net_weight_count", "yp_u2net_weight_info", "yp_u2net_set_weight", "yp_u2net_finalize",
            "yp_u2net_forward", "yp_u2net_forward_crops", "yp_u2net_set_graph", "yp_u2net_tensor_count", "yp_u2net_tensor_info", "yp_u2net_tensor_read",
```
